# fmazilu/ASR-using-robust-NN

Hardware: AMD Instinct MI355X
Metric: utterances/sec (train, 1 s@16 kHz) (higher is better)
Workload: dtype f32 accumulate, fp16 two-plane split products in the training GEMMs (22-bit operands); 1 GPU; raw 16 kHz waveform -> on-GPU MFCC -> Lipschitz-constrained MLP train step (Adam+NonNeg, simple_norm_constraint rho=0.1), 1xMI355X; global_batch=1024, per_gpu_batch=1024, clip=1 s @ 16 kHz fp32, resident_pool_clips_per_gpu=65536, parallelism=dp1, hip_graph=False

## Files before the change

### asr-using-robust-nn_amd/build.py

```python
from __future__ import annotations

import os
import subprocess
import sys

HERE = os.path.dirname(os.path.abspath(__file__))
CSRC = os.path.join(HERE, "csrc")
OUT = os.path.join(HERE, "lipasr", "liblipasr.so")
SOURCES = ["core.hip", "spectral.hip", "gemm.hip", "mlp.hip", "optim.hip", "mfcc.hip", "mfcc_vjp.hip", "stft_bdft.hip", "lp_attack.hip"]
HEADERS = ["common.h", "mlp.h", "gemm.h", "mfcc_tables.h", "stft.h", os.path.join("..", "..", "include", "lipasr.h")]
EXTRA = {"stft_bdft.hip": ["-fno-slp-vectorize"]}
FLAGS = ["-O3", "--offload-arch=gfx950", "-fPIC", "-std=c++17", "-Wall", "-Wno-unused-function",
         "-fgpu-rdc" if False else "-fno-gpu-rdc"]


def _hipcc() -> str:
    for cand in (os.environ.get("HIPCC"), "/opt/rocm/bin/hipcc", "hipcc"):
        if cand and (os.path.isabs(cand) and os.path.exists(cand) or not os.path.isabs(cand)):
            return cand
    raise RuntimeError("hipcc not found")


def _stale() -> bool:
    if not os.path.exists(OUT):
        return True
    t = os.path.getmtime(OUT)
    deps = [os.path.join(CSRC, s) for s in SOURCES + HEADERS] + [os.path.abspath(__file__)]
    return any(os.path.getmtime(d) > t for d in deps)


def build(force: bool = False, verbose: bool = True) -> str:
    if not force and not _stale():
        return OUT
    objs = []
    procs = []
    os.makedirs(os.path.join(HERE, "build"), exist_ok=True)
    for s in SOURCES:
        obj = os.path.join(HERE, "build", s.replace(".hip", ".o"))
        cmd = [_hipcc(), *FLAGS, *EXTRA.get(s, []), "-c", os.path.join(CSRC, s), "-o", obj]
        if verbose:
            print(" ".join(cmd), flush=True)
        procs.append((s, subprocess.Popen(cmd, stdout=subprocess.PIPE, stderr=subprocess.STDOUT, text=True)))
        objs.append(obj)
    failed = False
    for s, p in procs:
        out, _ = p.communicate()
        if out.strip() and verbose:
            print(out)
        if p.returncode != 0:
            failed = True
            print(f"hipcc failed on {s}:\n{out}", file=sys.stderr)
    if failed:
        raise RuntimeError("liblipasr build failed")
    cmd = [_hipcc(), "--offload-arch=gfx950", "-shared", "-fPIC", *objs, "-o", OUT]
    if verbose:
        print(" ".join(cmd), flush=True)
    subprocess.check_call(cmd)
    return OUT


if __name__ == "__main__":
    print(build(force="--force" in sys.argv))
```

### asr-using-robust-nn_amd/csrc/gemm.h

```cpp
#pragma once
#include "mlp.h"

namespace lipasr {

enum Epi {
  EPI_STORE = 0,
  EPI_BIAS = 1,
  EPI_BIAS_RELU = 2,
  EPI_BIAS_RELU_BN = 3,
  EPI_DZ_INFER = 4,
  EPI_SIGNSTEP = 5,
  EPI_BIAS_RELU_STATS = 6,
  EPI_DH_STATS = 7,
  EPI_DZ_NOBN = 8,
  EPI_BIAS_SOFTMAX_CE = 9,
  EPI_BIAS_RELU_BNX = 10,
  EPI_DH_BNX = 11
};

struct DropArgs {
  int mode;
  float rate;
  uint64_t seed;
  const int* step_dev;
// ... 33 lines not shown
  float* extra_out;
  const float* y;
  float inv_batch;
  float* prob;
  float* dz;
  float* loss_rows;
  float* correct_rows;
  int bf16;
  const unsigned* sa_dyn;
  const unsigned* sb_dyn;
  unsigned* amax_out;
  unsigned* amax_zero;
  float sa, sb;
  int lds_min_tiles;
  const float* zeros;
  int cus;
  int ring;
  int xcd_map;
  unsigned long long* xc_gran;
  unsigned* xc_ctrl;
  int* xc_err;
  int xc_rt_max;
  int Bstat;
  float grad_scale;
  float* h_out;
  float* mmean_w;
  float* mvar_w;
  float* save_w;
  float* dgamma;
  float* dbeta;
};

constexpr int kAmaxSlots = 64, kAmaxStride = 16;
__device__ __forceinline__ float scale_from_amax(const unsigned* p, const float fallback) {
  if (!p) return fallback;
  const float a = wave_max(__uint_as_float(p[(threadIdx.x & 63) * kAmaxStride]));
  if (!(a > 0.0f) || !(a < INFINITY)) return 1.0f;
  int e = 0;
  (void)frexpf(a, &e);
  return ldexpf(1.0f, 14 - e);
}
__device__ __forceinline__ void amax_publish(unsigned* out, float m) {
  m = wave_max(m);
  if ((threadIdx.x & 63) == 0) {
    const unsigned w = (blockIdx.y * gridDim.x + blockIdx.x) * (blockDim.x >> 6) + (threadIdx.x >> 6);
    atomicMax(out + (w & (kAmaxSlots - 1)) * kAmaxStride, __float_as_uint(m));
  }
}
__device__ __forceinline__ void amax_clear(unsigned* out) {
  if (threadIdx.x < kAmaxSlots) out[threadIdx.x * kAmaxStride] = 0u;
}

constexpr int kMaxGroup = 8;
struct GemmGroup {
  int n;
  int tile_start[kMaxGroup + 1];
  GemmArgs g[kMaxGroup];
};

struct GemmKnobs {
  int gemm_mode = 0;
  bool split_dw0 = false;
  bool group_lds = true;
  int xcd_map = 0;
  bool no_ring = false;
  int ring_tile = 2;
  bool ring2 = true;
  bool ring_x1 = true;
};
const GemmKnobs& gemm_knobs();

enum GemmKind { GK_FRAG4 = 0, GK_FRAG16, GK_LDS, GK_RING, GK_RING_X1, GK_RING2, GK_KINDS };

struct GemmPick {
  int kind;
  int tile_m, tile_n, threads;
  size_t lds_bytes;
  const void* fn;
};

int pick_gemm(int amode, int bmode, const GemmArgs& g, GemmPick* out);
int launch_gemm(int amode, int bmode, const GemmArgs& g, hipStream_t st);
int launch_gemm_group_tn(const GemmArgs* gs, int n, hipStream_t st);
GemmArgs gemm_args(const float* A, int lda, const float* B, int ldb, float* C, int ldc, int M, int N, int K, int epi);
int gemm_row_tiles(int amode, int bmode, const GemmArgs& g);
bool exchange_fits(int bmode, int arith, int M, int N, int K, int lds_min_tiles, int xc_rt_max, int cus);

}
```

### asr-using-robust-nn_amd/csrc/gemm.hip

```cpp
#include "gemm.h"
#include <cstdint>
#include <map>
#include <mutex>
#include <type_traits>
#include <utility>

namespace lipasr {

typedef float f32x16 __attribute__((ext_vector_type(16)));
typedef __bf16 bf16x8 __attribute__((ext_vector_type(8)));

__device__ __forceinline__ bf16x8 to_bf16x8(const float (&v)[8]) {
  bf16x8 o;
#pragma unroll
  for (int j = 0; j < 8; ++j) o[j] = (__bf16)v[j];
  return o;
}

typedef _Float16 f16x8 __attribute__((ext_vector_type(8)));
typedef _Float16 f16x2v __attribute__((ext_vector_type(2)));
typedef float f32x2v __attribute__((ext_vector_type(2)));
template <bool UNIT>
__device__ __forceinline__ void split8(const float (&x)[8], const float scale, f16x8& hi, f16x8& lo) {
  unsigned h[4], l[4];
  if constexpr (UNIT) {
#pragma unroll
    for (int i = 0; i < 4; ++i) h[i] = __builtin_bit_cast(unsigned, __builtin_convertvector((f32x2v){x[2 * i], x[2 * i + 1]}, f16x2v));
    asm("v_fma_mixlo_f16 %0, %4, 1.0, -%12 op_sel_hi:[0,0,1]\n\t"
        "v_fma_mixlo_f16 %1, %6, 1.0, -%13 op_sel_hi:[0,0,1]\n\t"
        "v_fma_mixlo_f16 %2, %8, 1.0, -%14 op_sel_hi:[0,0,1]\n\t"
        "v_fma_mixlo_f16 %3, %10, 1.0, -%15 op_sel_hi:[0,0,1]\n\t"
        "v_fma_mixhi_f16 %0, %5, 1.0, -%12 op_sel:[0,0,1] op_sel_hi:[0,0,1]\n\t"
        "v_fma_mixhi_f16 %1, %7, 1.0, -%13 op_sel:[0,0,1] op_sel_hi:[0,0,1]\n\t"
        "v_fma_mixhi_f16 %2, %9, 1.0, -%14 op_sel:[0,0,1] op_sel_hi:[0,0,1]\n\t"
        "v_fma_mixhi_f16 %3, %11, 1.0, -%15 op_sel:[0,0,1] op_sel_hi:[0,0,1]\n\t"
        "s_nop 1"
        : "=&v"(l[0]), "=&v"(l[1]), "=&v"(l[2]), "=&v"(l[3])
        : "v"(x[0]), "v"(x[1]), "v"(x[2]), "v"(x[3]), "v"(x[4]), "v"(x[5]), "v"(x[6]), "v"(x[7]), "v"(h[0]), "v"(h[1]), "v"(h[2]), "v"(h[3]));
  } else {
    const float s = __builtin_bit_cast(float, __builtin_amdgcn_readfirstlane(__builtin_bit_cast(int, scale)));
    asm("v_fma_mixlo_f16 %0, %8, %16, 0 op_sel_hi:[0,0,0]\n\t"
        "v_fma_mixlo_f16 %1, %10, %16, 0 op_sel_hi:[0,0,0]\n\t"
        "v_fma_mixlo_f16 %2, %12, %16, 0 op_sel_hi:[0,0,0]\n\t"
        "v_fma_mixlo_f16 %3, %14, %16, 0 op_sel_hi:[0,0,0]\n\t"
        "v_fma_mixhi_f16 %0, %9, %16, 0 op_sel_hi:[0,0,0]\n\t"
        "v_fma_mixhi_f16 %1, %11, %16, 0 op_sel_hi:[0,0,0]\n\t"
        "v_fma_mixhi_f16 %2, %13, %16, 0 op_sel_hi:[0,0,0]\n\t"
        "v_fma_mixhi_f16 %3, %15, %16, 0 op_sel_hi:[0,0,0]\n\t"
        "v_fma_mixlo_f16 %4, %8, %16, -%0 op_sel_hi:[0,0,1]\n\t"
        "v_fma_mixlo_f16 %5, %10, %16, -%1 op_sel_hi:[0,0,1]\n\t"
        "v_fma_mixlo_f16 %6, %12, %16, -%2 op_sel_hi:[0,0,1]\n\t"
        "v_fma_mixlo_f16 %7, %14, %16, -%3 op_sel_hi:[0,0,1]\n\t"
        "v_fma_mixhi_f16 %4, %9, %16, -%0 op_sel:[0,0,1] op_sel_hi:[0,0,1]\n\t"
        "v_fma_mixhi_f16 %5, %11, %16, -%1 op_sel:[0,0,1] op_sel_hi:[0,0,1]\n\t"
        "v_fma_mixhi_f16 %6, %13, %16, -%2 op_sel:[0,0,1] op_sel_hi:[0,0,1]\n\t"
        "v_fma_mixhi_f16 %7, %15, %16, -%3 op_sel:[0,0,1] op_sel_hi:[0,0,1]\n\t"
        "s_nop 1"
        : "=&v"(h[0]), "=&v"(h[1]), "=&v"(h[2]), "=&v"(h[3]), "=&v"(l[0]), "=&v"(l[1]), "=&v"(l[2]), "=&v"(l[3])
        : "v"(x[0]), "v"(x[1]), "v"(x[2]), "v"(x[3]), "v"(x[4]), "v"(x[5]), "v"(x[6]), "v"(x[7]), "s"(s));
  }
  hi = __builtin_bit_cast(f16x8, make_uint4(h[0], h[1], h[2], h[3]));
  lo = __builtin_bit_cast(f16x8, make_uint4(l[0], l[1], l[2], l[3]));
}
// ... 259 lines not shown
    if (by == 0 && col < g.N) {
      g.dbeta[col] = dbt * g.grad_scale;
      g.dgamma[col] = dg * g.grad_scale;
    }
  }
}

struct BnxPre {
  float p0[4], p1[4], p2[4];
};
__device__ __forceinline__ void bnx_prefetch(const GemmArgs& g, const int gm, const int gn, BnxPre& q) {
  const bool rv = gm < g.M;
#pragma unroll
  for (int e = 0; e < 4; ++e) {
    const bool cv = rv && gn + e < g.N;
    if (g.epi == EPI_BIAS_RELU_BNX) {
      q.p0[e] = cv ? g.bias[gn + e] : 0.0f;
      q.p1[e] = 0.0f; q.p2[e] = 0.0f;
    } else {
      q.p0[e] = cv ? g.aux[(size_t)gm * g.ldc + gn + e] : 0.0f;
      q.p1[e] = cv ? g.save_mean[gn + e] : 0.0f;
      q.p2[e] = cv ? g.save_mean[g.N + gn + e] : 0.0f;
    }
  }
}

__device__ __forceinline__ void bnx_elem(const GemmArgs& g, const int step, const bool cv, const int gm, const int gn, const float acc,
                                         const BnxPre& q, const int e, float& val, float& av, float& s1, float& s2) {
  if (g.epi == EPI_BIAS_RELU_BNX) {
    const float a = cv ? fmaxf(acc + q.p0[e], 0.0f) : 0.0f;
    val = a; av = a; s1 = a; s2 = a * a;
  } else {
    const size_t idx = (size_t)gm * g.ldc + gn;
    const float gg = cv ? acc * dropout_mult(g.drop, step, idx) : 0.0f;
    const float a = q.p0[e];
    const float xh = cv ? (a - q.p1[e]) * q.p2[e] : 0.0f;
    val = gg; av = a; s1 = gg; s2 = gg * xh;
  }
}

__device__ __forceinline__ void xcd_tile(const int L, const int ntx, const int nty, int& bx, int& by) {
  const int total = ntx * nty;
  if (total < 16) { bx = L % ntx; by = L / ntx; return; }
  const int xcd = L & 7, q = L >> 3, base = total >> 3, rem = total & 7;
  const int t = xcd * base + min(xcd, rem) + q;
  int h = (int)(sqrtf((float)(base + (rem ? 1 : 0))) + 0.5f);
  h = max(1, min(h, nty));
  const int per_group = h * ntx, grp = t / per_group, u = t - grp * per_group;
  const int hg = min(h, nty - grp * h);
  bx = u / hg;
  by = grp * h + (u - bx * hg);
}

template <int AMODE, int BMODE, int NW, int BF, bool X = false>
__device__ __forceinline__ void gemm_tile(const GemmArgs& g, const int bx, const int by, const int n_row_tiles) {
  constexpr int TS = 32;
  constexpr int TPR = 8;
  extern __shared__ __attribute__((aligned(16))) float red[];
  float* stat = red + NW * TS * TS;
  const int tid = threadIdx.x, lane = tid & 63, wave = tid >> 6;
  const int r = lane & 31, h = lane >> 5;
  const int m0 = by * TS, n0 = bx * TS;
  const int nch = (g.K + 15) >> 4;
  const bool vecA = (AMODE == 0) && ((g.lda & 3) == 0) && ((reinterpret_cast<uintptr_t>(g.A) & 15) == 0);
  const bool vecB = (BMODE == 0) && ((g.ldb & 3) == 0) && ((reinterpret_cast<uintptr_t>(g.B) & 15) == 0);
  const int m_real = g.ones_row ? g.M - 1 : g.M;
  const int row_a = m0 + r;
  const bool aones = (AMODE == 1) && g.ones_row && (row_a == g.M - 1);
  const int ai = min(row_a, m_real - 1);
  const int bj = min(n0 + r, g.N - 1);

  unsigned xtag = 0;
  if constexpr (X) xtag = xc_tag<32>(XcView{g.xc_gran, g.xc_ctrl, g.xc_err, g.xc_rt_max}, bx);
  float rsa = 1.0f, rsb = 1.0f;
  if (BF == 2) { rsa = scale_from_amax(g.sa_dyn, g.sa); rsb = scale_from_amax(g.sb_dyn, g.sb); }
  if (g.amax_zero && bx == 0 && by == 0) amax_clear(g.amax_zero);
  f32x16 acc;
#pragma unroll
  for (int q = 0; q < 16; ++q) acc[q] = 0.0f;
  float a0[8], b0[8], a1[8], b1[8];
#pragma unroll
  for (int q = 0; q < 8; ++q) { a0[q] = b0[q] = a1[q] = b1[q] = 0.0f; }
  int c = wave;
  if (c < nch) {
    load_frag<AMODE>(g.A, g.lda, ai, c * 16 + 8 * h, g.K, vecA, a0, aones);
    load_frag<BMODE>(g.B, g.ldb, bj, c * 16 + 8 * h, g.K, vecB, b0);
  }
  while (c < nch) {
    const int cn = c + NW;
    if (cn < nch) {
      load_frag<AMODE>(g.A, g.lda, ai, cn * 16 + 8 * h, g.K, vecA, a1, aones);
      load_frag<BMODE>(g.B, g.ldb, bj, cn * 16 + 8 * h, g.K, vecB, b1);
    }
    if (BF == 1) {
      acc = __builtin_amdgcn_mfma_f32_32x32x16_bf16(to_bf16x8(a0), to_bf16x8(b0), acc, 0, 0, 0);
    } else if (BF == 2) {
      acc = mfma_split(a0, b0, rsa, rsb, acc);
    } else {
#pragma unroll
      for (int q = 0; q < 8; ++q) acc = __builtin_amdgcn_mfma_f32_32x32x2f32(a0[q], b0[q], acc, 0, 0, 0);
    }
#pragma unroll
    for (int q = 0; q < 8; ++q) { a0[q] = a1[q]; b0[q] = b1[q]; }
    c = cn;
  }
  if (BF == 2) {
    const float un = 1.0f / (rsa * rsb);
#pragma unroll
// ... 29 lines not shown
        for (int o = TPR; o < 64; o <<= 1) {
          c1[e] += __shfl_xor(c1[e], o, 64);
          c2[e] += __shfl_xor(c2[e], o, 64);
        }
      }
      if (lane < TPR) {
#pragma unroll
        for (int e = 0; e < 4; ++e) {
          stat[(wave * TPR + lane) * 8 + e] = c1[e];
          stat[(wave * TPR + lane) * 8 + 4 + e] = c2[e];
        }
      }
      __syncthreads();
      float* mine = red;
      float* colp = red + 64;
      double* sbuf = reinterpret_cast<double*>(red + 128);
      double* tot = sbuf + 4 * 64;
      if (tid < 2 * TS) {
        const int which = tid / TS, col = tid % TS, l4 = col >> 2, e = col & 3;
        float t = 0.0f;
#pragma unroll
        for (int w = 0; w < 4; ++w) t += stat[(w * TPR + l4) * 8 + which * 4 + e];
        mine[tid] = t;
      }
      __syncthreads();
      BnxLate late;
      bnx_late_load(g, gn, late);
      float mm0, mv0;
      bnx_moving_load(g, by, n0 + tid, tid < TS, mm0, mv0);
      XcView xc{g.xc_gran, g.xc_ctrl, g.xc_err, g.xc_rt_max};
      xc_exchange<256, 32>(xc, bx, by, g.Bstat < 0 ? 0 : n_row_tiles, xtag, mine, sbuf, tot, [&]() {
        if (g.epi == EPI_BIAS_RELU_BNX && gm1[0] < g.M) {
          float* crow = g.C + (size_t)gm1[0] * g.ldc;
          if (gn + 3 < g.N && ((g.ldc & 3) == 0) && ((reinterpret_cast<uintptr_t>(crow) & 15) == 0)) {
            *reinterpret_cast<float4*>(crow + gn) = make_float4(val[0][0], val[0][1], val[0][2], val[0][3]);
          } else {
#pragma unroll
            for (int e = 0; e < 4; ++e)
              if (gn + e < g.N) crow[gn + e] = val[0][e];
          }
        }
      });
      if (tid < TS) bnx_column(g, by, n0 + tid, tid, TS, tot, colp, mm0, mv0);
      __syncthreads();
      bnx_finish<1>(g, step, gm1, gn, val, av, colp, TS, c4, late);
      return;
    }
  }

  const bool stats = (g.epi == EPI_BIAS_RELU_STATS) || (g.epi == EPI_DH_STATS);
  float cs1[4] = {0.f, 0.f, 0.f, 0.f}, cs2[4] = {0.f, 0.f, 0.f, 0.f};
  if (tid < 256) {
    const int step = g.drop.step_dev ? *g.drop.step_dev : 0;
    const int tcol = tid & 7, row = tid >> 3;
    const int c4 = tcol * 4;
    const int gn = n0 + c4;
    float4 s = *reinterpret_cast<const float4*>(red + row * TS + c4);
#pragma unroll
    for (int w = 1; w < NW; ++w) {
      const float4 t = *reinterpret_cast<const float4*>(red + w * TS * TS + row * TS + c4);
      s.x += t.x; s.y += t.y; s.z += t.z; s.w += t.w;
    }
    const int gm = m0 + row;
    if (g.epi == EPI_BIAS_SOFTMAX_CE) {
      const bool rv = gm < g.M;
      float z[4];
      float mx = -INFINITY;
      int am = 0x7fffffff;
#pragma unroll
      for (int e = 0; e < 4; ++e) {
        const bool cv = rv && (gn + e < g.N);
        z[e] = cv ? (&s.x)[e] + g.bias[gn + e] : -INFINITY;
        if (z[e] > mx) { mx = z[e]; am = gn + e; }
      }
#pragma unroll
      for (int o2 = 1; o2 < 8; o2 <<= 1) {
        const float omx = __shfl_xor(mx, o2, 64);
        const int oam = __shfl_xor(am, o2, 64);
        if (omx > mx || (omx == mx && oam < am)) { mx = omx; am = oam; }
      }
      float se = 0.0f;
#pragma unroll
      for (int e = 0; e < 4; ++e) se += (z[e] > -INFINITY) ? expf(z[e] - mx) : 0.0f;
#pragma unroll
      for (int o2 = 1; o2 < 8; o2 <<= 1) se += __shfl_xor(se, o2, 64);
      const float lse = logf(se), inv = 1.0f / se;
      float loss = 0.0f, ymax = -INFINITY;
      int ay = 0x7fffffff;
#pragma unroll
      for (int e = 0; e < 4; ++e) {
        if (rv && gn + e < g.N) {
          const size_t idx = (size_t)gm * g.N + gn + e;
          const float zs = z[e] - mx;
          const float pc = expf(zs) * inv;
          g.C[(size_t)gm * g.ldc + gn + e] = z[e];
          if (g.prob) g.prob[idx] = pc;
          if (g.y) {
            const float yc = g.y[idx];
            if (yc != 0.0f) loss -= yc * (zs - lse);
            if (yc > ymax) { ymax = yc; ay = gn + e; }
            if (g.dz) g.dz[idx] = (pc - yc) * g.inv_batch;
          }
        }
      }
#pragma unroll
      for (int o2 = 1; o2 < 8; o2 <<= 1) {
        loss += __shfl_xor(loss, o2, 64);
        const float oym = __shfl_xor(ymax, o2, 64);
        const int oay = __shfl_xor(ay, o2, 64);
        if (oym > ymax || (oym == ymax && oay < ay)) { ymax = oym; ay = oay; }
      }
      if (rv && tcol == 0) {
        if (g.loss_rows) g.loss_rows[gm] = loss;
        if (g.correct_rows) g.correct_rows[gm] = (am == ay) ? 1.0f : 0.0f;
      }
    } else if (gm < g.M) {
      const float v[4] = {s.x, s.y, s.z, s.w};
      float o[4];
#pragma unroll
      for (int e = 0; e < 4; ++e) {
        float t1 = 0.0f, t2 = 0.0f;
        o[e] = (gn + e < g.N) ? epilogue_elem(g, step, gm, gn + e, v[e], t1, t2) : 0.0f;
        cs1[e] = t1;
        cs2[e] = t2;
      }
      float* crow;
      if (g.ones_row && gm == g.M - 1) crow = g.extra_out;
      else crow = (g.epi == EPI_SIGNSTEP ? g.x_adv : g.C) + (size_t)gm * g.ldc;
      if (gn + 3 < g.N && ((g.ldc & 3) == 0) && ((reinterpret_cast<uintptr_t>(crow) & 15) == 0)) {
        *reinterpret_cast<float4*>(crow + gn) = make_float4(o[0], o[1], o[2], o[3]);
      } else {
#pragma unroll
        for (int e = 0; e < 4; ++e)
          if (gn + e < g.N) crow[gn + e] = o[e];
      }
    }
  }
  if (stats) {
    if (tid < 256) {
#pragma unroll
      for (int e = 0; e < 4; ++e) {
#pragma unroll
        for (int o = TPR; o < 64; o <<= 1) {
          cs1[e] += __shfl_xor(cs1[e], o, 64);
          cs2[e] += __shfl_xor(cs2[e], o, 64);
        }
      }
      if (lane < TPR) {
#pragma unroll
        for (int e = 0; e < 4; ++e) {
          stat[(wave * TPR + lane) * 8 + e] = cs1[e];
          stat[(wave * TPR + lane) * 8 + 4 + e] = cs2[e];
        }
      }
    }
    __syncthreads();
    if (tid < 2 * TS) {
      const int which = tid / TS, col = tid % TS;
      const int l4 = col >> 2, e = col & 3;
      float t = 0.0f;
#pragma unroll
      for (int w = 0; w < 4; ++w) t += stat[(w * TPR + l4) * 8 + which * 4 + e];
      if (n0 + col < g.N) g.part[((size_t)which * n_row_tiles + by) * g.N + n0 + col] = t;
    }
  }
}

template <int AMODE, int BMODE, int NW, int BF = 0, bool X = false>
__global__ __launch_bounds__(64 * NW) void gemm_f32_kernel(GemmArgs g) {
  int bx = blockIdx.x, by = blockIdx.y;
  if (g.xcd_map) xcd_tile(blockIdx.y * gridDim.x + blockIdx.x, gridDim.x, gridDim.y, bx, by);
  gemm_tile<AMODE, BMODE, NW, BF, X>(g, bx, by, gridDim.y);
}


template <int AMODE, int BMODE, int NW, int BF = 0>
__global__ __launch_bounds__(64 * NW) void gemm_f32_grouped_kernel(GemmGroup grp) {
  int p = 0;
  while (p + 1 < grp.n && (int)blockIdx.x >= grp.tile_start[p + 1]) ++p;
  const GemmArgs& g = grp.g[p];
  const int local = blockIdx.x - grp.tile_start[p];
  const int ntx = (g.N + 31) / 32, nty = (g.M + 31) / 32;
  int bx = local % ntx, by = local / ntx;
  if (g.xcd_map && (grp.tile_start[p] & 7) == 0) xcd_tile(local, ntx, nty, bx, by);
  gemm_tile<AMODE, BMODE, NW, BF>(g, bx, by, nty);
}

constexpr int kLdsBK = 32, kLdsLD = 68;

template <int MODE>
__device__ __forceinline__ float4 tile_fetch(const float* __restrict__ P, int ld, int i0, int i_real, int k0, int K,
                                             bool ones_last, int i_last, int tid) {
  float t[4] = {0.f, 0.f, 0.f, 0.f};
  const bool al = ((ld & 3) == 0) && ((reinterpret_cast<uintptr_t>(P) & 15) == 0);
  if (MODE == 0) {
    const int i = i0 + (tid >> 3);
    const int kq = k0 + (tid & 7) * 4;
    const float* p = P + (size_t)min(i, i_real - 1) * ld + kq;
    if (kq + 3 < K && al) {
      const float4 x = *reinterpret_cast<const float4*>(p);
      t[0] = x.x; t[1] = x.y; t[2] = x.z; t[3] = x.w;
    } else {
#pragma unroll
      for (int c = 0; c < 4; ++c) t[c] = (kq + c < K) ? p[c] : 0.0f;
    }
  } else {
    const int k = k0 + (tid >> 4);
    const int iq = i0 + (tid & 15) * 4;
    if (k < K) {
      const float* p = P + (size_t)k * ld;
      if (iq + 3 < i_real && al) {
        const float4 x = *reinterpret_cast<const float4*>(p + iq);
        t[0] = x.x; t[1] = x.y; t[2] = x.z; t[3] = x.w;
      } else {
#pragma unroll
        for (int c = 0; c < 4; ++c) {
          const int i = iq + c;
          t[c] = (ones_last && i == i_last) ? 1.0f : p[min(i, i_real - 1)];
        }
      }
    }
  }
  return make_float4(t[0], t[1], t[2], t[3]);
}

template <int MODE>
__device__ __forceinline__ void tile_store(float* __restrict__ S, int tid, const float4 v) {
  if (MODE == 0) {
    const int i = tid >> 3, kq = (tid & 7) * 4;
    S[(kq + 0) * kLdsLD + i] = v.x;
    S[(kq + 1) * kLdsLD + i] = v.y;
    S[(kq + 2) * kLdsLD + i] = v.z;
    S[(kq + 3) * kLdsLD + i] = v.w;
  } else {
    const int k = tid >> 4, iq = (tid & 15) * 4;
    *reinterpret_cast<float4*>(S + k * kLdsLD + iq) = v;
  }
}

constexpr int kLdsBKMax = 32;
constexpr size_t lds_gemm_bytes(int bk) {
  return ((size_t)(2 * 2 * bk * kLdsLD > 2 * 64 * 64 ? 2 * 2 * bk * kLdsLD : 2 * 64 * 64) + 8 * 16 * 8) * sizeof(float);
}

template <bool X>
__device__ __forceinline__ void lds_tile_epilogue(const GemmArgs& g, const f32x16& acc, float* lds, float* stat, const int bx, const int by,
                                                  const int n_row_tiles, const unsigned xtag) {
  constexpr int TS = 64;
  const int tid = threadIdx.x, lane = tid & 63, wave = tid >> 6;
  const int r = lane & 31, h = lane >> 5;
  const int kh = wave >> 2, wi = (wave >> 1) & 1, wj = wave & 1;
  const int m0 = by * TS, n0 = bx * TS;
  BnxPre xpre[2];
  if constexpr (X) {
    bnx_prefetch(g, m0 + (tid >> 4), n0 + (tid & 15) * 4, xpre[0]);
    bnx_prefetch(g, m0 + (tid >> 4) + 32, n0 + (tid & 15) * 4, xpre[1]);
  }
  float* red = lds;
#pragma unroll
  for (int q = 0; q < 16; ++q) {
    const int row = 32 * wi + (q & 3) + 8 * (q >> 2) + 4 * h;
    red[kh * TS * TS + row * TS + 32 * wj + r] = acc[q];
  }
  __syncthreads();
  const bool stats = (g.epi == EPI_BIAS_RELU_STATS) || (g.epi == EPI_DH_STATS);
  const int step = g.drop.step_dev ? *g.drop.step_dev : 0;
  const int tcol = tid & 15, trow = tid >> 4;
  const int c4 = tcol * 4, gn = n0 + c4;
  if constexpr (X) {
    const int gm2[2] = {m0 + trow, m0 + trow + 32};
    float val[2][4], av[2][4], c1[4] = {0.f, 0.f, 0.f, 0.f}, c2[4] = {0.f, 0.f, 0.f, 0.f};
#pragma unroll
    for (int pass = 0; pass < 2; ++pass) {
      const int row = trow + 32 * pass;
      float4 s = *reinterpret_cast<const float4*>(red + row * TS + c4);
      const float4 s2 = *reinterpret_cast<const float4*>(red + TS * TS + row * TS + c4);
      const float accv[4] = {s.x + s2.x, s.y + s2.y, s.z + s2.z, s.w + s2.w};
#pragma unroll
      for (int e = 0; e < 4; ++e) {
        float t1, t2;
        bnx_elem(g, step, gm2[pass] < g.M && gn + e < g.N, gm2[pass], gn + e, accv[e], xpre[pass], e, val[pass][e], av[pass][e], t1, t2);
        c1[e] += t1;
        c2[e] += t2;
      }
    }
#pragma unroll
    for (int e = 0; e < 4; ++e) {
      c1[e] += __shfl_xor(c1[e], 16, 64); c1[e] += __shfl_xor(c1[e], 32, 64);
      c2[e] += __shfl_xor(c2[e], 16, 64); c2[e] += __shfl_xor(c2[e], 32, 64);
    }
    if (lane < 16) {
#pragma unroll
      for (int e = 0; e < 4; ++e) {
        stat[(wave * 16 + lane) * 8 + e] = c1[e];
        stat[(wave * 16 + lane) * 8 + 4 + e] = c2[e];
      }
    }
    __syncthreads();
    float* mine = red;
    float* colp = red + 128;
    double* sbuf = reinterpret_cast<double*>(red + 256);
    double* tot = sbuf + 4 * 128;
    if (tid < 2 * TS) {
      const int which = tid / TS, col = tid % TS, l4 = col >> 2, e = col & 3;
      float t = 0.0f;
#pragma unroll
      for (int w = 0; w < 8; ++w) t += stat[(w * 16 + l4) * 8 + which * 4 + e];
      mine[tid] = t;
    }
    __syncthreads();
    BnxLate late;
    bnx_late_load(g, gn, late);
    float mm0, mv0;
    bnx_moving_load(g, by, n0 + tid, tid < TS, mm0, mv0);
    XcView xc{g.xc_gran, g.xc_ctrl, g.xc_err, g.xc_rt_max};
    xc_exchange<512, 64>(xc, bx, by, g.Bstat < 0 ? 0 : n_row_tiles, xtag, mine, sbuf, tot, [&]() {
      if (g.epi != EPI_BIAS_RELU_BNX) return;
#pragma unroll
      for (int pass = 0; pass < 2; ++pass) {
        if (gm2[pass] >= g.M) continue;
        float* crow = g.C + (size_t)gm2[pass] * g.ldc;
        if (gn + 3 < g.N && ((g.ldc & 3) == 0) && ((reinterpret_cast<uintptr_t>(crow) & 15) == 0)) {
          *reinterpret_cast<float4*>(crow + gn) = make_float4(val[pass][0], val[pass][1], val[pass][2], val[pass][3]);
        } else {
#pragma unroll
          for (int e = 0; e < 4; ++e)
            if (gn + e < g.N) crow[gn + e] = val[pass][e];
        }
      }
    });
    if (tid < TS) bnx_column(g, by, n0 + tid, tid, TS, tot, colp, mm0, mv0);
    __syncthreads();
    bnx_finish<2>(g, step, gm2, gn, val, av, colp, TS, c4, late);
    return;
  }
  float cs1[4] = {0.f, 0.f, 0.f, 0.f}, cs2[4] = {0.f, 0.f, 0.f, 0.f};
#pragma unroll
  for (int pass = 0; pass < 2; ++pass) {
    const int row = trow + 32 * pass;
    float4 s = *reinterpret_cast<const float4*>(red + row * TS + c4);
    const float4 s2 = *reinterpret_cast<const float4*>(red + TS * TS + row * TS + c4);
    s.x += s2.x; s.y += s2.y; s.z += s2.z; s.w += s2.w;
    const int gm = m0 + row;
    if (gm < g.M) {
      const float v[4] = {s.x, s.y, s.z, s.w};
      float o[4];
#pragma unroll
      for (int e = 0; e < 4; ++e) {
        float t1 = 0.0f, t2 = 0.0f;
        o[e] = (gn + e < g.N) ? epilogue_elem(g, step, gm, gn + e, v[e], t1, t2) : 0.0f;
        cs1[e] += t1;
        cs2[e] += t2;
      }
      float* crow;
      if (g.ones_row && gm == g.M - 1) crow = g.extra_out;
      else crow = (g.epi == EPI_SIGNSTEP ? g.x_adv : g.C) + (size_t)gm * g.ldc;
      if (gn + 3 < g.N && ((g.ldc & 3) == 0) && ((reinterpret_cast<uintptr_t>(crow) & 15) == 0)) {
        *reinterpret_cast<float4*>(crow + gn) = make_float4(o[0], o[1], o[2], o[3]);
      } else {
#pragma unroll
        for (int e = 0; e < 4; ++e)
          if (gn + e < g.N) crow[gn + e] = o[e];
      }
    }
  }
  if (stats) {
#pragma unroll
    for (int e = 0; e < 4; ++e) {
      cs1[e] += __shfl_xor(cs1[e], 16, 64); cs1[e] += __shfl_xor(cs1[e], 32, 64);
      cs2[e] += __shfl_xor(cs2[e], 16, 64); cs2[e] += __shfl_xor(cs2[e], 32, 64);
    }
    if (lane < 16) {
#pragma unroll
      for (int e = 0; e < 4; ++e) {
        stat[(wave * 16 + lane) * 8 + e] = cs1[e];
        stat[(wave * 16 + lane) * 8 + 4 + e] = cs2[e];
      }
    }
    __syncthreads();
    if (tid < 2 * TS) {
      const int which = tid / TS, col = tid % TS;
      const int l4 = col >> 2, e = col & 3;
      float t = 0.0f;
#pragma unroll
      for (int w = 0; w < 8; ++w) t += stat[(w * 16 + l4) * 8 + which * 4 + e];
      if (n0 + col < g.N) g.part[((size_t)which * n_row_tiles + by) * g.N + n0 + col] = t;
    }
  }
}


template <int AMODE, int BMODE, int BF, int BK, bool X = false>
__device__ __forceinline__ void gemm_lds_tile(const GemmArgs& g, const int bx, const int by, const int n_row_tiles) {
  constexpr int TS = 64;
  constexpr int NF = BK / kLdsBK;
  extern __shared__ __attribute__((aligned(16))) float lds[];
  float* stat = lds + (2 * 2 * BK * kLdsLD > 2 * 64 * 64 ? 2 * 2 * BK * kLdsLD : 2 * 64 * 64);
  const int tid = threadIdx.x, lane = tid & 63, wave = tid >> 6;
  const int r = lane & 31, h = lane >> 5;
  const int kh = wave >> 2, wi = (wave >> 1) & 1, wj = wave & 1;
  const int m0 = by * TS, n0 = bx * TS;
  const int m_real = g.ones_row ? g.M - 1 : g.M;
  const int nst = (g.K + BK - 1) / BK;
  const bool ones = g.ones_row != 0;
  unsigned xtag = 0;
  if constexpr (X) xtag = xc_tag<64>(XcView{g.xc_gran, g.xc_ctrl, g.xc_err, g.xc_rt_max}, bx);
  float rsa = 1.0f, rsb = 1.0f;
  if (BF == 2) { rsa = scale_from_amax(g.sa_dyn, g.sa); rsb = scale_from_amax(g.sb_dyn, g.sb); }
  if (g.amax_zero && bx == 0 && by == 0) amax_clear(g.amax_zero);
  f32x16 acc;
#pragma unroll
  for (int q = 0; q < 16; ++q) acc[q] = 0.0f;
  struct Tile { float4 a[NF], b[NF]; };
  auto fetch = [&](Tile& tl, const int t) {
#pragma unroll
    for (int f = 0; f < NF; ++f) {
      tl.a[f] = tile_fetch<AMODE>(g.A, g.lda, m0, m_real, t * BK + f * kLdsBK, g.K, ones, g.M - 1, tid);
      tl.b[f] = tile_fetch<BMODE>(g.B, g.ldb, n0, g.N, t * BK + f * kLdsBK, g.K, false, 0, tid);
    }
  };
  auto park = [&](const Tile& tl, const int t) {
    float* An = lds + (t & 1) * 2 * BK * kLdsLD;
#pragma unroll
    for (int f = 0; f < NF; ++f) {
      tile_store<AMODE>(An + f * kLdsBK * kLdsLD, tid, tl.a[f]);
      tile_store<BMODE>(An + BK * kLdsLD + f * kLdsBK * kLdsLD, tid, tl.b[f]);
    }
  };
  Tile t0, t1;
  fetch(t0, 0);
  if (nst > 1) fetch(t1, 1);
  park(t0, 0);
  __syncthreads();
  auto kstep = [&](const int t, Tile& free_slot, const Tile& ready) {
    if (t + 2 < nst) fetch(free_slot, t + 2);
    constexpr int kstr = BF ? kLdsLD : 2 * kLdsLD;
    const int koff = BF ? 8 * h : h;
    const float* base = lds + (t & 1) * 2 * BK * kLdsLD + ((BK / 2) * kh + koff) * kLdsLD + r;
#pragma unroll
    for (int q = 0; q < BK / 32; ++q) {
      const float* As = base + 16 * q * kLdsLD + 32 * wi;
      const float* Bs = base + BK * kLdsLD + 16 * q * kLdsLD + 32 * wj;
      float av[8], bv[8];
#pragma unroll
      for (int s = 0; s < 8; ++s) {
        av[s] = As[s * kstr];
        bv[s] = Bs[s * kstr];
      }
      if (BF == 1) {
        acc = __builtin_amdgcn_mfma_f32_32x32x16_bf16(to_bf16x8(av), to_bf16x8(bv), acc, 0, 0, 0);
      } else if (BF == 2) {
        acc = mfma_split(av, bv, rsa, rsb, acc);
      } else {
#pragma unroll
        for (int s = 0; s < 8; ++s) acc = __builtin_amdgcn_mfma_f32_32x32x2f32(av[s], bv[s], acc, 0, 0, 0);
      }
    }
    if (t + 1 < nst) park(ready, t + 1);
    __syncthreads();
  };
  for (int t = 0; t < nst; t += 2) {
    kstep(t, t0, t1);
    if (t + 1 < nst) kstep(t + 1, t1, t0);
  }
  if (BF == 2) {
    const float un = 1.0f / (rsa * rsb);
#pragma unroll
    for (int q = 0; q < 16; ++q) acc[q] *= un;
  }
  lds_tile_epilogue<X>(g, acc, lds, stat, bx, by, n_row_tiles, xtag);
}


#ifndef LIPASR_RING_STAGES
#define LIPASR_RING_STAGES 4
#endif
constexpr int kRingStages = LIPASR_RING_STAGES;
constexpr int kRingTile = 64 * 32;
constexpr size_t ring_gemm_bytes() { return (size_t)(kRingStages * 2 * kRingTile + 8 * 16 * 8) * sizeof(float); }

__device__ __forceinline__ void dma16(const float* gsrc, const unsigned lds_byte_addr) {
  unsigned keep;
  asm volatile("s_mov_b32 %0, m0\n\ts_mov_b32 m0, %2\n\ts_nop 0\n\tglobal_load_lds_dwordx4 %1, off\n\ts_mov_b32 m0, %0"
               : "=&s"(keep)
               : "v"(gsrc), "s"(lds_byte_addr)
               : "memory");
}

template <int MODE>
__device__ __forceinline__ const float* ring_src(const float* P, const int ld, const int i0, const int i_real, const int wave, const int lane) {
  if (MODE == 1) {
    const int k = 4 * wave + (lane >> 4), i = min(i0 + (lane & 15) * 4, i_real - 4);
    return P + (size_t)k * ld + i;
  }
  const int il = 8 * wave + (lane >> 3), c = (lane & 7) ^ ((il >> 1) & 7);
  return P + (size_t)min(i0 + il, i_real - 1) * ld + 4 * c;
}
template <int MODE>
__device__ __forceinline__ size_t ring_step(const int ld) { return MODE == 1 ? (size_t)32 * ld : (size_t)32; }

template <int MODE>
__device__ __forceinline__ void ring_frag(const float* __restrict__ T, const int il, const int kh, const int hh, float (&v)[8]) {
  if (MODE == 1) {
    const float* q = T + (16 * kh + 8 * hh) * 64 + il;
#pragma unroll
    for (int s = 0; s < 8; ++s) v[s] = q[s * 64];
  } else {
    const int sw = (il >> 1) & 7, c0 = 4 * kh + 2 * hh;
    const float4 lo = *reinterpret_cast<const float4*>(T + (il * 8 + (c0 ^ sw)) * 4);
    const float4 hi = *reinterpret_cast<const float4*>(T + (il * 8 + ((c0 + 1) ^ sw)) * 4);
    v[0] = lo.x; v[1] = lo.y; v[2] = lo.z; v[3] = lo.w;
    v[4] = hi.x; v[5] = hi.y; v[6] = hi.z; v[7] = hi.w;
  }
}

template <int AMODE, int BMODE, bool X = false, int NL = 0>
__device__ __forceinline__ void gemm_ring_tile(const GemmArgs& g, const int bx, const int by, const int n_row_tiles) {
  constexpr int TS = 64, S = kRingStages;
  extern __shared__ __attribute__((aligned(16))) float lds[];
  float* stat = lds + S * 2 * kRingTile;
  const int tid = threadIdx.x, lane = tid & 63;
  const int wave = __builtin_amdgcn_readfirstlane(tid >> 6);
  const int r = lane & 31, hh = lane >> 5;
  const int kh = wave >> 2, wi = (wave >> 1) & 1, wj = wave & 1;
  const int m0 = by * TS, n0 = bx * TS;
  const int m_real = g.ones_row ? g.M - 1 : g.M;
  const int nst = (g.K + 31) >> 5;
  unsigned xtag = 0;
  if constexpr (X) xtag = xc_tag<64>(XcView{g.xc_gran, g.xc_ctrl, g.xc_err, g.xc_rt_max}, bx);
  const int koff_a = AMODE == 1 ? 4 * wave + (lane >> 4) : 4 * ((lane & 7) ^ (((8 * wave + (lane >> 3)) >> 1) & 7));
  const int koff_b = BMODE == 1 ? 4 * wave + (lane >> 4) : 4 * ((lane & 7) ^ (((8 * wave + (lane >> 3)) >> 1) & 7));
  const bool k_tail = (g.K & 31) != 0;
  const float rsa = scale_from_amax(g.sa_dyn, g.sa), rsb = scale_from_amax(g.sb_dyn, g.sb);
  if (g.amax_zero && bx == 0 && by == 0) amax_clear(g.amax_zero);
  const float* pa = ring_src<AMODE>(g.A, g.lda, m0, m_real, wave, lane);
  const float* pb = ring_src<BMODE>(g.B, g.ldb, n0, g.N, wave, lane);
  const size_t sa_step = ring_step<AMODE>(g.lda), sb_step = ring_step<BMODE>(g.ldb);
  const unsigned lds0 = __builtin_amdgcn_readfirstlane((unsigned)(size_t)lds) + (unsigned)wave * 1024u;
  auto issue = [&](const int t) {
    const unsigned slot = lds0 + (unsigned)(t % S) * (2u * kRingTile * 4u);
    const bool last = k_tail && t == nst - 1;
    dma16((last && 32 * t + koff_a >= g.K) ? g.zeros : pa, slot);
    dma16((last && 32 * t + koff_b >= g.K) ? g.zeros : pb, slot + kRingTile * 4u);
    pa += sa_step;
    pb += sb_step;
  };
  const int il_ones = (AMODE == 1 && g.ones_row && g.M - 1 >= m0 && g.M - 1 < m0 + TS) ? g.M - 1 - m0 : -1;
  if constexpr (NL > 0) {
    if (wave >= 8) {
      const int L = wave - 8;
      constexpr int NP = 8 / NL;
      const float* sa[NP];
      const float* sb[NP];
      int ka[NP], kb[NP];
#pragma unroll
      for (int q = 0; q < NP; ++q) {
        const int w = L + NL * q;
        sa[q] = ring_src<AMODE>(g.A, g.lda, m0, m_real, w, lane);
        sb[q] = ring_src<BMODE>(g.B, g.ldb, n0, g.N, w, lane);
        ka[q] = AMODE == 1 ? 4 * w + (lane >> 4) : 4 * ((lane & 7) ^ (((8 * w + (lane >> 3)) >> 1) & 7));
        kb[q] = BMODE == 1 ? 4 * w + (lane >> 4) : 4 * ((lane & 7) ^ (((8 * w + (lane >> 3)) >> 1) & 7));
      }
      const unsigned base = __builtin_amdgcn_readfirstlane((unsigned)(size_t)lds);
      auto issue_l = [&](const int t) {
        const unsigned slot = base + (unsigned)(t % S) * (2u * kRingTile * 4u);
        const bool last = k_tail && t == nst - 1;
#pragma unroll
        for (int q = 0; q < NP; ++q) {
          const unsigned d = slot + (unsigned)(L + NL * q) * 1024u;
          dma16((last && 32 * t + ka[q] >= g.K) ? g.zeros : sa[q], d);
// ... 4 lines not shown
      };
      for (int t = 0; t < min(S - 1, nst); ++t) issue_l(t);
      for (int t = 0; t < nst; ++t) {
        const int ahead = min(t + S - 2, nst - 1) - t;
        if (ahead >= 2) asm volatile("s_waitcnt vmcnt(%0)" ::"n"(4 * NP) : "memory");
        else if (ahead == 1) asm volatile("s_waitcnt vmcnt(%0)" ::"n"(2 * NP) : "memory");
        else asm volatile("s_waitcnt vmcnt(0)" ::: "memory");
        if (il_ones >= 0 && lane < 4 * NP) lds[(t % S) * 2 * kRingTile + (4 * (L + NL * (lane >> 2)) + (lane & 3)) * 64 + il_ones] = 1.0f;
        __syncthreads();
        if (t + S - 1 < nst) issue_l(t + S - 1);
      }
      __syncthreads();
      return;
    }
  }
  const int pre = NL > 0 ? 0 : min(S - 1, nst);
  for (int t = 0; t < pre; ++t) issue(t);
  f32x16 acc;
#pragma unroll
  for (int q = 0; q < 16; ++q) acc[q] = 0.0f;
  auto k_loop = [&](auto unit_a) {
    constexpr bool UA = decltype(unit_a)::value;
    for (int t = 0; t < nst; ++t) {
      float* At = lds + (t % S) * 2 * kRingTile;
      if constexpr (NL == 0) {
        const int ahead = min(t + S - 2, nst - 1) - t;
        if (ahead >= 2) asm volatile("s_waitcnt vmcnt(4)" ::: "memory");
        else if (ahead == 1) asm volatile("s_waitcnt vmcnt(2)" ::: "memory");
        else asm volatile("s_waitcnt vmcnt(0)" ::: "memory");
        if (il_ones >= 0 && lane < 4) At[(4 * wave + lane) * 64 + il_ones] = 1.0f;
      }
      __syncthreads();
#if !defined(LIPASR_RING_PROBE) || LIPASR_RING_PROBE != 2
      if constexpr (NL == 0) {
        if (t + S - 1 < nst) issue(t + S - 1);
      }
#endif
#if !defined(LIPASR_RING_PROBE) || LIPASR_RING_PROBE != 1
      float av[8], bv[8];
      ring_frag<AMODE>(At, 32 * wi + r, kh, hh, av);
      ring_frag<BMODE>(At + kRingTile, 32 * wj + r, kh, hh, bv);
      acc = mfma_split<UA>(av, bv, rsa, rsb, acc);
#endif
    }
  };
  if (rsa == 1.0f) k_loop(std::true_type{});
  else k_loop(std::false_type{});
  {
    const float un = 1.0f / (rsa * rsb);
#pragma unroll
    for (int q = 0; q < 16; ++q) acc[q] *= un;
  }
  __syncthreads();
  lds_tile_epilogue<X>(g, acc, lds, stat, bx, by, n_row_tiles, xtag);
}

#ifndef LIPASR_RING_LOADERS
#define LIPASR_RING_LOADERS 0
#endif
constexpr int kRingLoaders = LIPASR_RING_LOADERS;
template <int AMODE, int BMODE, bool X = false>
__global__ __launch_bounds__(512 + 64 * kRingLoaders) void gemm_ring_kernel(GemmArgs g) {
  int bx = blockIdx.x, by = blockIdx.y;
  if (g.xcd_map) xcd_tile(blockIdx.y * gridDim.x + blockIdx.x, gridDim.x, gridDim.y, bx, by);
  gemm_ring_tile<AMODE, BMODE, X, kRingLoaders>(g, bx, by, gridDim.y);
}
constexpr int kRingLoadersOnePerCu = 4;
template <int BMODE>
__global__ __launch_bounds__(512 + 64 * kRingLoadersOnePerCu) void gemm_ring_x1_kernel(GemmArgs g) {
  int bx = blockIdx.x, by = blockIdx.y;
  if (g.xcd_map) xcd_tile(blockIdx.y * gridDim.x + blockIdx.x, gridDim.x, gridDim.y, bx, by);
  gemm_ring_tile<0, BMODE, true, kRingLoadersOnePerCu>(g, bx, by, gridDim.y);
}

template <int AMODE, int BMODE, int BF = 0, int BK = kLdsBKMax, bool X = false>
__global__ __launch_bounds__(512) void gemm_lds_kernel(GemmArgs g) {
  int bx = blockIdx.x, by = blockIdx.y;
  if (g.xcd_map) xcd_tile(blockIdx.y * gridDim.x + blockIdx.x, gridDim.x, gridDim.y, bx, by);
  gemm_lds_tile<AMODE, BMODE, BF, BK, X>(g, bx, by, gridDim.y);
}

template <int AMODE, int BMODE, int BF = 0>
__global__ __launch_bounds__(512) void gemm_lds_grouped_kernel(GemmGroup grp) {
  int p = 0;
  while (p + 1 < grp.n && (int)blockIdx.x >= grp.tile_start[p + 1]) ++p;
  const GemmArgs& g = grp.g[p];
  const int local = blockIdx.x - grp.tile_start[p];
  const int ntx = (g.N + 63) / 64, nty = (g.M + 63) / 64;
  int bx = local % ntx, by = local / ntx;
  if (g.xcd_map && (grp.tile_start[p] & 7) == 0) xcd_tile(local, ntx, nty, bx, by);
  gemm_lds_tile<AMODE, BMODE, BF, kLdsBKMax>(g, bx, by, nty);
}


constexpr int kR128Stages = 3;
constexpr int kR128Tile = 32 * 128;
constexpr size_t ring128_bytes() { return (size_t)(kR128Stages * 2 * kR128Tile) * sizeof(float); }

__device__ __forceinline__ void gemm_ring128_tile(const GemmArgs& g, const int bx, const int by) {
  constexpr int TS = 128, S = kR128Stages;
  extern __shared__ __attribute__((aligned(16))) float lds[];
  const int tid = threadIdx.x, lane = tid & 63;
  const int wave = __builtin_amdgcn_readfirstlane(tid >> 6);
  const int r = lane & 31, hh = lane >> 5;
  const int ri = wave >> 1, cj = wave & 1;
  const int m0 = by * TS, n0 = bx * TS;
  const int m_real = g.ones_row ? g.M - 1 : g.M;
  const int nst = (g.K + 31) >> 5;
  const float rsa = scale_from_amax(g.sa_dyn, g.sa), rsb = scale_from_amax(g.sb_dyn, g.sb);
  const int kl = 4 * wave + (lane >> 5), il = (lane & 31) * 4;
  const float* pa = g.A + (size_t)kl * g.lda + min(m0 + il, m_real - 4);
  const float* pb = g.B + (size_t)kl * g.ldb + min(n0 + il, g.N - 4);
  const size_t a2 = (size_t)2 * g.lda, b2 = (size_t)2 * g.ldb, a32 = (size_t)32 * g.lda, b32 = (size_t)32 * g.ldb;
  const bool k_tail = (g.K & 31) != 0;
  const unsigned lds0 = __builtin_amdgcn_readfirstlane((unsigned)(size_t)lds) + (unsigned)wave * 2048u;
  auto issue = [&](const int t) {
    const unsigned slot = lds0 + (unsigned)(t % S) * (2u * kR128Tile * 4u);
    const bool z0 = k_tail && 32 * t + kl >= g.K, z1 = k_tail && 32 * t + kl + 2 >= g.K;
    dma16(z0 ? g.zeros : pa, slot);
    dma16(z1 ? g.zeros : pa + a2, slot + 1024u);
    dma16(z0 ? g.zeros : pb, slot + kR128Tile * 4u);
    dma16(z1 ? g.zeros : pb + b2, slot + kR128Tile * 4u + 1024u);
    pa += a32;
    pb += b32;
  };
  const int pre = min(S - 1, nst);
  for (int t = 0; t < pre; ++t) issue(t);
  const int il_ones = (g.ones_row && g.M - 1 >= m0 && g.M - 1 < m0 + TS) ? g.M - 1 - m0 : -1;
  f32x16 acc0, acc1;
#pragma unroll
  for (int q = 0; q < 16; ++q) { acc0[q] = 0.0f; acc1[q] = 0.0f; }
  auto k_loop = [&](auto unit_a) {
  constexpr bool UA = decltype(unit_a)::value;
  for (int t = 0; t < nst; ++t) {
    const int ahead = min(t + S - 2, nst - 1) - t;
    if (ahead >= 1) asm volatile("s_waitcnt vmcnt(4)" ::: "memory");
    else asm volatile("s_waitcnt vmcnt(0)" ::: "memory");
    float* At = lds + (t % S) * 2 * kR128Tile;
    if (il_ones >= 0 && lane < 4) At[(4 * wave + lane) * TS + il_ones] = 1.0f;
    __syncthreads();
#if !defined(LIPASR_RING_PROBE) || LIPASR_RING_PROBE != 2
    if (t + S - 1 < nst) issue(t + S - 1);
#endif
    const float* Bt = At + kR128Tile;
#if !defined(LIPASR_RING_PROBE) || LIPASR_RING_PROBE != 1
#pragma unroll
    for (int c = 0; c < 2; ++c) {
      const float* qa = At + (16 * c + 8 * hh) * TS + 32 * ri + r;
      const float* qb = Bt + (16 * c + 8 * hh) * TS + 64 * cj + r;
      float av[8], b0[8], b1[8];
#pragma unroll
      for (int s8 = 0; s8 < 8; ++s8) {
        av[s8] = qa[s8 * TS];
        b0[s8] = qb[s8 * TS];
        b1[s8] = qb[s8 * TS + 32];
      }
      f16x8 ah, al, bh, bl;
      split8<UA>(av, rsa, ah, al);
      split8<false>(b0, rsb, bh, bl);
      acc0 = __builtin_amdgcn_mfma_f32_32x32x16_f16(ah, bh, acc0, 0, 0, 0);
      acc0 = __builtin_amdgcn_mfma_f32_32x32x16_f16(ah, bl, acc0, 0, 0, 0);
      acc0 = __builtin_amdgcn_mfma_f32_32x32x16_f16(al, bh, acc0, 0, 0, 0);
      split8<false>(b1, rsb, bh, bl);
      acc1 = __builtin_amdgcn_mfma_f32_32x32x16_f16(ah, bh, acc1, 0, 0, 0);
      acc1 = __builtin_amdgcn_mfma_f32_32x32x16_f16(ah, bl, acc1, 0, 0, 0);
      acc1 = __builtin_amdgcn_mfma_f32_32x32x16_f16(al, bh, acc1, 0, 0, 0);
    }
#else
    (void)Bt;
#endif
  }
  };
  if (rsa == 1.0f) k_loop(std::true_type{});
  else k_loop(std::false_type{});
  const float un = 1.0f / (rsa * rsb);
  const int gn0 = n0 + 64 * cj + r, gn1 = gn0 + 32;
#pragma unroll
  for (int q = 0; q < 16; ++q) {
    const int gm = m0 + 32 * ri + (q & 3) + 8 * (q >> 2) + 4 * hh;
    if (gm >= g.M) continue;
    float* crow = (g.ones_row && gm == g.M - 1) ? g.extra_out : g.C + (size_t)gm * g.ldc;
    if (gn0 < g.N) crow[gn0] = acc0[q] * un;
    if (gn1 < g.N) crow[gn1] = acc1[q] * un;
  }
}

#ifndef LIPASR_R128_LOADERS
#define LIPASR_R128_LOADERS 4
#endif
constexpr int kR128Loaders = LIPASR_R128_LOADERS;
constexpr int kR128PlaneBytes = 128 * 64;
constexpr size_t ring128s_bytes() { return ring128_bytes() + (size_t)2 * 4 * kR128PlaneBytes; }

__device__ __forceinline__ void gemm_ring128s_tile(const GemmArgs& g, const int bx, const int by) {
  constexpr int TS = 128, S = kR128Stages;
  extern __shared__ __attribute__((aligned(16))) float lds[];
  char* const planes = reinterpret_cast<char*>(lds) + ring128_bytes();
  const int tid = threadIdx.x, lane = tid & 63;
  const int wave = __builtin_amdgcn_readfirstlane(tid >> 6);
  const int r = lane & 31, hh = lane >> 5;
  const int ri = wave >> 1, cj = wave & 1;
  const int m0 = by * TS, n0 = bx * TS;
  const int m_real = g.ones_row ? g.M - 1 : g.M;
  const int nst = (g.K + 31) >> 5;
  const float rsa = scale_from_amax(g.sa_dyn, g.sa), rsb = scale_from_amax(g.sb_dyn, g.sb);
  const int il_ones = (g.ones_row && g.M - 1 >= m0 && g.M - 1 < m0 + TS) ? g.M - 1 - m0 : -1;
  if (wave >= 8) {
    const int L = wave - 8;
    constexpr int NQ = 32 / kR128Loaders;
    const float* src[NQ];
    int krow[NQ];
    unsigned dst[NQ];
#pragma unroll
    for (int q = 0; q < NQ; ++q) {
      const int op = q / (NQ / 2), j = kR128Loaders * (q % (NQ / 2)) + L;
      krow[q] = 2 * j + (lane >> 5);
      const int c = (lane & 31) * 4;
      src[q] = op ? g.B + (size_t)krow[q] * g.ldb + min(n0 + c, g.N - 4) : g.A + (size_t)krow[q] * g.lda + min(m0 + c, m_real - 4);
      dst[q] = (unsigned)op * (unsigned)(kR128Tile * 4) + (unsigned)j * 1024u;
    }
    const size_t a32 = (size_t)32 * g.lda, b32 = (size_t)32 * g.ldb;
    const bool k_tail = (g.K & 31) != 0;
    const unsigned lds0 = __builtin_amdgcn_readfirstlane((unsigned)(size_t)lds);
    auto issue = [&](const int t) {
      const unsigned slot = lds0 + (unsigned)(t % S) * (2u * kR128Tile * 4u);
#pragma unroll
      for (int q = 0; q < NQ; ++q) {
#if defined(LIPASR_R128_PROBE) && LIPASR_R128_PROBE == 3
        dma16(g.zeros, slot + dst[q]);
#else
        dma16((k_tail && 32 * t + krow[q] >= g.K) ? g.zeros : src[q], slot + dst[q]);
#endif
        src[q] += q < NQ / 2 ? a32 : b32;
      }
    };
    for (int t = 0; t < min(2, nst); ++t) issue(t);
    for (int t = 0; t <= nst; ++t) {
      if (t < nst) {
        if (t + 1 < nst) asm volatile("s_waitcnt vmcnt(%0)" ::"n"(NQ) : "memory");
        else asm volatile("s_waitcnt vmcnt(0)" ::: "memory");
        if (il_ones >= 0 && lane < NQ) {
          const int k = 2 * (kR128Loaders * (lane >> 1) + L) + (lane & 1);
          lds[(t % S) * 2 * kR128Tile + k * TS + il_ones] = 1.0f;
        }
      }
      __syncthreads();
#if !defined(LIPASR_R128_PROBE) || LIPASR_R128_PROBE != 2
      if (t + 2 < nst) issue(t + 2);
#endif
    }
    return;
  }
  const int si = 64 * (wave & 1) + lane, sc = wave >> 1;
  const unsigned sp_off = (unsigned)si * 64u + (unsigned)((sc ^ ((si >> 2) & 3)) << 4);
  const int row_a = 32 * ri + r, row_b = 64 * cj + r;
  unsigned off_a[2], off_b[2];
#pragma unroll
  for (int cc = 0; cc < 2; ++cc) {
    off_a[cc] = (unsigned)row_a * 64u + (unsigned)(((2 * cc + hh) ^ ((row_a >> 2) & 3)) << 4);
    off_b[cc] = (unsigned)row_b * 64u + (unsigned)(((2 * cc + hh) ^ ((row_b >> 2) & 3)) << 4);
  }
  f32x16 acc0, acc1;
#pragma unroll
  for (int q = 0; q < 16; ++q) { acc0[q] = 0.0f; acc1[q] = 0.0f; }
  auto k_loop = [&](auto unit_a) {
    constexpr bool UA = decltype(unit_a)::value;
    for (int t = 0; t <= nst; ++t) {
      __syncthreads();
#if !defined(LIPASR_R128_PROBE) || (LIPASR_R128_PROBE != 1 && LIPASR_R128_PROBE != 3)
      if (t < nst) {
        const float* Ra = lds + (t % S) * 2 * kR128Tile + (8 * sc) * TS + si;
        char* P = planes + (t & 1) * 4 * kR128PlaneBytes + sp_off;
        float av[8], bv[8];
#pragma unroll
        for (int s8 = 0; s8 < 8; ++s8) {
          av[s8] = Ra[s8 * TS];
          bv[s8] = Ra[kR128Tile + s8 * TS];
        }
        f16x8 h, l;
        split8<UA>(av, rsa, h, l);
        *reinterpret_cast<f16x8*>(P) = h;
        *reinterpret_cast<f16x8*>(P + kR128PlaneBytes) = l;
        split8<false>(bv, rsb, h, l);
        *reinterpret_cast<f16x8*>(P + 2 * kR128PlaneBytes) = h;
        *reinterpret_cast<f16x8*>(P + 3 * kR128PlaneBytes) = l;
      }
      if (t >= 1) {
        const char* P = planes + ((t - 1) & 1) * 4 * kR128PlaneBytes;
#pragma unroll
        for (int cc = 0; cc < 2; ++cc) {
          const f16x8 ah = *reinterpret_cast<const f16x8*>(P + off_a[cc]);
          const f16x8 al = *reinterpret_cast<const f16x8*>(P + kR128PlaneBytes + off_a[cc]);
          const f16x8 b0h = *reinterpret_cast<const f16x8*>(P + 2 * kR128PlaneBytes + off_b[cc]);
          const f16x8 b0l = *reinterpret_cast<const f16x8*>(P + 3 * kR128PlaneBytes + off_b[cc]);
          const f16x8 b1h = *reinterpret_cast<const f16x8*>(P + 2 * kR128PlaneBytes + off_b[cc] + 32 * 64);
          const f16x8 b1l = *reinterpret_cast<const f16x8*>(P + 3 * kR128PlaneBytes + off_b[cc] + 32 * 64);
          acc0 = __builtin_amdgcn_mfma_f32_32x32x16_f16(ah, b0h, acc0, 0, 0, 0);
          acc1 = __builtin_amdgcn_mfma_f32_32x32x16_f16(ah, b1h, acc1, 0, 0, 0);
          acc0 = __builtin_amdgcn_mfma_f32_32x32x16_f16(ah, b0l, acc0, 0, 0, 0);
          acc1 = __builtin_amdgcn_mfma_f32_32x32x16_f16(ah, b1l, acc1, 0, 0, 0);
          acc0 = __builtin_amdgcn_mfma_f32_32x32x16_f16(al, b0h, acc0, 0, 0, 0);
          acc1 = __builtin_amdgcn_mfma_f32_32x32x16_f16(al, b1h, acc1, 0, 0, 0);
        }
      }
#endif
    }
  };
  if (rsa == 1.0f) k_loop(std::true_type{});
  else k_loop(std::false_type{});
  const float un = 1.0f / (rsa * rsb);
  const int gn0 = n0 + 64 * cj + r, gn1 = gn0 + 32;
#pragma unroll
  for (int q = 0; q < 16; ++q) {
    const int gm = m0 + 32 * ri + (q & 3) + 8 * (q >> 2) + 4 * hh;
    if (gm >= g.M) continue;
    float* crow = (g.ones_row && gm == g.M - 1) ? g.extra_out : g.C + (size_t)gm * g.ldc;
    if (gn0 < g.N) crow[gn0] = acc0[q] * un;
    if (gn1 < g.N) crow[gn1] = acc1[q] * un;
  }
}

__global__ __launch_bounds__(512 + 64 * kR128Loaders) void gemm_ring_grouped_kernel(GemmGroup grp) {
  int p = 0;
  while (p + 1 < grp.n && (int)blockIdx.x >= grp.tile_start[p + 1]) ++p;
  const GemmArgs& g = grp.g[p];
  const int local = blockIdx.x - grp.tile_start[p];
  const int ts = g.ring >= 2 ? 128 : 64;
  const int ntx = (g.N + ts - 1) / ts, nty = (g.M + ts - 1) / ts;
  int bx = local % ntx, by = local / ntx;
  if (g.xcd_map && (grp.tile_start[p] & 7) == 0) xcd_tile(local, ntx, nty, bx, by);
  if (g.ring == 2) { gemm_ring128s_tile(g, bx, by); return; }
  if (threadIdx.x >= 512) return;
  if (g.ring == 3) gemm_ring128_tile(g, bx, by);
  else if (g.ring) gemm_ring_tile<1, 1>(g, bx, by, nty);
  else gemm_lds_tile<1, 1, 2, kLdsBKMax>(g, bx, by, nty);
}

constexpr int kR2TileA = 128 * 32, kR2TileB = 64 * 32;
constexpr int kR2Slot = kR2TileA + kR2TileB;
constexpr int kR2Stages = 3;
constexpr int kR2PlaneA = 128 * 64, kR2PlaneB = 64 * 64;
constexpr int kR2Planes = 2 * kR2PlaneA + 2 * kR2PlaneB;
constexpr size_t ring2_bytes() { return (size_t)kR2Stages * kR2Slot * sizeof(float) + 2 * (size_t)kR2Planes + (size_t)8 * 16 * 8 * sizeof(float); }
#ifndef LIPASR_R2_LOADERS
#define LIPASR_R2_LOADERS 4
#endif
constexpr int kR2Loaders = LIPASR_R2_LOADERS;

template <int BMODE>
__device__ __forceinline__ void gemm_ring2_tile(const GemmArgs& g, const int bx, const int by, const int n_row_tiles) {
  constexpr int S = kR2Stages;
  extern __shared__ __attribute__((aligned(16))) float lds[];
  char* const planes = reinterpret_cast<char*>(lds + S * kR2Slot);
  float* const stat = reinterpret_cast<float*>(planes + 2 * kR2Planes);
  const int tid = threadIdx.x, lane = tid & 63;
  const int wave = __builtin_amdgcn_readfirstlane(tid >> 6);
  const int r = lane & 31, hh = lane >> 5;
  const int ri = wave >> 1, cj = wave & 1;
  const int m0 = by * 128, n0 = bx * 64;
  const int nst = (g.K + 31) >> 5;
  const unsigned xtag = xc_tag<64>(XcView{g.xc_gran, g.xc_ctrl, g.xc_err, g.xc_rt_max}, bx);
  const float rsa = scale_from_amax(g.sa_dyn, g.sa), rsb = scale_from_amax(g.sb_dyn, g.sb);
  if (g.amax_zero && bx == 0 && by == 0) amax_clear(g.amax_zero);
  if (wave >= 8) {
    const int L = wave - 8;
    constexpr int NQ = 24 / kR2Loaders;
    const float* src[NQ];
    int koff[NQ];
#pragma unroll
    for (int q = 0; q < NQ; ++q) {
      const int j = kR2Loaders * q + L;
      if (j < 16) {
        const int row = 8 * j + (lane >> 3);
        koff[q] = 4 * ((lane & 7) ^ ((row >> 1) & 7));
        src[q] = g.A + (size_t)min(m0 + row, g.M - 1) * g.lda + koff[q];
      } else if (BMODE == 1) {
        koff[q] = 4 * (j - 16) + (lane >> 4);
        src[q] = g.B + (size_t)koff[q] * g.ldb + min(n0 + (lane & 15) * 4, g.N - 4);
      } else {
        const int br = 8 * (j - 16) + (lane >> 3);
        koff[q] = 4 * ((lane & 7) ^ ((br >> 1) & 7));
        src[q] = g.B + (size_t)min(n0 + br, g.N - 1) * g.ldb + koff[q];
      }
    }
    const size_t sb_step = BMODE == 1 ? (size_t)32 * g.ldb : (size_t)32;
    const bool k_tail = (g.K & 31) != 0;
    const unsigned lds0 = __builtin_amdgcn_readfirstlane((unsigned)(size_t)lds);
    auto issue = [&](const int t) {
// ... 285 lines not shown
    kind = ring_legal(amode, bmode, g) ? GK_RING : GK_LDS;
  } else {
    const long tiles = (long)((g.N + 31) / 32) * ((g.M + 31) / 32);
    const bool deep = tiles <= 192 && g.K >= 512 && g.epi != EPI_BIAS_RELU_STATS && g.epi != EPI_DH_STATS;
    kind = deep ? GK_FRAG16 : GK_FRAG4;
  }
  *out = gemm_instance(kind, exchange, amode ? 1 : 0, bmode ? 1 : 0, kind >= GK_RING ? 2 : arith_index(g.bf16));
  if (!out->fn) { set_error("gemm: no kernel instance for this problem"); return LIPASR_EINVAL; }
  return LIPASR_OK;
}

int launch_gemm(int amode, int bmode, const GemmArgs& g, hipStream_t st) {
  GemmPick p;
  const int rc = pick_gemm(amode, bmode, g, &p);
  if (rc != LIPASR_OK) return rc;
  if (p.kind == GK_RING2) ++g_launch_count[0];
  (void)ensure_dyn_lds(p.fn, p.lds_bytes);
  void* args[] = {const_cast<GemmArgs*>(&g)};
  (void)hipLaunchKernel(p.fn, dim3((g.N + p.tile_n - 1) / p.tile_n, (g.M + p.tile_m - 1) / p.tile_m), dim3(p.threads), args, p.lds_bytes, st);
  LP_LAUNCH_CHECK();
  return LIPASR_OK;
}

int gemm_row_tiles(int amode, int bmode, const GemmArgs& g) {
  GemmPick p;
  return pick_gemm(amode, bmode, g, &p) == LIPASR_OK ? (g.M + p.tile_m - 1) / p.tile_m : 0;
}

static int blocks_per_cu(const GemmPick& p) {
  int occ = 0;
  (void)ensure_dyn_lds(p.fn, p.lds_bytes);
  if (hipOccupancyMaxActiveBlocksPerMultiprocessor(&occ, p.fn, p.threads, p.lds_bytes) != hipSuccess) { (void)hipGetLastError(); return 0; }
  const int by_sgpr = 24 / (p.threads / 64);
  return std::min(occ, by_sgpr);
}

bool exchange_fits(int bmode, int arith, int M, int N, int K, int lds_min_tiles, int xc_rt_max, int cus) {
  const bool lds_k = use_lds_gemm(M, N, K, lds_min_tiles);
  const int ts = lds_k ? 64 : 32;
  const long row_tiles = (M + ts - 1) / ts, tiles = row_tiles * ((N + ts - 1) / ts);
  if (row_tiles > xc_rt_max || row_tiles > 64) return false;
  static int per_cu[2][2][3] = {{{-1, -1, -1}, {-1, -1, -1}}, {{-1, -1, -1}, {-1, -1, -1}}}, ring_pc[2] = {-1, -1};
  const int b = bmode ? 1 : 0, ar = arith_index(arith);
  int& pc = per_cu[b][lds_k ? 1 : 0][ar];
  if (pc < 0) pc = blocks_per_cu(gemm_instance(lds_k ? GK_LDS : GK_FRAG4, true, 0, b, ar));
  int per = pc;
  if (ar == 2 && lds_k) {
    if (ring_pc[b] < 0) ring_pc[b] = blocks_per_cu(gemm_instance(GK_RING, true, 0, b, 2));
    per = std::min(per, ring_pc[b]);
  }
  return per > 0 && tiles <= (long)per * cus;
}

int launch_gemm_group_tn(const GemmArgs* gs, int n, hipStream_t st) {
  int done = 0;
  while (done < n) {
    GemmGroup grp;
    memset(&grp, 0, sizeof(grp));
    long big = 0;
    for (int k = 0; k < kMaxGroup && done + k < n; ++k)
      big += (long)((gs[done + k].N + 63) / 64) * ((gs[done + k].M + 63) / 64);
    const bool lds_tiles = g_knobs.group_lds && big >= 128 && gs[done].K >= 64;
    const int ts = lds_tiles ? 64 : 32;
    const int ar = gs[done].bf16;
    int ring_tile = g_knobs.ring_tile;
    if (ring_tile >= 2 && lds_tiles && ar == 2) {
      long n128 = 0;
      for (int q = 0; q < kMaxGroup && done + q < n; ++q)
        if (ring_legal(1, 1, gs[done + q])) n128 += (long)((gs[done + q].N + 127) / 128) * ((gs[done + q].M + 127) / 128);
      if (10 * n128 < 4 * (long)(gs[done].cus > 0 ? gs[done].cus : device_cus())) ring_tile = 1;
    }
    int k = 0, tiles = 0;
    bool any_ring = false;
    for (; k < kMaxGroup && done + k < n; ++k) {
      const GemmArgs& g = gs[done + k];
      if (g.M <= 0 || g.N <= 0 || g.K <= 0) { set_error("grouped gemm: empty problem"); return LIPASR_EINVAL; }
      grp.g[k] = g;
      if (lds_tiles && ar == 2 && ring_legal(1, 1, g)) { grp.g[k].ring = ring_tile; any_ring = true; }
      const int tp = grp.g[k].ring >= 2 ? 128 : ts;
      grp.tile_start[k] = tiles;
      tiles += ((g.N + tp - 1) / tp) * ((g.M + tp - 1) / tp);
    }
    grp.n = k;
    grp.tile_start[k] = tiles;
    const GemmTable& t = gemm_table();
    const void* fn = lds_tiles ? t.grouped_lds[arith_index(ar)] : t.grouped_frag[arith_index(ar)];
    int threads = lds_tiles ? 512 : 256;
    size_t lds = lds_tiles ? lds_gemm_bytes(kLdsBKMax) : frag_gemm_bytes(4);
    if (any_ring) {
      fn = t.grouped_ring;
      if (ring_tile == 2 && !ensure_dyn_lds(fn, ring128s_bytes())) {
        ring_tile = 3;
        for (int q = 0; q < k; ++q) if (grp.g[q].ring == 2) grp.g[q].ring = 3;
      }
      lds = std::max(ring_gemm_bytes(), ring_tile == 2 ? ring128s_bytes() : ring_tile == 3 ? ring128_bytes() : (size_t)0);
      threads = ring_tile == 2 ? 512 + 64 * kR128Loaders : 512;
      if (ring_tile == 2) ++g_launch_count[1];
    }
    (void)ensure_dyn_lds(fn, lds);
    void* args[] = {&grp};
    (void)hipLaunchKernel(fn, dim3(tiles), dim3(threads), args, lds, st);
    LP_LAUNCH_CHECK();
    done += k;
  }
  return LIPASR_OK;
}

GemmArgs gemm_args(const float* A, int lda, const float* B, int ldb, float* C, int ldc, int M, int N, int K, int epi) {
  GemmArgs g;
  memset(&g, 0, sizeof(g));
  g.A = A; g.B = B; g.C = C; g.M = M; g.N = N; g.K = K; g.lda = lda; g.ldb = ldb; g.ldc = ldc; g.epi = epi;
  g.xcd_map = g_knobs.xcd_map;
  g.sa = g.sb = 1.0f;
  return g;
}

}

using namespace lipasr;

extern "C" {

long lipasr_debug_launch_count(int kind) { return (kind == 0 || kind == 1) ? g_launch_count[kind] : -1; }

int lipasr_debug_gemm_mode(int mode) {
  GemmKnobs k;
  k.gemm_mode = mode & 3;
  k.split_dw0 = (mode >> 2) & 1;
  k.group_lds = !((mode >> 3) & 1);
  k.xcd_map = (mode >> 4) & 1;
  k.no_ring = (mode >> 5) & 1;
  k.ring_tile = ((mode >> 6) & 1) ? 1 : ((mode >> 7) & 1) ? 3 : 2;
  k.ring2 = !((mode >> 8) & 1);
  k.ring_x1 = !((mode >> 9) & 1);
  g_knobs = k;
  return LIPASR_OK;
}

int lipasr_gemm_f32(lipasr_handle_t h, int transA, int transB, int M, int N, int K, const float* A, int lda,
                    const float* B, int ldb, float* C, int ldc, lipasr_stream_t stream) {
  LP_CHECK_ARG(h && A && B && C, "lipasr_gemm_f32: null argument");
  LP_CHECK_ARG(M > 0 && N > 0 && K > 0, "lipasr_gemm_f32: empty problem %dx%dx%d", M, N, K);
  LP_CHECK_ARG(lda >= (transA ? M : K) && ldb >= (transB ? K : N) && ldc >= N, "lipasr_gemm_f32: leading dimension too small");
  GemmArgs g = gemm_args(A, lda, B, ldb, C, ldc, M, N, K, EPI_STORE);
  return launch_gemm(transA ? 1 : 0, transB ? 0 : 1, g, S(stream));
}

int lipasr_gemm_f16x2(lipasr_handle_t h, int transA, int transB, int M, int N, int K, const float* A, int lda, const float* B,
                      int ldb, float* C, int ldc, float scale_a, float scale_b, lipasr_stream_t stream) {
  LP_CHECK_ARG(h && A && B && C, "lipasr_gemm_f16x2: null argument");
  LP_CHECK_ARG(M > 0 && N > 0 && K > 0, "lipasr_gemm_f16x2: empty problem %dx%dx%d", M, N, K);
  LP_CHECK_ARG(lda >= (transA ? M : K) && ldb >= (transB ? K : N) && ldc >= N, "lipasr_gemm_f16x2: leading dimension too small");
  int ea = 0, eb = 0;
  LP_CHECK_ARG(scale_a > 0.0f && scale_b > 0.0f && frexpf(scale_a, &ea) == 0.5f && frexpf(scale_b, &eb) == 0.5f,
// ... 11 lines not shown
```

### asr-using-robust-nn_amd/csrc/mlp.h

```cpp
#pragma once
#include "common.h"

namespace lipasr {

struct MlpLayer {
  int n_in = 0, n_out = 0;
  bool bn = false, nonneg = false;
  float dropout = 0.f;
  size_t offW = 0, offb = 0, offg = 0, offbe = 0;
  size_t offmm = 0, offmv = 0;
  size_t offA = 0;
  size_t offH = 0;
  size_t offMean = 0;
  size_t offDz = 0;
};

constexpr float kBnMomentum = 0.99f;
constexpr float kBnEps = 1e-3f;

}

struct lipasr_mlp {
  lipasr_ctx* ctx = nullptr;
  int n_layers = 0;
  int max_batch = 0;
  int max_width = 0;
  lipasr::MlpLayer L[LIPASR_MAX_LAYERS];
  size_t n_params = 0, n_state = 0;
  float* ws = nullptr;
  size_t ws_floats = 0;
  size_t offLogits = 0, offProb = 0, offDzLast = 0, offG0 = 0, offG1 = 0, offG2 = 0, offPart = 0;
  int compute_bf16 = 0;
  float last_inv_batch = 1.0f;
  int lds_min_tiles = 0;
  int fuse_bn = 1;
  int cu_budget = 0;
  int n_cus = 0;
  int xc_rt_max = 0;
  unsigned long long* xc_gran = nullptr;
  unsigned* xc_ctrl = nullptr;
  unsigned* amax = nullptr;
  int* xc_err = nullptr;
  size_t xc_gran_off[2][LIPASR_MAX_LAYERS] = {};
  size_t xc_ctrl_off[2][LIPASR_MAX_LAYERS] = {};
};
```

### asr-using-robust-nn_amd/csrc/mlp.hip

```cpp
#include "gemm.h"
#include <cstdlib>

namespace lipasr {

enum OperandKind { OP_ACT = 0, OP_WEIGHT = 1, OP_GRAD = 2 };
static float grad_scale_for(float g0) {
  int e = 0;
  (void)frexpf(g0 > 0.0f ? g0 : 1.0f, &e);
  return ldexpf(1.0f, 8 - e);
}
static int plan_cus(const lipasr_mlp* m) { return m->cu_budget > 0 ? std::min(m->cu_budget, m->n_cus) : m->n_cus; }
static void set_arith(GemmArgs& g, const lipasr_mlp* m, int kind_a, int kind_b, float g0 = 1.0f, bool training = true) {
  g.bf16 = (m->compute_bf16 == 2 && !training) ? 0 : m->compute_bf16;
  g.zeros = reinterpret_cast<const float*>(m->xc_ctrl + 4);
  g.cus = plan_cus(m);
  const float sc[3] = {1.0f, 4096.0f, grad_scale_for(g0)};
  g.sa = sc[kind_a];
  g.sb = sc[kind_b];
}
static bool bnx_fits(const lipasr_mlp* m, bool forward, int M, int N, int K) {
  if (!m->fuse_bn || !m->xc_gran) return false;
  return exchange_fits(forward ? 1 : 0, m->compute_bf16, M, N, K, m->lds_min_tiles, m->xc_rt_max, plan_cus(m));
}
#ifdef LIPASR_PROBES
// ... 633 lines not shown
    gx.drop = drop_for_layer(m, l - 1, dropout);
    gx.part = part;
    if (P.bn) gx.save_mean = ws + P.offMean;
    if (bnx) {
      gx.xc_gran = m->xc_gran + m->xc_gran_off[1][l - 1]; gx.xc_ctrl = m->xc_ctrl + m->xc_ctrl_off[1][l - 1]; gx.xc_err = m->xc_err;
      gx.xc_rt_max = m->xc_rt_max;
      gx.Bstat = xc_nowait() ? -bstat : bstat; gx.grad_scale = sa.grad_scale;
      gx.gamma = params + P.offg;
      gx.dgamma = grads + P.offg; gx.dbeta = grads + P.offbe;
    }
    set_arith(gx, m, OP_GRAD, OP_WEIGHT, inv_batch);
    const bool dyn = m->compute_bf16 == 2;
    if (dyn && l < Lc - 1 && L.bn) gx.sa_dyn = m->amax + (size_t)l * kAmaxSlots * kAmaxStride;
    if (dyn && P.bn) gx.amax_out = m->amax + (size_t)(l - 1) * kAmaxSlots * kAmaxStride;
    gx.lds_min_tiles = m->lds_min_tiles;
    if (LP_ON) {
      rc = launch_gemm(0, 0, gx, st);
      if (rc != LIPASR_OK) return rc;
      if (sa.seg >= 0 && P.bn) {
        hipLaunchKernelGGL(part_reduce_kernel, dim3((P.n_out + 255) / 256), dim3(256), 0, st, part,
                           gemm_row_tiles(0, 0, gx), P.n_out);
        LP_LAUNCH_CHECK();
      }
    }
    if (P.bn) ++cur;
    if (P.bn && LP_ON && !bnx) {
      BnBwdArgs b;
      memset(&b, 0, sizeof(b));
      b.g = tmp; b.a = ws + P.offA; b.dz = ws + P.offDz; b.B = batch; b.N = P.n_out;
      b.Bstat = bstat; b.grad_scale = sa.grad_scale;
      b.part = part;
      b.n_tiles = sa.seg >= 0 ? 1 : gemm_row_tiles(0, 0, gx);
      b.gamma = params + P.offg; b.save_mean = ws + P.offMean;
      b.dgamma = grads + P.offg; b.dbeta = grads + P.offbe;
      b.amax_out = dyn ? m->amax + (size_t)(l - 1) * kAmaxSlots * kAmaxStride : nullptr;
      const dim3 grid((P.n_out + 127) / 128, (batch + kApplyRows - 1) / kApplyRows);
      hipLaunchKernelGGL(bn_apply_bwd_kernel, grid, apply_block, 0, st, b);
      LP_LAUNCH_CHECK();
    }
  }
  GemmArgs gw[LIPASR_MAX_LAYERS];
  for (int l = 0; l < Lc; ++l) {
    const MlpLayer& L = m->L[l];
    const float* lin = (l == 0) ? x : (ws + m->L[l - 1].offH);
    const float* gin = (l == Lc - 1) ? (ws + m->offDzLast) : (ws + L.offDz);
    gw[l] = gemm_args(lin, L.n_in, gin, L.n_out, grads + L.offW, L.n_out, L.n_in + 1, L.n_out, batch, EPI_STORE);
    gw[l].ones_row = 1;
    gw[l].extra_out = grads + L.offb;
    set_arith(gw[l], m, OP_ACT, OP_GRAD, inv_batch);
    if (m->compute_bf16 == 2 && l < Lc - 1 && L.bn) gw[l].sb_dyn = m->amax + (size_t)l * kAmaxSlots * kAmaxStride;
  }
  if (!LP_ON) return LIPASR_OK;
#undef LP_ON
  if (dw_mode == 0 || Lc == 1) return launch_gemm_group_tn(gw, Lc, st);
  rc = launch_gemm_group_tn(gw + 1, Lc - 1, st);
  if (rc != LIPASR_OK || dw_mode == 2) return rc;
  return launch_gemm(1, 1, gw[0], st);
}

int lipasr_mlp_train_fwd_bwd(lipasr_mlp_t m, const float* params, float* bnstate, const float* x, const float* y_onehot,
                             int batch, float inv_batch, const lipasr_dropout_cfg* dropout, float* grads,
                             float* loss_rows, float* correct_rows, float* probs, lipasr_stream_t stream) {
  return train_fwd_bwd_impl(m, params, bnstate, x, y_onehot, batch, inv_batch, dropout, grads, loss_rows, correct_rows, probs,
                            stream, gemm_knobs().split_dw0 ? 1 : 0);
}

int lipasr_mlp_train_fwd_bwd_head(lipasr_mlp_t m, const float* params, float* bnstate, const float* x, const float* y_onehot,
                                  int batch, float inv_batch, const lipasr_dropout_cfg* dropout, float* grads,
                                  float* loss_rows, float* correct_rows, float* probs, lipasr_stream_t stream) {
  return train_fwd_bwd_impl(m, params, bnstate, x, y_onehot, batch, inv_batch, dropout, grads, loss_rows, correct_rows, probs,
                            stream, 2);
}

int lipasr_mlp_train_dw0(lipasr_mlp_t m, const float* x, int batch, float* grads, lipasr_stream_t stream) {
  int rc = check_batch("lipasr_mlp_train_dw0", m, batch);
  if (rc != LIPASR_OK) return rc;
  LP_CHECK_ARG(x && grads, "lipasr_mlp_train_dw0: null argument");
  if (m->n_layers == 1) return LIPASR_OK;
  const MlpLayer& L = m->L[0];
  GemmArgs g = gemm_args(x, L.n_in, m->ws + L.offDz, L.n_out, grads + L.offW, L.n_out, L.n_in + 1, L.n_out, batch, EPI_STORE);
  g.ones_row = 1;
  g.extra_out = grads + L.offb;
  set_arith(g, m, OP_ACT, OP_GRAD, m->last_inv_batch);
  if (m->compute_bf16 == 2 && L.bn) g.sb_dyn = m->amax;
  return launch_gemm(1, 1, g, S(stream));
}

int lipasr_mlp_train_segments(lipasr_mlp_t m, int* n_segments) {
  LP_CHECK_ARG(m && n_segments, "lipasr_mlp_train_segments: null argument");
  int n = 1;
  for (int l = 0; l + 1 < m->n_layers; ++l)
    if (m->L[l].bn) n += 2;
  *n_segments = n;
  return LIPASR_OK;
}

int lipasr_mlp_train_segment_exchange(lipasr_mlp_t m, int batch, int seg, size_t* floats) {
  int rc = check_batch("lipasr_mlp_train_segment_exchange", m, batch);
  if (rc != LIPASR_OK) return rc;
  LP_CHECK_ARG(floats != nullptr && seg >= 0, "lipasr_mlp_train_segment_exchange: bad argument");
  *floats = 0;
  int cur = 0;
  for (int l = 0; l + 1 < m->n_layers; ++l)
    if (m->L[l].bn) {
      if (cur == seg) { *floats = 2 * (size_t)m->L[l].n_out; return LIPASR_OK; }
      ++cur;
// ... 101 lines not shown
  if (rc != LIPASR_OK) return rc;
  LP_CHECK_ARG(params && x_adv && x0 && y_onehot, "lipasr_mlp_attack_step: null argument");
  LP_CHECK_ARG(m->n_state == 0 || bnstate, "lipasr_mlp_attack_step: bnstate is null");
  LP_CHECK_ARG(eps >= 0.0f && !(alpha != alpha), "lipasr_mlp_attack_step: eps=%g alpha=%g", (double)eps, (double)alpha);
  return attack_common(m, params, bnstate, x_adv, y_onehot, batch, nullptr, x_adv, x0, alpha, eps, S(stream));
}

int lipasr_mlp_attack_step_lp(lipasr_mlp_t m, const float* params, const float* bnstate, float* x_adv, const float* x0,
                              const float* y_onehot, int batch, float norm, float alpha, float eps, lipasr_stream_t stream) {
  int code = 0;
  int rc = lp_norm_code("lipasr_mlp_attack_step_lp", norm, &code);
  if (rc != LIPASR_OK) return rc;
  if (code == 0) return lipasr_mlp_attack_step(m, params, bnstate, x_adv, x0, y_onehot, batch, alpha, eps, stream);
  rc = check_batch("lipasr_mlp_attack_step_lp", m, batch);
  if (rc != LIPASR_OK) return rc;
  LP_CHECK_ARG(params && x_adv && x0 && y_onehot, "lipasr_mlp_attack_step_lp: null argument");
  LP_CHECK_ARG(m->n_state == 0 || bnstate, "lipasr_mlp_attack_step_lp: bnstate is null");
  LP_CHECK_ARG(eps >= 0.0f && !(alpha != alpha), "lipasr_mlp_attack_step_lp: eps=%g alpha=%g", (double)eps, (double)alpha);
  float* g = m->ws + (((m->n_layers - 1) & 1) ? m->offG1 : m->offG0);
  rc = attack_common(m, params, bnstate, x_adv, y_onehot, batch, g, nullptr, nullptr, 0.0f, 0.0f, S(stream));
  if (rc != LIPASR_OK) return rc;
  return lp_step_launch(x_adv, x0, g, batch, m->L[0].n_in, code, alpha, eps, S(stream));
}

int lipasr_mlp_output_vjp(lipasr_mlp_t m, const float* params, const float* bnstate, const float* x, const float* v,
                          int on_logits, int batch, float* probs_out, float* dx, lipasr_stream_t stream) {
  int rc = check_batch("lipasr_mlp_output_vjp", m, batch);
  if (rc != LIPASR_OK) return rc;
  LP_CHECK_ARG(params && x && v && dx, "lipasr_mlp_output_vjp: null argument");
  LP_CHECK_ARG(m->n_state == 0 || bnstate, "lipasr_mlp_output_vjp: bnstate is null");
  hipStream_t st = S(stream);
  float* lg = m->ws + m->offLogits;
  rc = forward_infer(m, params, bnstate, x, batch, true, lg, st);
  if (rc != LIPASR_OK) return rc;
  const int C = m->L[m->n_layers - 1].n_out;
  hipLaunchKernelGGL(softmax_vjp_kernel, dim3((batch + 255) / 256), dim3(256), 0, st, lg, v, batch, C, on_logits ? 1 : 0,
                     probs_out, m->ws + m->offDzLast);
  LP_LAUNCH_CHECK();
  return backward_infer(m, params, bnstate, batch, dx, nullptr, nullptr, 0.0f, 0.0f, st);
}

int lipasr_mlp_set_gemm_tiles(lipasr_mlp_t m, int lds_min_tiles) {
  LP_CHECK_ARG(m != nullptr && lds_min_tiles >= 0, "lipasr_mlp_set_gemm_tiles: bad argument");
  m->lds_min_tiles = lds_min_tiles;
  return LIPASR_OK;
}

int lipasr_mlp_set_fuse_bn(lipasr_mlp_t m, int mode) {
  LP_CHECK_ARG(m != nullptr && (mode == 0 || mode == 1), "lipasr_mlp_set_fuse_bn: bad argument");
  m->fuse_bn = mode;
  return LIPASR_OK;
}

int lipasr_mlp_set_cu_budget(lipasr_mlp_t m, int n_cus) {
  LP_CHECK_ARG(m != nullptr && n_cus >= 0, "lipasr_mlp_set_cu_budget: bad argument");
  m->cu_budget = n_cus;
  return LIPASR_OK;
}

int lipasr_mlp_exchange_errors(lipasr_mlp_t m, int* errors_host) {
  LP_CHECK_ARG(m != nullptr && errors_host != nullptr, "lipasr_mlp_exchange_errors: null argument");
  *errors_host = 0;
  if (!m->xc_err) return LIPASR_OK;
  DeviceGuard g(m->ctx->device);
  LP_HIP(hipMemcpy(errors_host, m->xc_err, sizeof(int), hipMemcpyDeviceToHost));
  if (*errors_host) LP_HIP(hipMemset(m->xc_err, 0, sizeof(int)));
  return LIPASR_OK;
}

int lipasr_mlp_set_compute(lipasr_mlp_t m, int mode) {
  LP_CHECK_ARG(m != nullptr, "lipasr_mlp_set_compute: null plan");
  LP_CHECK_ARG(mode >= 0 && mode <= 2, "lipasr_mlp_set_compute: mode %d (0 = exact fp32, 1 = bf16 operands, 2 = fp16 two-plane split)", mode);
  if (mode == 2) {
    for (int l = 0; l + 1 < m->n_layers; ++l)
      if (!m->L[l].bn) {
        set_error("lipasr_mlp_set_compute: mode 2 (fp16 two-plane split) needs BatchNormalization after every hidden Dense layer (layer %d has none); use mode 0", l);
        return LIPASR_EUNSUPPORTED;
      }
  }
  m->compute_bf16 = mode;
  return LIPASR_OK;
}

}
```

### asr-using-robust-nn_amd/csrc/optim.hip

```cpp
#include "mlp.h"

namespace lipasr {

struct SegTable {
  int n;
  unsigned start[4 * LIPASR_MAX_LAYERS];
  unsigned char nonneg[4 * LIPASR_MAX_LAYERS];
};

__global__ __launch_bounds__(256) void adam_nonneg_kernel(float* __restrict__ w, const float* __restrict__ g,
                                                           float* __restrict__ m, float* __restrict__ v, size_t n4,
                                                           SegTable segs, const int* __restrict__ step_dev, float lr,
                                                           float b1, float b2, float eps, float gscale) {
  __shared__ float lr_t_s;
  if (threadIdx.x == 0) {
    const double t = (double)(*step_dev + 1);
    lr_t_s = (float)((double)lr * sqrt(1.0 - pow((double)b2, t)) / (1.0 - pow((double)b1, t)));
  }
  __syncthreads();
  const float lr_t = lr_t_s;
  const float ob1 = 1.0f - b1, ob2 = 1.0f - b2;
  const size_t stride = (size_t)gridDim.x * 256;
  for (size_t i = (size_t)blockIdx.x * 256 + threadIdx.x; i < n4; i += stride) {
    const unsigned e = (unsigned)(i << 2);
    int s = 0;
    while (s + 1 < segs.n && e >= segs.start[s + 1]) ++s;
    const bool nn = segs.nonneg[s] != 0;
    float4 wv = reinterpret_cast<float4*>(w)[i];
    float4 gv = reinterpret_cast<const float4*>(g)[i];
    float4 mv = reinterpret_cast<float4*>(m)[i];
    float4 vv = reinterpret_cast<float4*>(v)[i];
#define LP_ADAM1(c)                                  \
  {                                                  \
    const float gg = gv.c * gscale;                  \
    mv.c = mv.c * b1 + gg * ob1;                     \
    vv.c = vv.c * b2 + (gg * gg) * ob2;              \
    float x = wv.c - lr_t * mv.c / (sqrtf(vv.c) + eps); \
    wv.c = (nn && !(x >= 0.0f)) ? 0.0f : x;          \
  }
    LP_ADAM1(x) LP_ADAM1(y) LP_ADAM1(z) LP_ADAM1(w)
#undef LP_ADAM1
    reinterpret_cast<float4*>(w)[i] = wv;
    reinterpret_cast<float4*>(m)[i] = mv;
    reinterpret_cast<float4*>(v)[i] = vv;
  }
}

__global__ void step_inc_kernel(int* step_dev) { *step_dev += 1; }

__global__ __launch_bounds__(256) void sign_step_kernel(float* __restrict__ x_adv, const float* __restrict__ x0,
                                                         const float* __restrict__ g, size_t n, float alpha, float eps) {
  const size_t stride = (size_t)gridDim.x * 256;
  const bool noclip = isinf(eps);
  for (size_t i = (size_t)blockIdx.x * 256 + threadIdx.x; i < n; i += stride) {
    const float gv = g[i];
    const float sg = (gv > 0.0f) ? 1.0f : ((gv < 0.0f) ? -1.0f : 0.0f);
    const float xa = x_adv[i] + alpha * sg;
    const float b = x0[i];
    x_adv[i] = noclip ? xa : b + fminf(fmaxf(xa - b, -eps), eps);
  }
}

__global__ __launch_bounds__(256) void scaler_fit_kernel(const float* __restrict__ x, int n_rows, int n_feat,
                                                          double* __restrict__ mean_out, double* __restrict__ scale_out) {
  __shared__ double part[8][33];
  const int tid = threadIdx.x, cx = tid & 31, ry = tid >> 5;
  const int j = blockIdx.x * 32 + cx;
  double s = 0.0;
  if (j < n_feat)
    for (int b = ry; b < n_rows; b += 8) s += (double)x[(size_t)b * n_feat + j];
  part[ry][cx] = s;
  __syncthreads();
  double tot = 0.0;
  for (int k = 0; k < 8; ++k) tot += part[k][cx];
  const double mean = tot / (double)n_rows;
  __syncthreads();
  double q = 0.0;
  if (j < n_feat)
    for (int b = ry; b < n_rows; b += 8) {
      const double d = (double)x[(size_t)b * n_feat + j] - mean;
      q += d * d;
    }
  part[ry][cx] = q;
  __syncthreads();
  if (ry == 0 && j < n_feat) {
    double tq = 0.0;
    for (int k = 0; k < 8; ++k) tq += part[k][cx];
    const double var = tq / (double)n_rows;
    double sc = sqrt(var);
    if (sc < 10.0 * 2.220446049250313e-16 || var <= (double)n_rows * 2.220446049250313e-16 * var +
                                                        ((double)n_rows * mean * 2.220446049250313e-16) *
                                                            ((double)n_rows * mean * 2.220446049250313e-16))
      sc = 1.0;
    mean_out[j] = mean;
    scale_out[j] = sc;
  }
}

__global__ __launch_bounds__(256) void scaler_apply_kernel(const float* __restrict__ x, size_t n, int n_feat,
                                                            const double* __restrict__ mean, const double* __restrict__ scale,
                                                            float* __restrict__ out) {
  const size_t stride = (size_t)gridDim.x * 256;
  for (size_t i = (size_t)blockIdx.x * 256 + threadIdx.x; i < n; i += stride) {
    const int j = (int)(i % (size_t)n_feat);
    out[i] = (float)(((double)x[i] - mean[j]) / scale[j]);
  }
}

static int layer_arrays(lipasr_mlp_t m, float* params, float** Ws, int* rows, int* cols) {
  for (int l = 0; l < m->n_layers; ++l) {
    Ws[l] = params + m->L[l].offW;
    rows[l] = m->L[l].n_in;
    cols[l] = m->L[l].n_out;
  }
  return m->n_layers;
}

}

using namespace lipasr;

extern "C" {

static int adam_launch(lipasr_mlp_t m, float* params, const float* grads, float* adam_m, float* adam_v, int* step_dev,
                       float lr, float beta1, float beta2, float eps, float grad_scale, bool bump_step,
                       lipasr_stream_t stream) {
  LP_CHECK_ARG(m && params && grads && adam_m && adam_v && step_dev, "lipasr_mlp_adam_nonneg: null argument");
  LP_CHECK_ARG(((reinterpret_cast<uintptr_t>(params) | reinterpret_cast<uintptr_t>(grads) |
                 reinterpret_cast<uintptr_t>(adam_m) | reinterpret_cast<uintptr_t>(adam_v)) & 15) == 0,
               "lipasr_mlp_adam_nonneg: flat buffers must be 16-byte aligned");
  LP_CHECK_ARG(lr > 0.0f && beta1 >= 0.0f && beta1 < 1.0f && beta2 >= 0.0f && beta2 < 1.0f && eps >= 0.0f,
               "lipasr_mlp_adam_nonneg: bad hyper-parameters");
  SegTable segs;
  memset(&segs, 0, sizeof(segs));
  int n = 0;
  for (int l = 0; l < m->n_layers; ++l) {
    const MlpLayer& L = m->L[l];
    segs.start[n] = (unsigned)L.offW; segs.nonneg[n++] = L.nonneg ? 1 : 0;
    segs.start[n] = (unsigned)L.offb; segs.nonneg[n++] = 0;
    if (L.bn) {
      segs.start[n] = (unsigned)L.offg; segs.nonneg[n++] = 0;
      segs.start[n] = (unsigned)L.offbe; segs.nonneg[n++] = 0;
    }
  }
  segs.n = n;
  const size_t n4 = m->n_params >> 2;
  int blocks = (int)((n4 + 255) / 256);
  if (blocks > 2048) blocks = 2048;
  hipLaunchKernelGGL(adam_nonneg_kernel, dim3(blocks), dim3(256), 0, S(stream), params, grads, adam_m, adam_v, n4, segs,
                     step_dev, lr, beta1, beta2, eps, grad_scale);
  LP_LAUNCH_CHECK();
  if (bump_step) {
    hipLaunchKernelGGL(step_inc_kernel, dim3(1), dim3(1), 0, S(stream), step_dev);
    LP_LAUNCH_CHECK();
  }
  return LIPASR_OK;
}

int lipasr_mlp_adam_nonneg(lipasr_mlp_t m, float* params, const float* grads, float* adam_m, float* adam_v,
                           int* step_dev, float lr, float beta1, float beta2, float eps, float grad_scale,
                           lipasr_stream_t stream) {
  return adam_launch(m, params, grads, adam_m, adam_v, step_dev, lr, beta1, beta2, eps, grad_scale, true, stream);
}

int lipasr_mlp_adam_project_product(lipasr_mlp_t m, float* params, const float* grads, float* adam_m, float* adam_v,
                                    int* step_dev, float lr, float beta1, float beta2, float eps, float grad_scale,
                                    float rho, const int* order, int n_order, float* norms_out,
                                    lipasr_stream_t stream) {
  int rc = adam_launch(m, params, grads, adam_m, adam_v, step_dev, lr, beta1, beta2, eps, grad_scale, false, stream);
  if (rc != LIPASR_OK) return rc;
  float* Ws[LIPASR_MAX_LAYERS];
  int rows[LIPASR_MAX_LAYERS], cols[LIPASR_MAX_LAYERS];
  const int n = layer_arrays(m, params, Ws, rows, cols);
  return lipasr::project_product_bump(m->ctx, Ws, rows, cols, n, rho, order, n_order, norms_out, step_dev, stream);
}

int lipasr_sign_step(lipasr_handle_t h, float* x_adv, const float* x0, const float* g, size_t n, float alpha, float eps,
                     lipasr_stream_t stream) {
  LP_CHECK_ARG(h && x_adv && x0 && g, "lipasr_sign_step: null argument");
  LP_CHECK_ARG(eps >= 0.0f, "lipasr_sign_step: eps=%g must be non-negative", (double)eps);
  if (n == 0) return LIPASR_OK;
  int blocks = (int)((n + 255) / 256);
  if (blocks > 2048) blocks = 2048;
  hipLaunchKernelGGL(sign_step_kernel, dim3(blocks), dim3(256), 0, S(stream), x_adv, x0, g, n, alpha, eps);
  LP_LAUNCH_CHECK();
// ... 54 lines not shown
```

### asr-using-robust-nn_amd/csrc/spectral.hip

```cpp
#include "common.h"

namespace lipasr {

constexpr double kEps = 2.220446049250313e-16;
constexpr int kMaxR = 32;
constexpr int kMaxOrder = 64;
constexpr int kChainRowsPerWave = 1;
constexpr int kChainRowsPerBlock = 4 * kChainRowsPerWave;
#ifndef LIPASR_SQUARINGS
#define LIPASR_SQUARINGS 40
#endif
constexpr int kSquarings = LIPASR_SQUARINGS;
#ifndef LIPASR_SIGMA_WGS
#define LIPASR_SIGMA_WGS 192
#endif

template <int RM>
__global__ __launch_bounds__(256) void chain_step_kernel(const float* __restrict__ Pin, int p_mode,
                                                          const float* __restrict__ W, int n_rows, int n_in, int R,
                                                          float* __restrict__ Pout, int emit_gram,
                                                          double* __restrict__ gram_part) {
  extern __shared__ __attribute__((aligned(16))) char smem_raw[];
  float* Ps = reinterpret_cast<float*>(smem_raw);
  float* rowsum = Ps + (size_t)R * n_in;
// ... 304 lines not shown
      double* t = cur; cur = nxt; nxt = t;
      if (fabs(tj - 1.0) < 1e-12) break;
    }
  }
  if (tid == 0) {
    if (bump) *bump += 1;
    const double sigma = zero ? 0.0 : exp(0.5 * log_lambda);
    if (sigma_out) *sigma_out = (float)sigma;
    if (scales) {
      double sc[LIPASR_MAX_LAYERS];
      for (int l = 0; l < oa.n_layers; ++l) sc[l] = 1.0;
      double n = sigma;
      for (int v = 0; v < oa.n_order; ++v) {
        norms_out[v] = (float)n;
        const double s = root_m(rho / (n + kEps), oa.n_layers);
        sc[oa.order[v]] *= s;
        n *= s;
      }
      norms_out[oa.n_order] = (float)n;
      for (int l = 0; l < oa.n_layers; ++l) scales[l] = (float)sc[l];
    }
  }
}

struct LayerPtrs {
  int n_layers;
  float* W[LIPASR_MAX_LAYERS];
  int rows[LIPASR_MAX_LAYERS];
  int cols[LIPASR_MAX_LAYERS];
  int wg_start[LIPASR_MAX_LAYERS + 1];
};

__global__ __launch_bounds__(256) void scale_layers_kernel(LayerPtrs lp, const float* __restrict__ scales) {
  const int l = blockIdx.y;
  const float s = scales[l];
  if (s == 1.0f) return;
  float* w = lp.W[l];
  const size_t n = (size_t)lp.rows[l] * lp.cols[l];
  const size_t stride = (size_t)gridDim.x * 256;
  if ((reinterpret_cast<uintptr_t>(w) & 15) == 0) {
    const size_t n4 = n >> 2;
    float4* w4 = reinterpret_cast<float4*>(w);
    for (size_t i = (size_t)blockIdx.x * 256 + threadIdx.x; i < n4; i += stride) {
      float4 x = w4[i];
      x.x *= s; x.y *= s; x.z *= s; x.w *= s;
      w4[i] = x;
    }
    for (size_t i = (n4 << 2) + (size_t)blockIdx.x * 256 + threadIdx.x; i < n; i += stride) w[i] *= s;
  } else {
    for (size_t i = (size_t)blockIdx.x * 256 + threadIdx.x; i < n; i += stride) w[i] *= s;
  }
}

#ifndef LIPASR_SSL_THREADS
#define LIPASR_SSL_THREADS 512
#endif
constexpr int kSslThreads = LIPASR_SSL_THREADS, kSslWaves = kSslThreads / 64;
__global__ __launch_bounds__(kSslThreads) void sigma_scale_layers_kernel(const float* __restrict__ P, int n, int R, double rho, OrderArgs oa,
                                                                  LayerPtrs lp, float* __restrict__ scales_out, float* __restrict__ norms_out,
                                                                  float* __restrict__ sigma_out, int* __restrict__ bump) {
  extern __shared__ __attribute__((aligned(16))) char ssl_raw[];
  const int tid = threadIdx.x;
  const int RR = R * R, total = R * n;
  double* A = reinterpret_cast<double*>(ssl_raw);
  double* B = A + RR;
  double* gpart0 = B + RR;
  float* Ps = reinterpret_cast<float*>(gpart0 + kSslWaves * RR);
  __shared__ float sc_s[LIPASR_MAX_LAYERS];
  if ((total & 3) == 0 && (reinterpret_cast<uintptr_t>(P) & 15) == 0) {
    const float4* src = reinterpret_cast<const float4*>(P);
    float4* dst = reinterpret_cast<float4*>(Ps);
    for (int f = tid; f < (total >> 2); f += kSslThreads) dst[f] = src[f];
  } else {
    for (int f = tid; f < total; f += kSslThreads) Ps[f] = P[f];
  }
  __syncthreads();
  {
    const int w = tid >> 6, lane = tid & 63;
    const int n_ent = R * (R + 1) / 2, nq = n >> 2;
    for (int e = lane; e < n_ent; e += 64) {
      int a = 0, rem = e;
      while (rem >= R - a) { rem -= R - a; ++a; }
      const int b = a + rem;
      const float* pa = Ps + (size_t)a * n;
      const float* pb = Ps + (size_t)b * n;
      double s = 0.0;
      if ((n & 3) == 0) {
        for (int q = w; q < nq; q += kSslWaves) {
          const float4 x = *reinterpret_cast<const float4*>(pa + 4 * q), y = *reinterpret_cast<const float4*>(pb + 4 * q);
          s = fma((double)x.x, (double)y.x, s); s = fma((double)x.y, (double)y.y, s);
          s = fma((double)x.z, (double)y.z, s); s = fma((double)x.w, (double)y.w, s);
        }
      } else {
        for (int i = w; i < n; i += kSslWaves) s = fma((double)pa[i], (double)pb[i], s);
      }
      gpart0[w * RR + a * R + b] = s;
      gpart0[w * RR + b * R + a] = s;
    }
  }
  __syncthreads();
  for (int e = tid; e < RR; e += kSslThreads) {
    double part[kSslWaves];
#pragma unroll
    for (int w = 0; w < kSslWaves; ++w) part[w] = gpart0[w * RR + e];
#pragma unroll
    for (int h = kSslWaves / 2; h >= 1; h >>= 1)
#pragma unroll
      for (int w = 0; w < h; ++w) part[w] = part[2 * w] + part[2 * w + 1];
    A[e] = part[0];
  }
  __syncthreads();
  double t0 = 0.0;
  for (int a = 0; a < R; ++a) t0 += A[a * R + a];
  __syncthreads();
  __shared__ double tj_s[kSquarings + 1];
  __shared__ double ll_s;
  const bool zero = !(t0 > 0.0);
  int n_it = 0;
  if (!zero) {
    for (int e = tid; e < RR; e += kSslThreads) A[e] /= t0;
    __syncthreads();
    double* cur = A;
    double* nxt = B;
    double c2 = 1.0;
    for (int it = 0; it < kSquarings; ++it) {
      for (int e = tid; e < RR; e += kSslThreads) {
        const int a = e / R, b = e - a * R;
        double s = 0.0;
        for (int c = 0; c < R; ++c) s = fma(cur[a * R + c], cur[c * R + b], s);
        nxt[e] = s * c2;
      }
      __syncthreads();
      double tj = 0.0;
      for (int a = 0; a < R; ++a) tj += nxt[a * R + a];
      if (tid == 0) tj_s[it] = tj;
      n_it = it + 1;
      const double inv = 1.0 / tj;
      c2 = inv * inv;
      double* t = cur; cur = nxt; nxt = t;
      if (fabs(tj - 1.0) < 1e-12) break;
    }
    if (tid < 64) {
      double term = 0.0;
      if (tid < n_it) term = ldexp(log(tj_s[tid]), -(tid + 1));
      term = wave_sum_d(term);
      if (tid == 0) ll_s = log(t0) + term;
    }
    __syncthreads();
  }
  const double log_lambda = zero ? 0.0 : ll_s;
  if (tid == 0) {
    const bool first = blockIdx.x == 0;
    if (first && bump) *bump += 1;
    const double sigma = zero ? 0.0 : exp(0.5 * log_lambda);
    if (first && sigma_out) *sigma_out = (float)sigma;
    double sc[LIPASR_MAX_LAYERS];
    for (int l = 0; l < oa.n_layers; ++l) sc[l] = 1.0;
    double nrm = sigma;
    for (int v = 0; v < oa.n_order; ++v) {
      if (first) norms_out[v] = (float)nrm;
      const double s = root_m(rho / (nrm + kEps), oa.n_layers);
      sc[oa.order[v]] *= s;
      nrm *= s;
    }
    if (first) norms_out[oa.n_order] = (float)nrm;
    for (int l = 0; l < oa.n_layers; ++l) {
      sc_s[l] = (float)sc[l];
      if (first && scales_out) scales_out[l] = (float)sc[l];
    }
  }
  __syncthreads();
  int l = 0;
  while (l + 1 < lp.n_layers && (int)blockIdx.x >= lp.wg_start[l + 1]) ++l;
  const float s = sc_s[l];
  if (s == 1.0f) return;
  float* w = lp.W[l];
  const size_t nw = (size_t)lp.rows[l] * lp.cols[l];
  const size_t j = (size_t)((int)blockIdx.x - lp.wg_start[l]);
  const size_t stride = (size_t)(lp.wg_start[l + 1] - lp.wg_start[l]) * kSslThreads;
  if ((reinterpret_cast<uintptr_t>(w) & 15) == 0) {
    const size_t n4 = nw >> 2;
    float4* w4 = reinterpret_cast<float4*>(w);
    for (size_t i = j * kSslThreads + threadIdx.x; i < n4; i += stride) {
      float4 x = w4[i];
      x.x *= s; x.y *= s; x.z *= s; x.w *= s;
      w4[i] = x;
    }
    for (size_t i = (n4 << 2) + j * kSslThreads + threadIdx.x; i < nw; i += stride) w[i] *= s;
  } else {
    for (size_t i = j * kSslThreads + threadIdx.x; i < nw; i += stride) w[i] *= s;
  }
}

struct PiArgs {
  int n_layers;
  const float* W[LIPASR_MAX_LAYERS];
  int rows[LIPASR_MAX_LAYERS];
  int cols[LIPASR_MAX_LAYERS];
  float* v[LIPASR_MAX_LAYERS];
  float* u[LIPASR_MAX_LAYERS];
  int blk_u[LIPASR_MAX_LAYERS + 1];
  int blk_v[LIPASR_MAX_LAYERS + 1];
  int clamp;
};

constexpr int kPiMaxDim = 8192;

__device__ __forceinline__ int find_layer(const int* prefix, int n, int blk) {
  int l = 0;
  while (l + 1 < n && blk >= prefix[l + 1]) ++l;
  return l;
}

__device__ __forceinline__ float start_vec(int j) {
  return 1.0f + 0.001f * (float)((((unsigned)j * 2654435761u) >> 24) & 255u);
}

__device__ __forceinline__ float block_sum_256(float x, float* red) {
  x = wave_sum(x);
  const int tid = threadIdx.x;
  __syncthreads();
  if ((tid & 63) == 0) red[tid >> 6] = x;
  __syncthreads();
  return (red[0] + red[1]) + (red[2] + red[3]);
}

__global__ __launch_bounds__(256) void pi_u_kernel(PiArgs a, int cold) {
  __shared__ __attribute__((aligned(16))) float vs[kPiMaxDim];
  __shared__ float red[4];
  const int tid = threadIdx.x, lane = tid & 63, wave = tid >> 6;
  const int l = find_layer(a.blk_u, a.n_layers, blockIdx.x);
  const int rows = a.rows[l], cols = a.cols[l];
  const float* W = a.W[l];
  float ss = 0.0f;
  for (int j = tid; j < cols; j += 256) {
    const float x = cold ? start_vec(j) : a.v[l][j];
    vs[j] = x;
    ss = fmaf(x, x, ss);
  }
  const float nv2 = block_sum_256(ss, red);
  const float inv = nv2 > 0.0f ? 1.0f / sqrtf(nv2) : 0.0f;
  const bool vec = ((cols & 3) == 0) && ((reinterpret_cast<uintptr_t>(W) & 15) == 0);
  const int row0 = (blockIdx.x - a.blk_u[l]) * 8 + wave * 2;
// ... 628 lines not shown
```

### asr-using-robust-nn_amd/lipasr/_native.py

```python
from __future__ import annotations

import ctypes as C
import os

import torch

_HERE = os.path.dirname(os.path.abspath(__file__))
LIB_PATH = os.environ.get("LIPASR_LIBRARY") or os.path.join(_HERE, "liblipasr.so")

if not os.path.exists(LIB_PATH):
    raise ImportError(
        f"{LIB_PATH} not found: build it with `python asr-using-robust-nn_amd/build.py` "
        "(or __graft_entry__.build()).  lipasr has no CPU fallback."
    )

lib = C.CDLL(LIB_PATH)

OK, EINVAL, ENOMEM, EHIP, EUNSUPPORTED, ESTATE = 0, -1, -2, -3, -4, -5
MAX_LAYERS = 16
SEG_W, SEG_B, SEG_GAMMA, SEG_BETA, SEG_MMEAN, SEG_MVAR = range(6)

c_f = C.c_void_p
c_h = C.c_void_p
c_s = C.c_void_p
# ... 11 lines not shown

PROTOTYPES = {
    "lipasr_version": (i32, []),
    "lipasr_last_error": (C.c_char_p, []),
    "lipasr_create": (i32, [i32, C.POINTER(c_h)]),
    "lipasr_destroy": (i32, [c_h]),
    "lipasr_timer_create": (i32, [c_h, PI]),
    "lipasr_timer_start": (i32, [c_h, i32, c_s]),
    "lipasr_timer_stop": (i32, [c_h, i32, c_s]),
    "lipasr_timer_elapsed_ms": (i32, [c_h, i32, C.POINTER(f32)]),
    "lipasr_graph_begin": (i32, [c_h, c_s]),
    "lipasr_graph_end": (i32, [c_h, c_s, PI]),
    "lipasr_graph_launch": (i32, [c_h, i32, c_s]),
    "lipasr_stream_create_masked": (i32, [c_h, C.POINTER(C.c_uint32), i32, C.POINTER(c_s)]),
    "lipasr_stream_destroy": (i32, [c_h, c_s]),
    "lipasr_graph_destroy": (i32, [c_h, i32]),
    "lipasr_sigma_max": (i32, [c_h, c_f, i32, i32, c_f, i32, i32, i32, c_f, c_s]),
    "lipasr_project_per_layer": (i32, [c_h, PV, PI, PI, i32, f32, c_f, i32, i32, c_f, c_s]),
    "lipasr_project_product": (i32, [c_h, PV, PI, PI, i32, f32, PI, i32, c_f, c_s]),
    "lipasr_product_norm": (i32, [c_h, PV, PI, PI, i32, c_f, c_s]),
    "lipasr_frobenius_project": (i32, [c_h, c_f, sz, f32, c_s]),
    "lipasr_bn_correction": (i32, [c_h, c_f, c_f, i32, c_f, c_s]),
    "lipasr_sv_clip": (i32, [c_h, c_f, i32, i32, f32, c_f, c_f, c_s]),
    "lipasr_sign_step": (i32, [c_h, c_f, c_f, c_f, sz, f32, f32, c_s]),
    "lipasr_lp_step": (i32, [c_h, c_f, c_f, c_f, i32, i32, f32, f32, f32, c_s]),
    "lipasr_lp_ball_init": (i32, [c_h, c_f, c_f, i32, i32, f32, f32, u64, c_f, i32, c_s]),
    "lipasr_scaler_fit": (i32, [c_h, c_f, i32, i32, c_f, c_f, c_s]),
    "lipasr_scaler_apply": (i32, [c_h, c_f, i32, i32, c_f, c_f, c_f, c_s]),
    "lipasr_gemm_f32": (i32, [c_h, i32, i32, i32, i32, i32, c_f, i32, c_f, i32, c_f, i32, c_s]),
    "lipasr_gemm_f16x2": (i32, [c_h, i32, i32, i32, i32, i32, c_f, i32, c_f, i32, c_f, i32, f32, f32, c_s]),
    "lipasr_mlp_create": (i32, [c_h, i32, PI, PI, C.POINTER(f32), PI, i32, C.POINTER(c_h)]),
    "lipasr_mlp_destroy": (i32, [c_h]),
    "lipasr_mlp_sizes": (i32, [c_h, C.POINTER(sz), C.POINTER(sz)]),
    "lipasr_mlp_segment": (i32, [c_h, i32, i32, C.POINTER(sz), C.POINTER(sz)]),
    "lipasr_mlp_train_fwd_bwd": (i32, [c_h, c_f, c_f, c_f, c_f, i32, f32, C.POINTER(DropoutCfg), c_f, c_f, c_f, c_f, c_s]),
    "lipasr_mlp_train_fwd_bwd_head": (i32, [c_h, c_f, c_f, c_f, c_f, i32, f32, C.POINTER(DropoutCfg), c_f, c_f, c_f, c_f, c_s]),
    "lipasr_mlp_train_dw0": (i32, [c_h, c_f, i32, c_f, c_s]),
    "lipasr_mlp_grad_split": (i32, [c_h, C.POINTER(sz)]),
    "lipasr_mlp_train_segments": (i32, [c_h, PI]),
    "lipasr_mlp_train_segment_exchange": (i32, [c_h, i32, i32, C.POINTER(sz)]),
    "lipasr_mlp_part_floats": (i32, [c_h, C.POINTER(sz)]),
    "lipasr_mlp_train_segment": (i32, [c_h, i32, c_f, c_f, c_f, c_f, i32, f32, C.POINTER(DropoutCfg), c_f, c_f, c_f, c_f, c_f, i32, f32, c_s]),
    "lipasr_mlp_adam_nonneg": (i32, [c_h, c_f, c_f, c_f, c_f, c_f, f32, f32, f32, f32, f32, c_s]),
    "lipasr_mlp_project_product": (i32, [c_h, c_f, f32, PI, i32, c_f, c_s]),
    "lipasr_mlp_adam_project_product": (i32, [c_h, c_f, c_f, c_f, c_f, c_f, f32, f32, f32, f32, f32, f32, PI, i32, c_f, c_s]),
    "lipasr_mlp_project_per_layer": (i32, [c_h, c_f, f32, c_f, i32, i32, c_f, c_s]),
    "lipasr_mlp_product_norm": (i32, [c_h, c_f, c_f, c_s]),
    "lipasr_mlp_predict": (i32, [c_h, c_f, c_f, c_f, i32, c_f, c_f, c_s]),
    "lipasr_mlp_input_grad": (i32, [c_h, c_f, c_f, c_f, c_f, i32, c_f, c_s]),
    "lipasr_mlp_set_compute": (i32, [c_h, i32]),
    "lipasr_mlp_set_gemm_tiles": (i32, [c_h, i32]),
    "lipasr_mlp_set_fuse_bn": (i32, [c_h, i32]),
    "lipasr_mlp_set_cu_budget": (i32, [c_h, i32]),
    "lipasr_mlp_exchange_errors": (i32, [c_h, C.POINTER(C.c_int)]),
    "lipasr_mlp_output_vjp": (i32, [c_h, c_f, c_f, c_f, c_f, i32, i32, c_f, c_f, c_s]),
    "lipasr_mlp_attack_step": (i32, [c_h, c_f, c_f, c_f, c_f, c_f, i32, f32, f32, c_s]),
    "lipasr_mlp_attack_step_lp": (i32, [c_h, c_f, c_f, c_f, c_f, c_f, i32, f32, f32, f32, c_s]),
    "lipasr_mlp_own_labels": (i32, [c_h, c_f, c_f, c_f, i32, c_f, c_s]),
    "lipasr_mfcc_plan": (i32, [c_h, i32, i32, i32]),
    "lipasr_mfcc_plan_ex": (i32, [c_h, i32, i32, i32, i32, i32]),
    "lipasr_mfcc_dims": (i32, [c_h, PI, PI]),
    "lipasr_mfcc_f32": (i32, [c_h, c_f, i32, i32, c_f, c_f, c_f, c_s]),
    "lipasr_resample_f32": (i32, [c_h, c_f, i32, c_f, c_s]),
    "lipasr_mfcc_from_22k": (i32, [c_h, c_f, i32, i32, i32, c_f, c_f, c_f, c_s]),
    "lipasr_mfcc_i16": (i32, [c_h, c_f, c_f, i32, i32, c_f, c_f, c_f, c_s]),
    "lipasr_mfcc_create": (i32, [c_h, i32, i32, i32, i32, i32, C.POINTER(c_h)]),
    "lipasr_mfcc_destroy": (i32, [c_h]),
    "lipasr_mfcc_plan_dims": (i32, [c_h, PI, PI, PI]),
    "lipasr_mfcc_extract": (i32, [c_h, c_f, i32, c_f, i32, i32, c_f, c_f, c_f, c_s]),
    "lipasr_mfcc_plan_resample": (i32, [c_h, c_f, i32, c_f, c_s]),
    "lipasr_mfcc_plan_from_22k": (i32, [c_h, c_f, i32, i32, i32, c_f, c_f, c_f, c_s]),
    "lipasr_mfcc_plan_vjp": (i32, [c_h, c_f, i32, i32, i32, c_f, c_f, c_f, i32, c_s]),
    "lipasr_mfcc_plan_resample_vjp": (i32, [c_h, c_f, i32, c_f, c_s]),
    "lipasr_mfcc_plan_profile_begin": (i32, [c_h, i32]),
    "lipasr_mfcc_plan_profile_end": (i32, [c_h, C.POINTER(f32), PI]),
    "lipasr_mfcc_plan_set": (i32, [c_h, i32, i32]),
    "lipasr_mfcc_profile_begin": (i32, [c_h, i32]),
    "lipasr_mfcc_profile_end": (i32, [c_h, C.POINTER(f32), PI]),
    "lipasr_add_noise_f32": (i32, [c_h, c_f, i32, i32, i32, f32, f32, u64, c_s]),
    "lipasr_debug_set": (i32, [c_h, i32, i32]),
    "lipasr_debug_gemm_mode": (i32, [i32]),
    "lipasr_debug_launch_count": (C.c_long, [i32]),
    "lipasr_flag_signal": (i32, [c_h, C.c_void_p, i32, c_s]),
    "lipasr_flag_wait": (i32, [c_h, C.c_void_p, i32, i32, C.c_void_p, c_s]),
    "lipasr_debug_chain_head": (i32, [i32]),
    "lipasr_debug_table": (i32, [i32, i32, C.POINTER(f32), i32]),
}

for _name, (_res, _args) in PROTOTYPES.items():
    _fn = getattr(lib, _name)
    _fn.restype = _res
    _fn.argtypes = _args


if os.environ.get("LIPASR_CHAIN_HEAD"):
    lib.lipasr_debug_chain_head(int(os.environ["LIPASR_CHAIN_HEAD"]))
if os.environ.get("LIPASR_GEMM_MODE"):
    lib.lipasr_debug_gemm_mode(int(os.environ["LIPASR_GEMM_MODE"]))


def last_error() -> str:
    return (lib.lipasr_last_error() or b"").decode("utf-8", "replace")


class LipasrError(RuntimeError):
    def __init__(self, code: int, msg: str):
# ... 151 lines not shown
```

### asr-using-robust-nn_amd/lipasr/keras.py

```python
from __future__ import annotations

import ctypes as C
import math
import os
import time

import numpy as np
import torch

from . import _native as N
from . import keras_h5

_name_counts = {}


def _auto_name(prefix):
    k = _name_counts.get(prefix, 0)
    _name_counts[prefix] = k + 1
    return prefix if k == 0 else f"{prefix}_{k}"


def reset_layer_names():
    _name_counts.clear()

# ... 433 lines not shown
        elif enable and any(b["drop"] for b in self._blocks):
            cfg.mode = 1
            cfg.seed = (self._dropout_seed + 0x9E3779B97F4A7C15 * self._replica_rank) & 0xFFFFFFFFFFFFFFFF
            cfg.step_dev = self._step.data_ptr()
        else:
            cfg.mode = 0
        return cfg

    def train_fwd_bwd(self, xb, yb, inv_batch=None, masks=None, dropout=True, probs=None, defer_dw0=False):
        bsz = xb.shape[0]
        cfg = self._dropout_cfg(masks, dropout)
        inv = 1.0 / bsz if inv_batch is None else inv_batch
        fn = N.lib.lipasr_mlp_train_fwd_bwd_head if defer_dw0 else N.lib.lipasr_mlp_train_fwd_bwd
        N.check(fn(self._plan, N.ptr(self._params), N.ptr(self._bnstate), N.ptr(xb), N.ptr(yb), bsz, inv,
                   C.byref(cfg), N.ptr(self._grads), N.ptr(self._loss_rows), N.ptr(self._correct_rows),
                   N.ptr(probs), N.stream_ptr()))

    def syncbn_segments(self):
        if getattr(self, "_part", None) is None:
            n = N.sz()
            N.check(N.lib.lipasr_mlp_part_floats(self._plan, C.byref(n)))
            self._part = torch.zeros(int(n.value), device=self._device)
            ns = C.c_int()
            N.check(N.lib.lipasr_mlp_train_segments(self._plan, C.byref(ns)))
            self._n_segments = ns.value
        return self._n_segments

    def syncbn_segment(self, seg, xb, yb, global_batch, world, masks=None, dropout=True, probs=None):
        bsz = xb.shape[0]
        cfg = self._dropout_cfg(masks, dropout)
        self.syncbn_segments()
        N.check(N.lib.lipasr_mlp_train_segment(self._plan, seg, N.ptr(self._params), N.ptr(self._bnstate), N.ptr(xb), N.ptr(yb), bsz,
                                               1.0 / float(global_batch), C.byref(cfg), N.ptr(self._grads), N.ptr(self._loss_rows),
                                               N.ptr(self._correct_rows), N.ptr(probs), N.ptr(self._part), int(global_batch),
                                               1.0 / float(world), N.stream_ptr()))
        n = N.sz()
        N.check(N.lib.lipasr_mlp_train_segment_exchange(self._plan, bsz, seg, C.byref(n)))
        return int(n.value)

    def train_fwd_bwd_syncbn(self, xb, yb, dp, global_batch, masks=None, dropout=True, probs=None):
        for seg in range(self.syncbn_segments()):
            n = self.syncbn_segment(seg, xb, yb, global_batch, dp.world, masks=masks, dropout=dropout, probs=probs)
            if n:
                dp.allreduce_grads(self._part[:n])

    def train_dw0(self, xb):
        N.check(N.lib.lipasr_mlp_train_dw0(self._plan, N.ptr(xb), xb.shape[0], N.ptr(self._grads), N.stream_ptr()))

    @property
    def late_floats(self):
        n = N.sz()
        N.check(N.lib.lipasr_mlp_grad_split(self._plan, C.byref(n)))
        return int(n.value)

    def apply_adam(self, grad_scale=1.0):
        lr, b1, b2, eps = self._adam
        N.check(N.lib.lipasr_mlp_adam_nonneg(self._plan, N.ptr(self._params), N.ptr(self._grads), N.ptr(self._adam_m), N.ptr(self._adam_v),
                                             N.ptr(self._step), lr, b1, b2, eps, grad_scale, N.stream_ptr()))

    def apply_adam_project_product(self, rho, order, norms_out, grad_scale=1.0):
        lr, b1, b2, eps = self._adam
        N.check(N.lib.lipasr_mlp_adam_project_product(self._plan, N.ptr(self._params), N.ptr(self._grads), N.ptr(self._adam_m),
                                                      N.ptr(self._adam_v), N.ptr(self._step), lr, b1, b2, eps, grad_scale, float(rho), order,
                                                      len(order), N.ptr(norms_out), N.stream_ptr()))

    def train_on_batch(self, xb, yb, masks=None, dropout=True):
        if self._dp is not None:
            self._dp.train_step(self, xb, yb, masks=masks, dropout=dropout)
            return
        self.train_fwd_bwd(xb, yb, masks=masks, dropout=dropout)
        self.apply_adam()

    def fit(self, x, y=None, epochs=1, batch_size=32, validation_data=None, verbose=1, callbacks=None):
        if not self._compiled:
            raise RuntimeError("call compile() before fit()")
        ds = x if isinstance(x, Dataset) else Dataset(x, y, batch_size)
        if ds.batch_size is None:
            ds = ds.batch(batch_size)
        if ds.batch_size > self._max_batch:
            raise ValueError(f"batch {ds.batch_size} exceeds the plan's max_batch {self._max_batch}")
        xs, ys = ds.materialize(self._device)
        val = None
        if validation_data is not None:
            vd = validation_data if isinstance(validation_data, Dataset) else Dataset(validation_data[0], validation_data[1], ds.batch_size)
            val = vd.materialize(self._device)
        callbacks = list(callbacks or [])
        for cb in callbacks:
            cb.set_model(self) if hasattr(cb, "set_model") else setattr(cb, "model", self)
        for cb in callbacks:
            cb.on_train_begin()
        self.stop_training = False
        history = {"loss": [], "accuracy": []}
        n, bs = xs.shape[0], ds.batch_size
        for epoch in range(epochs):
            t0 = time.time()
            for cb in callbacks:
                cb.on_epoch_begin(epoch)
            loss_sum = torch.zeros((), device=self._device)
            acc_sum = torch.zeros((), device=self._device)
            for bi, s in enumerate(range(0, n, bs)):
                xb, yb = xs[s:s + bs], ys[s:s + bs]
                self.train_on_batch(xb, yb)
                k = xb.shape[0]
                loss_sum += self._loss_rows[:k].sum()
                acc_sum += self._correct_rows[:k].sum()
                for cb in callbacks:
# ... 216 lines not shown
```

### asr-using-robust-nn_amd/lipasr/pipeline.py

```python
from __future__ import annotations

import ctypes as C

import torch

from . import _native as N
from .extract_features_construct_dataset import MfccExtractor
from .parallel import DataParallel


class TrainPipeline:
    def __init__(self, model, batch, sr_in=16000, n_samp=16000, utterance_length=44, rho=0.1, constraint="product",
                 affine=None, pgd=None, dp=None, use_graph="auto", per_layer_iters=4, extractor=None, mfcc_cus="auto",
                 sync_inputs=True, overlap_buckets=False, sync_bn=False, train_cus="auto"):
        self.sync_inputs = bool(sync_inputs)
        if pgd:
            from .attacks import _norm_value

            self._pgd_norm = _norm_value(pgd.get("norm", float("inf")))
            rinit = int(pgd.get("num_random_init", 0))
            if rinit not in (0, 1):
                raise ValueError(f"pgd num_random_init={rinit}: 0 or 1 (more restarts inside training are not supported)")
            self._pgd_rinit = rinit == 1
            self._pgd_seed = (0xBA11000000000000 + int(model._seed)) & 0xFFFFFFFFFFFFFFFF
        self._train_cus = train_cus
        self.overlap_buckets = bool(overlap_buckets)
        self.model, self.batch, self.L = model, int(batch), int(utterance_length)
        self.dev = model._device
        self.h = N.get_handle(self.dev.index)
        self.ex = MfccExtractor(sr_in, n_samp, self.batch, self.dev) if extractor is None else extractor
        self._custom_ex = extractor is not None
        self.rho, self.constraint, self.pgd = float(rho), constraint, pgd
        self.dp = dp if dp is not None else DataParallel()
        model._replica_rank = self.dp.rank
        self._late = model.late_floats
        self.sync_bn = bool(sync_bn) and self.dp.world > 1
        self.use_graph = (bool(pgd) or self.sync_bn) if use_graph == "auto" else bool(use_graph)
        self.per_layer_iters = per_layer_iters
        self.mean, self.scale = affine if affine is not None else (None, None)
        nf = 20 * self.L
        if model._widths[0] != nf:
            raise ValueError(f"model input width {model._widths[0]} != {nf}")
        self._nbuf = 2
        self._feats2 = [torch.zeros(self.batch, nf, device=self.dev) for _ in range(self._nbuf)]
        self._labels2 = [torch.zeros(self.batch, model._n_classes, device=self.dev) for _ in range(self._nbuf)]
        self.feats, self.labels = self._feats2[0], self._labels2[0]
        self.x_adv = torch.zeros(self.batch, nf, device=self.dev) if pgd else None
        nl = len(model._blocks)
        self.norms = torch.zeros(nl + 1, device=self.dev)
        self.sigmas = torch.zeros(nl, device=self.dev)
        self.v_state = torch.zeros(sum(model._widths[1:]), device=self.dev)
        self._order = N.int_array(list(range(nl)))
        self._warm = False
        self._masked_stream = self._masked_train_stream = None
        self._gemm_tiles_set = False
        self.stream = torch.cuda.Stream(device=self.dev)
        self.mfcc_stream = self._make_mfcc_stream(mfcc_cus)
        import os as _os

        self._wide_stream = torch.cuda.Stream(device=self.dev) if (self._masked_stream is not None and not self._custom_ex
                                                                  and _os.environ.get("LIPASR_WIDE_WHEN_IDLE", "1") == "1") else None
        self._ev_last_mfcc = None
        self._last_xs = None
        self._last_train_ev = None
        self._n_cu = torch.cuda.get_device_properties(self.dev).multi_processor_count
        self._flags = None
        self._flag_err = None
        want_flags = _os.environ.get("LIPASR_GPU_FLAGS", "auto")
# ... 75 lines not shown
    def _own_queue_train_stream(self, n_cu):
        import os

        if os.environ.get("LIPASR_TRAIN_OWN_QUEUE", "1") != "1":
            return
        words = (n_cu + 31) // 32
        mask2 = (C.c_uint32 * words)()
        for b in range(n_cu):
            mask2[b // 32] |= 1 << (b % 32)
        st2 = N.c_s()
        if N.lib.lipasr_stream_create_masked(self.h.h, mask2, words, C.byref(st2)) == N.OK:
            self._masked_train_stream = st2
            self.stream = torch.cuda.ExternalStream(st2.value, device=self.dev)

    def _check_flags(self):
        fe = self._flag_err
        if fe is None:
            return
        code = int(fe[0])
        if code:
            fe[0] = 0
            self._failed = True
            what = ("is overdue (it is still waiting: nothing ran out of order)" if code == 1
                    else "gave up: what its stream did afterwards was not ordered against the other stream")
            raise RuntimeError(f"TrainPipeline: a device-side wait between the extraction and the classifier stream {what} "
                               f"after {self._flag_timeout_ms} ms without the other stream's signal; LIPASR_GPU_FLAGS=0 uses events")

    def _pgd_loop(self, bsz, x, y):
        m = self.model
        eps, eps_step = float(self.pgd["eps"]), float(self.pgd.get("eps_step", 0.1))
        xa = self.x_adv[:bsz]
        if self._pgd_rinit:
            N.check(N.lib.lipasr_lp_ball_init(self.h.h, N.ptr(xa), N.ptr(x), bsz, xa.shape[1], self._pgd_norm, eps, self._pgd_seed,
                                              N.ptr(m._step), self.dp.rank, N.stream_ptr()))
        else:
            xa.copy_(x)
        for _ in range(int(self.pgd.get("max_iter", 20))):
            if self._pgd_norm == float("inf"):
                N.check(N.lib.lipasr_mlp_attack_step(m._plan, N.ptr(m._params), N.ptr(m._bnstate), N.ptr(xa), N.ptr(x), N.ptr(y), bsz,
                                                     eps_step, eps, N.stream_ptr()))
            else:
                N.check(N.lib.lipasr_mlp_attack_step_lp(m._plan, N.ptr(m._params), N.ptr(m._bnstate), N.ptr(xa), N.ptr(x), N.ptr(y), bsz,
                                                        self._pgd_norm, eps_step, eps, N.stream_ptr()))
        return xa

    def _attack_and_train(self, bsz, b, global_batch, defer_dw0=False):
        m = self.model
        x = self._feats2[b][:bsz]
        y = self._labels2[b][:bsz]
        if self.pgd:
            x = self._pgd_loop(bsz, x, y)
        m.train_fwd_bwd(x, y, inv_batch=1.0 / float(global_batch), defer_dw0=defer_dw0)

    def _attack_only(self, bsz, b):
        x = self._feats2[b][:bsz]
        if not self.pgd:
            return x
        return self._pgd_loop(bsz, x, self._labels2[b][:bsz])

    def _syncbn_step(self, bsz, b, gb):
        m = self.model
        n_seg = m.syncbn_segments()
        y = self._labels2[b][:bsz]
        xin = (self.x_adv if self.pgd else self._feats2[b])[:bsz]
        if not self.use_graph:
            self._attack_only(bsz, b)
            for seg in range(n_seg):
                n = m.syncbn_segment(seg, xin, y, gb, self.dp.world)
                if n:
                    self.dp.allreduce_grads(m._part[:n])
            self.dp.allreduce_grads(m._grads)
            self._update()
            return
        key = (bsz, b, gb, "syncbn")
        g = self._graphs.get(key)
        if g is None:
            counts = []

            def first():
                self._attack_only(bsz, b)
                counts.append(m.syncbn_segment(0, xin, y, gb, self.dp.world))

            ids = [self._capture(first)]
            for seg in range(1, n_seg):
                ids.append(self._capture(lambda s=seg: counts.append(m.syncbn_segment(s, xin, y, gb, self.dp.world))))
            ids.append(self._capture(self._update))
            self._sync_counts = getattr(self, "_sync_counts", {})
            self._sync_counts[key] = counts
            g = tuple(ids)
            self._graphs[key] = g
        counts = self._sync_counts[key]
        for seg in range(n_seg):
            N.check(N.lib.lipasr_graph_launch(self.h.h, g[seg], N.stream_ptr()))
            if counts[seg]:
                self.dp.allreduce_grads(m._part[:counts[seg]])
        self.dp.allreduce_grads(m._grads)
        N.check(N.lib.lipasr_graph_launch(self.h.h, g[n_seg], N.stream_ptr()))

    def _dw0(self, bsz, b):
        self.model.train_dw0((self.x_adv if self.pgd else self._feats2[b])[:bsz])

    def _reduce_and_update_eager(self, bsz, b):
        m = self.model
        late = self._late
        ha = self.dp.allreduce_async(m._grads[late:])
        self._dw0(bsz, b)
# ... 60 lines not shown
        if wide:
            xs = self._wide_stream
            self.ex.set(1, self._n_cu)
        if self.sync_inputs:
            xs.wait_stream(caller)
        with torch.cuda.stream(xs):
            if self._flags is not None:
                if self._last_xs is not None and self._last_xs is not xs:
                    xs.wait_stream(self._last_xs)
                self._last_xs = xs
            elif self._ev_last_mfcc is not None and self._wide_stream is not None:
                xs.wait_event(self._ev_last_mfcc)
            if self._flags is not None:
                fl = self._flags
                if self._i > self._nbuf:
                    N.check(N.lib.lipasr_flag_wait(self.h.h, fl[self._nbuf + b:].data_ptr(), self._i - self._nbuf, self._flag_timeout_ms, self._flag_err.data_ptr(), N.stream_ptr()))
            elif self._ev_free[b] is not None:
                xs.wait_event(self._ev_free[b])
            if features is not None:
                self._feats2[b][:bsz].copy_(features)
            else:
                if self._custom_ex:
                    self.ex(waves, self.mean, self.scale, out=self._feats2[b][:bsz])
                else:
                    self.ex(waves, self.L, self.mean, self.scale, out=self._feats2[b][:bsz])
            self._labels2[b][:bsz].copy_(y_onehot)
            if self._flags is not None:
                N.check(N.lib.lipasr_flag_signal(self.h.h, self._flags[b:].data_ptr(), self._i, N.stream_ptr()))
            else:
                self._ev_feat[b].record(xs)
                self._ev_last_mfcc = self._ev_feat[b]
        if wide:
            self.ex.set(1, self.mfcc_cus)
        if self.sync_inputs:
            if self._flags is not None:
                caller.wait_stream(xs)
            else:
                caller.wait_event(self._ev_feat[b])
        with torch.cuda.stream(self.stream):
            self._warm_start()
            if self._flags is not None:
                N.check(N.lib.lipasr_flag_wait(self.h.h, self._flags[b:].data_ptr(), self._i, self._flag_timeout_ms, self._flag_err.data_ptr(), N.stream_ptr()))
            else:
                self.stream.wait_event(self._ev_feat[b])
            prof = None
            if getattr(self, "_prof", None) is not None and self._prof_i < len(self._prof):
                prof = self._prof[self._prof_i]
                self._prof_i += 1
                prof[0].record(self.stream)
            if self.sync_bn:
                self._syncbn_step(bsz, b, gb)
            elif not self.use_graph:
                if self.dp.world == 1:
                    self._attack_and_train(bsz, b, gb)
                    self._update()
                elif self.overlap_buckets:
                    self._attack_and_train(bsz, b, gb, defer_dw0=True)
                    self._reduce_and_update_eager(bsz, b)
                else:
                    self._attack_and_train(bsz, b, gb)
                    self.dp.allreduce_grads(self.model._grads)
                    self._update()
            else:
                g = self._graphs.get((bsz, b, gb))
                if g is None:
                    if self.dp.world == 1:
                        g = (self._capture(lambda: (self._attack_and_train(bsz, b, gb), self._update())),)
                    elif self.overlap_buckets:
                        g = (self._capture(self._attack_and_train, bsz, b, gb, True), self._capture(self._dw0, bsz, b),
                             self._capture(self._update))
                    else:
                        g = (self._capture(self._attack_and_train, bsz, b, gb), self._capture(self._update))
                    self._graphs[(bsz, b, gb)] = g
                N.check(N.lib.lipasr_graph_launch(self.h.h, g[0], N.stream_ptr()))
                if len(g) == 3:
                    late = self._late
                    ha = self.dp.allreduce_async(self.model._grads[late:])
                    N.check(N.lib.lipasr_graph_launch(self.h.h, g[1], N.stream_ptr()))
                    hb = self.dp.allreduce_async(self.model._grads[:late])
                    ha.wait()
                    hb.wait()
                    N.check(N.lib.lipasr_graph_launch(self.h.h, g[2], N.stream_ptr()))
                elif len(g) == 2:
                    self.dp.allreduce_grads(self.model._grads)
                    N.check(N.lib.lipasr_graph_launch(self.h.h, g[1], N.stream_ptr()))
            if prof is not None:
                prof[1].record(self.stream)
            if self._flags is not None:
                N.check(N.lib.lipasr_flag_signal(self.h.h, self._flags[self._nbuf + b:].data_ptr(), self._i, N.stream_ptr()))
            else:
                ev = torch.cuda.Event()
                ev.record(self.stream)
                self._ev_free[b] = ev
                self._last_train_ev = ev

    def synchronize(self):
        if getattr(self, "_wide_stream", None) is not None:
            self._wide_stream.synchronize()
        self.mfcc_stream.synchronize()
        self.stream.synchronize()
        self._check_flags()
        if self.model.exchange_errors():
            raise RuntimeError("TrainPipeline: a BatchNorm exchange inside a GEMM gave up after 2 s (workgroups of one column block were never "
                               "resident together: is the plan's CU budget larger than its stream's CU mask?); the step's results are invalid. "
                               "LIPASR_FUSE_BN=0 uses the launch chain")

    @property
    def mfcc_stream_kind(self):
        return "masked" if self._masked_stream is not None else "shared"

    def close(self):
        if getattr(self, "_closed", True):
            return
        if N._capture_depth > 0:
            N._deferred.append((self.close, ()))
            return
        self._closed = True
        if not self.h.alive:
            self._graphs.clear()
            self._masked_stream = self._masked_train_stream = None
# ... 36 lines not shown
```

### include/lipasr.h

```cpp
#ifndef LIPASR_H
#define LIPASR_H

#include <stddef.h>
#include <stdint.h>

#ifdef __cplusplus
extern "C" {
#endif

#define LIPASR_OK            0
#define LIPASR_EINVAL       -1
#define LIPASR_ENOMEM       -2
#define LIPASR_EHIP         -3
#define LIPASR_EUNSUPPORTED -4
#define LIPASR_ESTATE       -5

#define LIPASR_MAX_LAYERS   16
#define LIPASR_N_MFCC       20
#define LIPASR_N_MELS       128
#define LIPASR_N_FFT        2048
#define LIPASR_HOP          512
#define LIPASR_SR           22050

typedef struct lipasr_ctx* lipasr_handle_t;
// ... 58 lines not shown
int lipasr_scaler_apply(lipasr_handle_t h, const float* x, int n_rows, int n_feat, const double* mean,
                        const double* scale, float* out, lipasr_stream_t stream);

int lipasr_gemm_f32(lipasr_handle_t h, int transA, int transB, int M, int N, int K, const float* A,
                    int lda, const float* B, int ldb, float* C, int ldc, lipasr_stream_t stream);

int lipasr_gemm_f16x2(lipasr_handle_t h, int transA, int transB, int M, int N, int K, const float* A, int lda,
                      const float* B, int ldb, float* C, int ldc, float scale_a, float scale_b, lipasr_stream_t stream);

#define LIPASR_SEG_W      0
#define LIPASR_SEG_B      1
#define LIPASR_SEG_GAMMA  2
#define LIPASR_SEG_BETA   3
#define LIPASR_SEG_MMEAN  4
#define LIPASR_SEG_MVAR   5

int lipasr_mlp_create(lipasr_handle_t h, int n_layers, const int* widths, const int* bn,
                      const float* dropout, const int* nonneg, int max_batch, lipasr_mlp_t* out);
int lipasr_mlp_destroy(lipasr_mlp_t m);
int lipasr_mlp_sizes(lipasr_mlp_t m, size_t* n_params, size_t* n_state);
int lipasr_mlp_segment(lipasr_mlp_t m, int layer, int kind, size_t* offset, size_t* count);

typedef struct lipasr_dropout_cfg {
  int mode;
  uint64_t seed;
  const int* step_dev;
  const float* const* masks;
} lipasr_dropout_cfg;

int lipasr_mlp_train_fwd_bwd(lipasr_mlp_t m, const float* params, float* bnstate, const float* x,
                             const float* y_onehot, int batch, float inv_batch,
                             const lipasr_dropout_cfg* dropout, float* grads, float* loss_rows,
                             float* correct_rows, float* probs, lipasr_stream_t stream);

int lipasr_mlp_train_fwd_bwd_head(lipasr_mlp_t m, const float* params, float* bnstate, const float* x,
                                  const float* y_onehot, int batch, float inv_batch,
                                  const lipasr_dropout_cfg* dropout, float* grads, float* loss_rows,
                                  float* correct_rows, float* probs, lipasr_stream_t stream);
int lipasr_mlp_train_dw0(lipasr_mlp_t m, const float* x, int batch, float* grads, lipasr_stream_t stream);
int lipasr_mlp_grad_split(lipasr_mlp_t m, size_t* late_floats);

int lipasr_mlp_train_segments(lipasr_mlp_t m, int* n_segments);
int lipasr_mlp_train_segment_exchange(lipasr_mlp_t m, int batch, int seg, size_t* floats);
int lipasr_mlp_part_floats(lipasr_mlp_t m, size_t* floats);
int lipasr_mlp_train_segment(lipasr_mlp_t m, int seg, const float* params, float* bnstate, const float* x,
                             const float* y_onehot, int batch, float inv_batch,
                             const lipasr_dropout_cfg* dropout, float* grads, float* loss_rows,
                             float* correct_rows, float* probs, float* part, int stat_batch,
                             float stat_grad_scale, lipasr_stream_t stream);

int lipasr_mlp_adam_nonneg(lipasr_mlp_t m, float* params, const float* grads, float* adam_m,
                           float* adam_v, int* step_dev, float lr, float beta1, float beta2, float eps,
                           float grad_scale, lipasr_stream_t stream);

int lipasr_mlp_adam_project_product(lipasr_mlp_t m, float* params, const float* grads, float* adam_m,
                                    float* adam_v, int* step_dev, float lr, float beta1, float beta2,
                                    float eps, float grad_scale, float rho, const int* order,
                                    int n_order, float* norms_out, lipasr_stream_t stream);
int lipasr_mlp_project_product(lipasr_mlp_t m, float* params, float rho, const int* order, int n_order,
                               float* norms_out, lipasr_stream_t stream);
int lipasr_mlp_project_per_layer(lipasr_mlp_t m, float* params, float rho, float* v_state, int warm,
                                 int iters, float* sigmas_out, lipasr_stream_t stream);
int lipasr_mlp_product_norm(lipasr_mlp_t m, const float* params, float* sigma_out, lipasr_stream_t stream);

int lipasr_mlp_set_compute(lipasr_mlp_t m, int mode);

int lipasr_mlp_set_gemm_tiles(lipasr_mlp_t m, int lds_min_tiles);

int lipasr_mlp_set_fuse_bn(lipasr_mlp_t m, int mode);
int lipasr_mlp_set_cu_budget(lipasr_mlp_t m, int n_cus);
int lipasr_mlp_exchange_errors(lipasr_mlp_t m, int* errors_host);

int lipasr_mlp_predict(lipasr_mlp_t m, const float* params, const float* bnstate, const float* x,
                       int batch, float* probs, float* logits, lipasr_stream_t stream);

int lipasr_mlp_input_grad(lipasr_mlp_t m, const float* params, const float* bnstate, const float* x,
                          const float* y_onehot, int batch, float* dx, lipasr_stream_t stream);

int lipasr_mlp_output_vjp(lipasr_mlp_t m, const float* params, const float* bnstate, const float* x,
                          const float* v, int on_logits, int batch, float* probs_out, float* dx,
                          lipasr_stream_t stream);

int lipasr_mlp_attack_step(lipasr_mlp_t m, const float* params, const float* bnstate, float* x_adv,
                           const float* x0, const float* y_onehot, int batch, float alpha, float eps,
                           lipasr_stream_t stream);

int lipasr_mlp_attack_step_lp(lipasr_mlp_t m, const float* params, const float* bnstate, float* x_adv, const float* x0,
                              const float* y_onehot, int batch, float norm, float alpha, float eps, lipasr_stream_t stream);

int lipasr_mlp_own_labels(lipasr_mlp_t m, const float* params, const float* bnstate, const float* x,
                          int batch, float* y_onehot_out, lipasr_stream_t stream);

int lipasr_mfcc_plan(lipasr_handle_t h, int sr_in, int n_samp, int batch_max);
int lipasr_mfcc_plan_ex(lipasr_handle_t h, int sr_in, int n_samp, int batch_max, int n_fft, int hop);
int lipasr_mfcc_dims(lipasr_handle_t h, int* n_y, int* n_frames);

int lipasr_mfcc_f32(lipasr_handle_t h, const float* wav, int batch, int utterance_length,
                    const double* affine_mean, const double* affine_scale, float* out,
                    lipasr_stream_t stream);
int lipasr_resample_f32(lipasr_handle_t h, const float* wav, int batch, float* y, lipasr_stream_t stream);
int lipasr_mfcc_from_22k(lipasr_handle_t h, const float* y, int batch, int n_y, int utterance_length,
                         const double* affine_mean, const double* affine_scale, float* out,
                         lipasr_stream_t stream);

int lipasr_mfcc_i16(lipasr_handle_t h, const int16_t* pcm, const int* n_valid, int batch,
                    int utterance_length, const double* affine_mean, const double* affine_scale,
// ... 43 lines not shown
```

Before: 3.070 million utterances/sec.

## Fuse Adam+NonNeg weight update into weight-gradient GEMM epilogues

Adds an optional fused path where the grouped weight-gradient GEMM kernels apply the Adam+NonNeg update to weights, m and v right in their epilogue, as each gradient tile is written. Leftover elementwise parameters such as biases are handled by extra blocks appended to the same grouped launch. The goal is to remove the separate optimizer pass that re-reads gradients, weights and moment buffers, plus its kernel launch. The cost is extra global traffic and register pressure in the GEMM epilogues, more complex kernels, and a stateful on/off mode set around the 1-GPU train step. The projection kernel is also restructured to prefetch weights before it computes the scale.

```diff
diff --git a/asr-using-robust-nn_amd/build.py b/asr-using-robust-nn_amd/build.py
--- a/asr-using-robust-nn_amd/build.py
+++ b/asr-using-robust-nn_amd/build.py
@@ -8,7 +8,7 @@
 CSRC = os.path.join(HERE, "csrc")
 OUT = os.path.join(HERE, "lipasr", "liblipasr.so")
 SOURCES = ["core.hip", "spectral.hip", "gemm.hip", "mlp.hip", "optim.hip", "mfcc.hip", "mfcc_vjp.hip", "stft_bdft.hip", "lp_attack.hip"]
-HEADERS = ["common.h", "mlp.h", "gemm.h", "mfcc_tables.h", "stft.h", os.path.join("..", "..", "include", "lipasr.h")]
+HEADERS = ["common.h", "mlp.h", "gemm.h", "adam.h", "mfcc_tables.h", "stft.h", os.path.join("..", "..", "include", "lipasr.h")]
 EXTRA = {"stft_bdft.hip": ["-fno-slp-vectorize"]}
 FLAGS = ["-O3", "--offload-arch=gfx950", "-fPIC", "-std=c++17", "-Wall", "-Wno-unused-function",
          "-fgpu-rdc" if False else "-fno-gpu-rdc"]
diff --git a/asr-using-robust-nn_amd/csrc/adam.h b/asr-using-robust-nn_amd/csrc/adam.h
--- /dev/null
+++ b/asr-using-robust-nn_amd/csrc/adam.h
@@ -0,0 +1,22 @@
+#pragma once
+#include <hip/hip_runtime.h>
+
+namespace lipasr {
+
+__device__ __forceinline__ float adam_lr_t(const int* __restrict__ step_dev, float lr, float b1, float b2) {
+  const double t = (double)(*step_dev + 1);
+  return (float)((double)lr * sqrt(1.0 - pow((double)b2, t)) / (1.0 - pow((double)b1, t)));
+}
+
+__device__ __forceinline__ void adam_nonneg_elem(float& w, float& m, float& v, const float g, const float gscale, const float lr_t,
+                                                 const float b1, const float ob1, const float b2, const float ob2, const float eps,
+                                                 const bool nn) {
+#pragma clang fp contract(off)
+  const float gg = g * gscale;
+  m = fmaf(gg, ob1, m * b1);
+  v = fmaf(gg * gg, ob2, v * b2);
+  const float x = w - lr_t * m / (sqrtf(v) + eps);
+  w = (nn && !(x >= 0.0f)) ? 0.0f : x;
+}
+
+}
diff --git a/asr-using-robust-nn_amd/csrc/gemm.h b/asr-using-robust-nn_amd/csrc/gemm.h
--- a/asr-using-robust-nn_amd/csrc/gemm.h
+++ b/asr-using-robust-nn_amd/csrc/gemm.h
@@ -109,10 +109,35 @@
 }
 
 constexpr int kMaxGroup = 8;
+
+constexpr int kFusedEwMax = 2 * kMaxGroup;
+struct FusedAdam {
+  float* w;
+  float* m;
+  float* v;
+  const float* g0;
+  const int* step_dev;
+  float lr, b1, b2, eps;
+  unsigned nonneg;
+  int ew_n, ew_block0;
+  unsigned ew_off[kFusedEwMax], ew_cnt[kFusedEwMax];
+  int ew_blk[kFusedEwMax + 1];
+};
+constexpr int kFusedEwPerBlock = 1024;
+
 struct GemmGroup {
   int n;
   int tile_start[kMaxGroup + 1];
   GemmArgs g[kMaxGroup];
+  FusedAdam fu;
+};
+
+struct FusedUpdate {
+  float* w; float* m; float* v; const float* g0; const int* step_dev;
+  float lr, b1, b2, eps;
+  const unsigned char* nonneg;
+  int ew_n;
+  unsigned ew_off[kFusedEwMax], ew_cnt[kFusedEwMax];
 };
 
 struct GemmKnobs {
@@ -138,7 +163,7 @@
 
 int pick_gemm(int amode, int bmode, const GemmArgs& g, GemmPick* out);
 int launch_gemm(int amode, int bmode, const GemmArgs& g, hipStream_t st);
-int launch_gemm_group_tn(const GemmArgs* gs, int n, hipStream_t st);
+int launch_gemm_group_tn(const GemmArgs* gs, int n, hipStream_t st, const FusedUpdate* fused = nullptr);
 GemmArgs gemm_args(const float* A, int lda, const float* B, int ldb, float* C, int ldc, int M, int N, int K, int epi);
 int gemm_row_tiles(int amode, int bmode, const GemmArgs& g);
 bool exchange_fits(int bmode, int arith, int M, int N, int K, int lds_min_tiles, int xc_rt_max, int cus);
diff --git a/asr-using-robust-nn_amd/csrc/gemm.hip b/asr-using-robust-nn_amd/csrc/gemm.hip
--- a/asr-using-robust-nn_amd/csrc/gemm.hip
+++ b/asr-using-robust-nn_amd/csrc/gemm.hip
@@ -1,4 +1,5 @@
 #include "gemm.h"
+#include "adam.h"
 #include <cstdint>
 #include <map>
 #include <mutex>
@@ -9,6 +10,51 @@
 
 typedef float f32x16 __attribute__((ext_vector_type(16)));
 typedef __bf16 bf16x8 __attribute__((ext_vector_type(8)));
+
+struct FuseCtx {
+  const FusedAdam* fu;
+  bool on;
+  bool nn;
+};
+__device__ __forceinline__ void fused_adam1(const FusedAdam& fu, const float lr_t, const bool nn, const float* gp, const float gval) {
+  const size_t i = (size_t)(gp - fu.g0);
+  float w = fu.w[i], m = fu.m[i], v = fu.v[i];
+  adam_nonneg_elem(w, m, v, gval, 1.0f, lr_t, fu.b1, 1.0f - fu.b1, fu.b2, 1.0f - fu.b2, fu.eps, nn);
+  fu.w[i] = w;
+  fu.m[i] = m;
+  fu.v[i] = v;
+}
+__device__ __forceinline__ void fused_adam4(const FusedAdam& fu, const float lr_t, const bool nn, const float* gp, const float (&gval)[4]) {
+  const size_t i = (size_t)(gp - fu.g0);
+  float4 w = *reinterpret_cast<const float4*>(fu.w + i), m = *reinterpret_cast<const float4*>(fu.m + i), v = *reinterpret_cast<const float4*>(fu.v + i);
+  const float ob1 = 1.0f - fu.b1, ob2 = 1.0f - fu.b2;
+  adam_nonneg_elem(w.x, m.x, v.x, gval[0], 1.0f, lr_t, fu.b1, ob1, fu.b2, ob2, fu.eps, nn);
+  adam_nonneg_elem(w.y, m.y, v.y, gval[1], 1.0f, lr_t, fu.b1, ob1, fu.b2, ob2, fu.eps, nn);
+  adam_nonneg_elem(w.z, m.z, v.z, gval[2], 1.0f, lr_t, fu.b1, ob1, fu.b2, ob2, fu.eps, nn);
+  adam_nonneg_elem(w.w, m.w, v.w, gval[3], 1.0f, lr_t, fu.b1, ob1, fu.b2, ob2, fu.eps, nn);
+  *reinterpret_cast<float4*>(fu.w + i) = w;
+  *reinterpret_cast<float4*>(fu.m + i) = m;
+  *reinterpret_cast<float4*>(fu.v + i) = v;
+}
+__device__ __forceinline__ bool fused_elementwise(const FusedAdam& fu) {
+  if (!fu.w || (int)blockIdx.x < fu.ew_block0) return false;
+  if (threadIdx.x >= kFusedEwPerBlock / 4) return true;
+  const int b = (int)blockIdx.x - fu.ew_block0;
+  int k = 0;
+  while (k + 1 < fu.ew_n && b >= fu.ew_blk[k + 1]) ++k;
+  const unsigned e = (unsigned)(b - fu.ew_blk[k]) * kFusedEwPerBlock + threadIdx.x * 4u, cnt = fu.ew_cnt[k];
+  if (e >= cnt) return true;
+  const float lr_t = adam_lr_t(fu.step_dev, fu.lr, fu.b1, fu.b2);
+  const float* gp = fu.g0 + fu.ew_off[k] + e;
+  if (e + 3 < cnt) {
+    const float4 gv = *reinterpret_cast<const float4*>(gp);
+    const float g4[4] = {gv.x, gv.y, gv.z, gv.w};
+    fused_adam4(fu, lr_t, false, gp, g4);
+  } else {
+    for (unsigned q = 0; e + q < cnt; ++q) fused_adam1(fu, lr_t, false, gp + q, gp[q]);
+  }
+  return true;
+}
 
 __device__ __forceinline__ bf16x8 to_bf16x8(const float (&v)[8]) {
   bf16x8 o;
@@ -374,8 +420,9 @@
   by = grp * h + (u - bx * hg);
 }
 
-template <int AMODE, int BMODE, int NW, int BF, bool X = false>
-__device__ __forceinline__ void gemm_tile(const GemmArgs& g, const int bx, const int by, const int n_row_tiles) {
+template <int AMODE, int BMODE, int NW, int BF, bool X = false, bool FU = false>
+__device__ __forceinline__ void gemm_tile(const GemmArgs& g, const int bx, const int by, const int n_row_tiles,
+                                          const FuseCtx fz = FuseCtx{nullptr, false, false}) {
   constexpr int TS = 32;
   constexpr int TPR = 8;
   extern __shared__ __attribute__((aligned(16))) float red[];
@@ -511,6 +558,9 @@
   float cs1[4] = {0.f, 0.f, 0.f, 0.f}, cs2[4] = {0.f, 0.f, 0.f, 0.f};
   if (tid < 256) {
     const int step = g.drop.step_dev ? *g.drop.step_dev : 0;
+    float lr_t = 0.0f;
+    if constexpr (FU) { if (fz.on) lr_t = adam_lr_t(fz.fu->step_dev, fz.fu->lr, fz.fu->b1, fz.fu->b2); }
+    (void)lr_t;
     const int tcol = tid & 7, row = tid >> 3;
     const int c4 = tcol * 4;
     const int gn = n0 + c4;
@@ -586,12 +636,25 @@
       float* crow;
       if (g.ones_row && gm == g.M - 1) crow = g.extra_out;
       else crow = (g.epi == EPI_SIGNSTEP ? g.x_adv : g.C) + (size_t)gm * g.ldc;
-      if (gn + 3 < g.N && ((g.ldc & 3) == 0) && ((reinterpret_cast<uintptr_t>(crow) & 15) == 0)) {
+      const bool vec4 = gn + 3 < g.N && ((g.ldc & 3) == 0) && ((reinterpret_cast<uintptr_t>(crow) & 15) == 0);
+      if (vec4) {
         *reinterpret_cast<float4*>(crow + gn) = make_float4(o[0], o[1], o[2], o[3]);
       } else {
 #pragma unroll
         for (int e = 0; e < 4; ++e)
           if (gn + e < g.N) crow[gn + e] = o[e];
+      }
+      if constexpr (FU) {
+        if (fz.on) {
+          const bool nn = fz.nn && !(g.ones_row && gm == g.M - 1);
+          if (vec4) {
+            fused_adam4(*fz.fu, lr_t, nn, crow + gn, o);
+          } else {
+#pragma unroll
+            for (int e = 0; e < 4; ++e)
+              if (gn + e < g.N) fused_adam1(*fz.fu, lr_t, nn, crow + gn + e, o[e]);
+          }
+        }
       }
     }
   }
@@ -635,6 +698,7 @@
 
 template <int AMODE, int BMODE, int NW, int BF = 0>
 __global__ __launch_bounds__(64 * NW) void gemm_f32_grouped_kernel(GemmGroup grp) {
+  if (fused_elementwise(grp.fu)) return;
   int p = 0;
   while (p + 1 < grp.n && (int)blockIdx.x >= grp.tile_start[p + 1]) ++p;
   const GemmArgs& g = grp.g[p];
@@ -642,7 +706,7 @@
   const int ntx = (g.N + 31) / 32, nty = (g.M + 31) / 32;
   int bx = local % ntx, by = local / ntx;
   if (g.xcd_map && (grp.tile_start[p] & 7) == 0) xcd_tile(local, ntx, nty, bx, by);
-  gemm_tile<AMODE, BMODE, NW, BF>(g, bx, by, nty);
+  gemm_tile<AMODE, BMODE, NW, BF, false, true>(g, bx, by, nty, FuseCtx{&grp.fu, grp.fu.w != nullptr, ((grp.fu.nonneg >> p) & 1u) != 0});
 }
 
 constexpr int kLdsBK = 32, kLdsLD = 68;
@@ -702,9 +766,9 @@
   return ((size_t)(2 * 2 * bk * kLdsLD > 2 * 64 * 64 ? 2 * 2 * bk * kLdsLD : 2 * 64 * 64) + 8 * 16 * 8) * sizeof(float);
 }
 
-template <bool X>
+template <bool X, bool FU = false>
 __device__ __forceinline__ void lds_tile_epilogue(const GemmArgs& g, const f32x16& acc, float* lds, float* stat, const int bx, const int by,
-                                                  const int n_row_tiles, const unsigned xtag) {
+                                                  const int n_row_tiles, const unsigned xtag, const FuseCtx fz = FuseCtx{nullptr, false, false}) {
   constexpr int TS = 64;
   const int tid = threadIdx.x, lane = tid & 63, wave = tid >> 6;
   const int r = lane & 31, h = lane >> 5;
@@ -794,6 +858,9 @@
     return;
   }
   float cs1[4] = {0.f, 0.f, 0.f, 0.f}, cs2[4] = {0.f, 0.f, 0.f, 0.f};
+  float lr_t = 0.0f;
+  if constexpr (FU) { if (fz.on) lr_t = adam_lr_t(fz.fu->step_dev, fz.fu->lr, fz.fu->b1, fz.fu->b2); }
+  (void)lr_t;
 #pragma unroll
   for (int pass = 0; pass < 2; ++pass) {
     const int row = trow + 32 * pass;
@@ -814,12 +881,25 @@
       float* crow;
       if (g.ones_row && gm == g.M - 1) crow = g.extra_out;
       else crow = (g.epi == EPI_SIGNSTEP ? g.x_adv : g.C) + (size_t)gm * g.ldc;
-      if (gn + 3 < g.N && ((g.ldc & 3) == 0) && ((reinterpret_cast<uintptr_t>(crow) & 15) == 0)) {
+      const bool vec4 = gn + 3 < g.N && ((g.ldc & 3) == 0) && ((reinterpret_cast<uintptr_t>(crow) & 15) == 0);
+      if (vec4) {
         *reinterpret_cast<float4*>(crow + gn) = make_float4(o[0], o[1], o[2], o[3]);
       } else {
 #pragma unroll
         for (int e = 0; e < 4; ++e)
           if (gn + e < g.N) crow[gn + e] = o[e];
+      }
+      if constexpr (FU) {
+        if (fz.on) {
+          const bool nn = fz.nn && !(g.ones_row && gm == g.M - 1);
+          if (vec4) {
+            fused_adam4(*fz.fu, lr_t, nn, crow + gn, o);
+          } else {
+#pragma unroll
+            for (int e = 0; e < 4; ++e)
+              if (gn + e < g.N) fused_adam1(*fz.fu, lr_t, nn, crow + gn + e, o[e]);
+          }
+        }
       }
     }
   }
@@ -849,8 +929,8 @@
 }
 
 
-template <int AMODE, int BMODE, int BF, int BK, bool X = false>
-__device__ __forceinline__ void gemm_lds_tile(const GemmArgs& g, const int bx, const int by, const int n_row_tiles) {
+template <int AMODE, int BMODE, int BF, int BK, bool X = false, bool FU = false>
+__device__ __forceinline__ void gemm_lds_tile(const GemmArgs& g, const int bx, const int by, const int n_row_tiles, const FuseCtx fz = FuseCtx{nullptr, false, false}) {
   constexpr int TS = 64;
   constexpr int NF = BK / kLdsBK;
   extern __shared__ __attribute__((aligned(16))) float lds[];
@@ -927,7 +1007,7 @@
 #pragma unroll
     for (int q = 0; q < 16; ++q) acc[q] *= un;
   }
-  lds_tile_epilogue<X>(g, acc, lds, stat, bx, by, n_row_tiles, xtag);
+  lds_tile_epilogue<X, FU>(g, acc, lds, stat, bx, by, n_row_tiles, xtag, fz);
 }
 
 
@@ -973,8 +1053,8 @@
   }
 }
 
-template <int AMODE, int BMODE, bool X = false, int NL = 0>
-__device__ __forceinline__ void gemm_ring_tile(const GemmArgs& g, const int bx, const int by, const int n_row_tiles) {
+template <int AMODE, int BMODE, bool X = false, int NL = 0, bool FU = false>
+__device__ __forceinline__ void gemm_ring_tile(const GemmArgs& g, const int bx, const int by, const int n_row_tiles, const FuseCtx fz = FuseCtx{nullptr, false, false}) {
   constexpr int TS = 64, S = kRingStages;
   extern __shared__ __attribute__((aligned(16))) float lds[];
   float* stat = lds + S * 2 * kRingTile;
@@ -1085,7 +1165,7 @@
     for (int q = 0; q < 16; ++q) acc[q] *= un;
   }
   __syncthreads();
-  lds_tile_epilogue<X>(g, acc, lds, stat, bx, by, n_row_tiles, xtag);
+  lds_tile_epilogue<X, FU>(g, acc, lds, stat, bx, by, n_row_tiles, xtag, fz);
 }
 
 #ifndef LIPASR_RING_LOADERS
@@ -1115,6 +1195,7 @@
 
 template <int AMODE, int BMODE, int BF = 0>
 __global__ __launch_bounds__(512) void gemm_lds_grouped_kernel(GemmGroup grp) {
+  if (fused_elementwise(grp.fu)) return;
   int p = 0;
   while (p + 1 < grp.n && (int)blockIdx.x >= grp.tile_start[p + 1]) ++p;
   const GemmArgs& g = grp.g[p];
@@ -1122,7 +1203,7 @@
   const int ntx = (g.N + 63) / 64, nty = (g.M + 63) / 64;
   int bx = local % ntx, by = local / ntx;
   if (g.xcd_map && (grp.tile_start[p] & 7) == 0) xcd_tile(local, ntx, nty, bx, by);
-  gemm_lds_tile<AMODE, BMODE, BF, kLdsBKMax>(g, bx, by, nty);
+  gemm_lds_tile<AMODE, BMODE, BF, kLdsBKMax, false, true>(g, bx, by, nty, FuseCtx{&grp.fu, grp.fu.w != nullptr, ((grp.fu.nonneg >> p) & 1u) != 0});
 }
 
 
@@ -1130,7 +1211,71 @@
 constexpr int kR128Tile = 32 * 128;
 constexpr size_t ring128_bytes() { return (size_t)(kR128Stages * 2 * kR128Tile) * sizeof(float); }
 
-__device__ __forceinline__ void gemm_ring128_tile(const GemmArgs& g, const int bx, const int by) {
+struct R128Chunk { float w[8], m[8], v[8]; };
+__device__ __forceinline__ float* r128_row(const GemmArgs& g, const int gm) {
+  return (g.ones_row && gm == g.M - 1) ? g.extra_out : g.C + (size_t)gm * g.ldc;
+}
+__device__ __forceinline__ void r128_chunk_load(const GemmArgs& g, const FusedAdam& fu, const int c, const int gm_base, const int gn0, R128Chunk& k) {
+#pragma unroll
+  for (int j = 0; j < 4; ++j) {
+    const int gm = gm_base + j + 8 * c;
+    const bool row = gm < g.M;
+    const size_t i = row ? (size_t)(r128_row(g, gm) - fu.g0) + gn0 : 0;
+#pragma unroll
+    for (int u = 0; u < 2; ++u) {
+      const bool ok = row && gn0 + 32 * u < g.N;
+      k.w[2 * j + u] = ok ? fu.w[i + 32 * u] : 0.0f;
+      k.m[2 * j + u] = ok ? fu.m[i + 32 * u] : 0.0f;
+      k.v[2 * j + u] = ok ? fu.v[i + 32 * u] : 0.0f;
+    }
+  }
+}
+__device__ __forceinline__ void r128_epilogue(const GemmArgs& g, const f32x16& acc0, const f32x16& acc1, const float un, const int gm_base,
+                                              const int gn0, const FuseCtx fz, const float lr_t, const R128Chunk& pre) {
+  if (!fz.on) {
+#pragma unroll
+    for (int q = 0; q < 16; ++q) {
+      const int gm = gm_base + (q & 3) + 8 * (q >> 2);
+      if (gm >= g.M) continue;
+      float* crow = r128_row(g, gm);
+      if (gn0 < g.N) crow[gn0] = acc0[q] * un;
+      if (gn0 + 32 < g.N) crow[gn0 + 32] = acc1[q] * un;
+    }
+    return;
+  }
+  const FusedAdam& fu = *fz.fu;
+  const float ob1 = 1.0f - fu.b1, ob2 = 1.0f - fu.b2;
+  auto update = [&](const int c, R128Chunk& k) {
+#pragma unroll
+    for (int j = 0; j < 4; ++j) {
+      const int q = 4 * c + j, gm = gm_base + j + 8 * c;
+      if (gm >= g.M) continue;
+      float* crow = r128_row(g, gm);
+      const bool nn = fz.nn && !(g.ones_row && gm == g.M - 1);
+      const size_t i = (size_t)(crow - fu.g0) + gn0;
+#pragma unroll
+      for (int u = 0; u < 2; ++u) {
+        if (gn0 + 32 * u >= g.N) continue;
+        const float gv = (u ? acc1[q] : acc0[q]) * un;
+        crow[gn0 + 32 * u] = gv;
+        adam_nonneg_elem(k.w[2 * j + u], k.m[2 * j + u], k.v[2 * j + u], gv, 1.0f, lr_t, fu.b1, ob1, fu.b2, ob2, fu.eps, nn);
+        fu.w[i + 32 * u] = k.w[2 * j + u];
+        fu.m[i + 32 * u] = k.m[2 * j + u];
+        fu.v[i + 32 * u] = k.v[2 * j + u];
+      }
+    }
+  };
+  R128Chunk a = pre, b;
+  r128_chunk_load(g, fu, 1, gm_base, gn0, b);
+  update(0, a);
+  r128_chunk_load(g, fu, 2, gm_base, gn0, a);
+  update(1, b);
+  r128_chunk_load(g, fu, 3, gm_base, gn0, b);
+  update(2, a);
+  update(3, b);
+}
+
+__device__ __forceinline__ void gemm_ring128_tile(const GemmArgs& g, const int bx, const int by, const FuseCtx fz) {
   constexpr int TS = 128, S = kR128Stages;
   extern __shared__ __attribute__((aligned(16))) float lds[];
   const int tid = threadIdx.x, lane = tid & 63;
@@ -1207,15 +1352,14 @@
   if (rsa == 1.0f) k_loop(std::true_type{});
   else k_loop(std::false_type{});
   const float un = 1.0f / (rsa * rsb);
-  const int gn0 = n0 + 64 * cj + r, gn1 = gn0 + 32;
-#pragma unroll
-  for (int q = 0; q < 16; ++q) {
-    const int gm = m0 + 32 * ri + (q & 3) + 8 * (q >> 2) + 4 * hh;
-    if (gm >= g.M) continue;
-    float* crow = (g.ones_row && gm == g.M - 1) ? g.extra_out : g.C + (size_t)gm * g.ldc;
-    if (gn0 < g.N) crow[gn0] = acc0[q] * un;
-    if (gn1 < g.N) crow[gn1] = acc1[q] * un;
-  }
+  const int gn0 = n0 + 64 * cj + r, gm_base = m0 + 32 * ri + 4 * hh;
+  float lr_t = 0.0f;
+  R128Chunk first;
+  if (fz.on) {
+    lr_t = adam_lr_t(fz.fu->step_dev, fz.fu->lr, fz.fu->b1, fz.fu->b2);
+    r128_chunk_load(g, *fz.fu, 0, gm_base, gn0, first);
+  }
+  r128_epilogue(g, acc0, acc1, un, gm_base, gn0, fz, lr_t, first);
 }
 
 #ifndef LIPASR_R128_LOADERS
@@ -1225,7 +1369,7 @@
 constexpr int kR128PlaneBytes = 128 * 64;
 constexpr size_t ring128s_bytes() { return ring128_bytes() + (size_t)2 * 4 * kR128PlaneBytes; }
 
-__device__ __forceinline__ void gemm_ring128s_tile(const GemmArgs& g, const int bx, const int by) {
+__device__ __forceinline__ void gemm_ring128s_tile(const GemmArgs& g, const int bx, const int by, const FuseCtx fz) {
   constexpr int TS = 128, S = kR128Stages;
   extern __shared__ __attribute__((aligned(16))) float lds[];
   char* const planes = reinterpret_cast<char*>(lds) + ring128_bytes();
@@ -1268,6 +1412,8 @@
       }
     };
     for (int t = 0; t < min(2, nst); ++t) issue(t);
+    float lr_t = 0.0f;
+    if (fz.on && L == 0) lr_t = adam_lr_t(fz.fu->step_dev, fz.fu->lr, fz.fu->b1, fz.fu->b2);
     for (int t = 0; t <= nst; ++t) {
       if (t < nst) {
         if (t + 1 < nst) asm volatile("s_waitcnt vmcnt(%0)" ::"n"(NQ) : "memory");
@@ -1282,6 +1428,10 @@
       if (t + 2 < nst) issue(t + 2);
 #endif
     }
+    if (fz.on) {
+      if (L == 0 && lane == 0) lds[0] = lr_t;
+      __syncthreads();
+    }
     return;
   }
   const int si = 64 * (wave & 1) + lane, sc = wave >> 1;
@@ -1296,6 +1446,9 @@
   f32x16 acc0, acc1;
 #pragma unroll
   for (int q = 0; q < 16; ++q) { acc0[q] = 0.0f; acc1[q] = 0.0f; }
+  const int gn0 = n0 + 64 * cj + r, gm_base = m0 + 32 * ri + 4 * hh;
+  R128Chunk pre;
+  if (fz.on) r128_chunk_load(g, *fz.fu, 0, gm_base, gn0, pre);
   auto k_loop = [&](auto unit_a) {
     constexpr bool UA = decltype(unit_a)::value;
     for (int t = 0; t <= nst; ++t) {
@@ -1342,18 +1495,16 @@
   if (rsa == 1.0f) k_loop(std::true_type{});
   else k_loop(std::false_type{});
   const float un = 1.0f / (rsa * rsb);
-  const int gn0 = n0 + 64 * cj + r, gn1 = gn0 + 32;
-#pragma unroll
-  for (int q = 0; q < 16; ++q) {
-    const int gm = m0 + 32 * ri + (q & 3) + 8 * (q >> 2) + 4 * hh;
-    if (gm >= g.M) continue;
-    float* crow = (g.ones_row && gm == g.M - 1) ? g.extra_out : g.C + (size_t)gm * g.ldc;
-    if (gn0 < g.N) crow[gn0] = acc0[q] * un;
-    if (gn1 < g.N) crow[gn1] = acc1[q] * un;
-  }
+  float lr_t = 0.0f;
+  if (fz.on) {
+    __syncthreads();
+    lr_t = lds[0];
+  }
+  r128_epilogue(g, acc0, acc1, un, gm_base, gn0, fz, lr_t, pre);
 }
 
 __global__ __launch_bounds__(512 + 64 * kR128Loaders) void gemm_ring_grouped_kernel(GemmGroup grp) {
+  if (fused_elementwise(grp.fu)) return;
   int p = 0;
   while (p + 1 < grp.n && (int)blockIdx.x >= grp.tile_start[p + 1]) ++p;
   const GemmArgs& g = grp.g[p];
@@ -1362,11 +1513,12 @@
   const int ntx = (g.N + ts - 1) / ts, nty = (g.M + ts - 1) / ts;
   int bx = local % ntx, by = local / ntx;
   if (g.xcd_map && (grp.tile_start[p] & 7) == 0) xcd_tile(local, ntx, nty, bx, by);
-  if (g.ring == 2) { gemm_ring128s_tile(g, bx, by); return; }
+  const FuseCtx fz{&grp.fu, grp.fu.w != nullptr, ((grp.fu.nonneg >> p) & 1u) != 0};
+  if (g.ring == 2) { gemm_ring128s_tile(g, bx, by, fz); return; }
   if (threadIdx.x >= 512) return;
-  if (g.ring == 3) gemm_ring128_tile(g, bx, by);
-  else if (g.ring) gemm_ring_tile<1, 1>(g, bx, by, nty);
-  else gemm_lds_tile<1, 1, 2, kLdsBKMax>(g, bx, by, nty);
+  if (g.ring == 3) gemm_ring128_tile(g, bx, by, fz);
+  else if (g.ring) gemm_ring_tile<1, 1, false, 0, true>(g, bx, by, nty, fz);
+  else gemm_lds_tile<1, 1, 2, kLdsBKMax, false, true>(g, bx, by, nty, fz);
 }
 
 constexpr int kR2TileA = 128 * 32, kR2TileB = 64 * 32;
@@ -1758,7 +1910,7 @@
   return per > 0 && tiles <= (long)per * cus;
 }
 
-int launch_gemm_group_tn(const GemmArgs* gs, int n, hipStream_t st) {
+int launch_gemm_group_tn(const GemmArgs* gs, int n, hipStream_t st, const FusedUpdate* fused) {
   int done = 0;
   while (done < n) {
     GemmGroup grp;
@@ -1789,6 +1941,25 @@
     }
     grp.n = k;
     grp.tile_start[k] = tiles;
+    int grid = tiles;
+    if (fused) {
+      FusedAdam& fu = grp.fu;
+      fu.w = fused->w; fu.m = fused->m; fu.v = fused->v; fu.g0 = fused->g0; fu.step_dev = fused->step_dev;
+      fu.lr = fused->lr; fu.b1 = fused->b1; fu.b2 = fused->b2; fu.eps = fused->eps;
+      for (int q = 0; q < k; ++q)
+        if (fused->nonneg[done + q]) fu.nonneg |= 1u << q;
+      fu.ew_block0 = tiles;
+      if (done == 0) {
+        fu.ew_n = fused->ew_n;
+        for (int q = 0; q < fused->ew_n; ++q) {
+          fu.ew_off[q] = fused->ew_off[q];
+          fu.ew_cnt[q] = fused->ew_cnt[q];
+          fu.ew_blk[q] = grid - tiles;
+          grid += (int)((fused->ew_cnt[q] + kFusedEwPerBlock - 1) / kFusedEwPerBlock);
+        }
+        fu.ew_blk[fused->ew_n] = grid - tiles;
+      }
+    }
     const GemmTable& t = gemm_table();
     const void* fn = lds_tiles ? t.grouped_lds[arith_index(ar)] : t.grouped_frag[arith_index(ar)];
     int threads = lds_tiles ? 512 : 256;
@@ -1805,7 +1976,7 @@
     }
     (void)ensure_dyn_lds(fn, lds);
     void* args[] = {&grp};
-    (void)hipLaunchKernel(fn, dim3(tiles), dim3(threads), args, lds, st);
+    (void)hipLaunchKernel(fn, dim3(grid), dim3(threads), args, lds, st);
     LP_LAUNCH_CHECK();
     done += k;
   }
diff --git a/asr-using-robust-nn_amd/csrc/mlp.h b/asr-using-robust-nn_amd/csrc/mlp.h
--- a/asr-using-robust-nn_amd/csrc/mlp.h
+++ b/asr-using-robust-nn_amd/csrc/mlp.h
@@ -43,4 +43,12 @@
   int* xc_err = nullptr;
   size_t xc_gran_off[2][LIPASR_MAX_LAYERS] = {};
   size_t xc_ctrl_off[2][LIPASR_MAX_LAYERS] = {};
+  int fused_on = 0;
+  float fu_lr = 0.f, fu_b1 = 0.f, fu_b2 = 0.f, fu_eps = 0.f;
+  float* fu_m = nullptr;
+  float* fu_v = nullptr;
+  int* fu_step = nullptr;
+  float* fu_params = nullptr;
+  const float* fu_grads = nullptr;
+  int fused_pending = 0;
 };
diff --git a/asr-using-robust-nn_amd/csrc/mlp.hip b/asr-using-robust-nn_amd/csrc/mlp.hip
--- a/asr-using-robust-nn_amd/csrc/mlp.hip
+++ b/asr-using-robust-nn_amd/csrc/mlp.hip
@@ -709,6 +709,28 @@
   }
   if (!LP_ON) return LIPASR_OK;
 #undef LP_ON
+  m->fused_pending = 0;
+  if (m->fused_on && dw_mode == 0 && sa.seg < 0) {
+    LP_CHECK_ARG(((reinterpret_cast<uintptr_t>(params) | reinterpret_cast<uintptr_t>(grads)) & 15) == 0,
+                 "lipasr_mlp_train_fwd_bwd: the fused update needs 16-byte aligned params and grads");
+    FusedUpdate fu;
+    memset(&fu, 0, sizeof(fu));
+    unsigned char nn[LIPASR_MAX_LAYERS];
+    fu.w = const_cast<float*>(params); fu.m = m->fu_m; fu.v = m->fu_v; fu.g0 = grads; fu.step_dev = m->fu_step;
+    fu.lr = m->fu_lr; fu.b1 = m->fu_b1; fu.b2 = m->fu_b2; fu.eps = m->fu_eps;
+    for (int l = 0; l < Lc; ++l) {
+      const MlpLayer& L = m->L[l];
+      nn[l] = L.nonneg ? 1 : 0;
+      if (L.bn) {
+        fu.ew_off[fu.ew_n] = (unsigned)L.offg; fu.ew_cnt[fu.ew_n++] = (unsigned)L.n_out;
+        fu.ew_off[fu.ew_n] = (unsigned)L.offbe; fu.ew_cnt[fu.ew_n++] = (unsigned)L.n_out;
+      }
+    }
+    fu.nonneg = nn;
+    rc = launch_gemm_group_tn(gw, Lc, st, &fu);
+    if (rc == LIPASR_OK) { m->fused_pending = 1; m->fu_params = fu.w; m->fu_grads = grads; }
+    return rc;
+  }
   if (dw_mode == 0 || Lc == 1) return launch_gemm_group_tn(gw, Lc, st);
   rc = launch_gemm_group_tn(gw + 1, Lc - 1, st);
   if (rc != LIPASR_OK || dw_mode == 2) return rc;
@@ -916,6 +938,38 @@
   return LIPASR_OK;
 }
 
+int lipasr_mlp_set_fused_update(lipasr_mlp_t m, int on, float lr, float beta1, float beta2, float eps, float* adam_m, float* adam_v,
+                                int* step_dev) {
+  LP_CHECK_ARG(m, "lipasr_mlp_set_fused_update: null plan");
+  if (!on) {
+    LP_CHECK_ARG(!m->fused_pending, "lipasr_mlp_set_fused_update: an in-place update is waiting for its Adam call");
+    m->fused_on = 0;
+    return LIPASR_OK;
+  }
+  LP_CHECK_ARG(adam_m && adam_v && step_dev, "lipasr_mlp_set_fused_update: null argument");
+  LP_CHECK_ARG(((reinterpret_cast<uintptr_t>(adam_m) | reinterpret_cast<uintptr_t>(adam_v)) & 15) == 0,
+               "lipasr_mlp_set_fused_update: flat buffers must be 16-byte aligned");
+  LP_CHECK_ARG(lr > 0.0f && beta1 >= 0.0f && beta1 < 1.0f && beta2 >= 0.0f && beta2 < 1.0f && eps >= 0.0f,
+               "lipasr_mlp_set_fused_update: bad hyper-parameters");
+  int n_bn = 0;
+  for (int l = 0; l < m->n_layers; ++l) n_bn += m->L[l].bn ? 1 : 0;
+  if (2 * n_bn > kFusedEwMax) {
+    set_error("lipasr_mlp_set_fused_update: %d BatchNorm layers; the fused launch carries at most %d", n_bn, kFusedEwMax / 2);
+    return LIPASR_EUNSUPPORTED;
+  }
+  m->fu_lr = lr; m->fu_b1 = beta1; m->fu_b2 = beta2; m->fu_eps = eps;
+  m->fu_m = adam_m; m->fu_v = adam_v; m->fu_step = step_dev;
+  m->fused_on = 1;
+  return LIPASR_OK;
+}
+
+int lipasr_mlp_fused_update_state(lipasr_mlp_t m, int* on, int* pending) {
+  LP_CHECK_ARG(m, "lipasr_mlp_fused_update_state: null plan");
+  if (on) *on = m->fused_on;
+  if (pending) *pending = m->fused_pending;
+  return LIPASR_OK;
+}
+
 int lipasr_mlp_set_cu_budget(lipasr_mlp_t m, int n_cus) {
   LP_CHECK_ARG(m != nullptr && n_cus >= 0, "lipasr_mlp_set_cu_budget: bad argument");
   m->cu_budget = n_cus;
diff --git a/asr-using-robust-nn_amd/csrc/optim.hip b/asr-using-robust-nn_amd/csrc/optim.hip
--- a/asr-using-robust-nn_amd/csrc/optim.hip
+++ b/asr-using-robust-nn_amd/csrc/optim.hip
@@ -1,4 +1,5 @@
 #include "mlp.h"
+#include "adam.h"
 
 namespace lipasr {
 
@@ -13,10 +14,7 @@
                                                            SegTable segs, const int* __restrict__ step_dev, float lr,
                                                            float b1, float b2, float eps, float gscale) {
   __shared__ float lr_t_s;
-  if (threadIdx.x == 0) {
-    const double t = (double)(*step_dev + 1);
-    lr_t_s = (float)((double)lr * sqrt(1.0 - pow((double)b2, t)) / (1.0 - pow((double)b1, t)));
-  }
+  if (threadIdx.x == 0) lr_t_s = adam_lr_t(step_dev, lr, b1, b2);
   __syncthreads();
   const float lr_t = lr_t_s;
   const float ob1 = 1.0f - b1, ob2 = 1.0f - b2;
@@ -30,16 +28,10 @@
     float4 gv = reinterpret_cast<const float4*>(g)[i];
     float4 mv = reinterpret_cast<float4*>(m)[i];
     float4 vv = reinterpret_cast<float4*>(v)[i];
-#define LP_ADAM1(c)                                  \
-  {                                                  \
-    const float gg = gv.c * gscale;                  \
-    mv.c = mv.c * b1 + gg * ob1;                     \
-    vv.c = vv.c * b2 + (gg * gg) * ob2;              \
-    float x = wv.c - lr_t * mv.c / (sqrtf(vv.c) + eps); \
-    wv.c = (nn && !(x >= 0.0f)) ? 0.0f : x;          \
-  }
-    LP_ADAM1(x) LP_ADAM1(y) LP_ADAM1(z) LP_ADAM1(w)
-#undef LP_ADAM1
+    adam_nonneg_elem(wv.x, mv.x, vv.x, gv.x, gscale, lr_t, b1, ob1, b2, ob2, eps, nn);
+    adam_nonneg_elem(wv.y, mv.y, vv.y, gv.y, gscale, lr_t, b1, ob1, b2, ob2, eps, nn);
+    adam_nonneg_elem(wv.z, mv.z, vv.z, gv.z, gscale, lr_t, b1, ob1, b2, ob2, eps, nn);
+    adam_nonneg_elem(wv.w, mv.w, vv.w, gv.w, gscale, lr_t, b1, ob1, b2, ob2, eps, nn);
     reinterpret_cast<float4*>(w)[i] = wv;
     reinterpret_cast<float4*>(m)[i] = mv;
     reinterpret_cast<float4*>(v)[i] = vv;
@@ -131,6 +123,17 @@
                "lipasr_mlp_adam_nonneg: flat buffers must be 16-byte aligned");
   LP_CHECK_ARG(lr > 0.0f && beta1 >= 0.0f && beta1 < 1.0f && beta2 >= 0.0f && beta2 < 1.0f && eps >= 0.0f,
                "lipasr_mlp_adam_nonneg: bad hyper-parameters");
+  if (m->fused_pending) {
+    LP_CHECK_ARG(params == m->fu_params && grads == m->fu_grads && adam_m == m->fu_m && adam_v == m->fu_v && step_dev == m->fu_step &&
+                     lr == m->fu_lr && beta1 == m->fu_b1 && beta2 == m->fu_b2 && eps == m->fu_eps && grad_scale == 1.0f,
+                 "lipasr_mlp_adam_nonneg: the fused update already applied these gradients (other buffers, hyper-parameters or grad_scale != 1)");
+    m->fused_pending = 0;
+    if (bump_step) {
+      hipLaunchKernelGGL(step_inc_kernel, dim3(1), dim3(1), 0, S(stream), step_dev);
+      LP_LAUNCH_CHECK();
+    }
+    return LIPASR_OK;
+  }
   SegTable segs;
   memset(&segs, 0, sizeof(segs));
   int n = 0;
diff --git a/asr-using-robust-nn_amd/csrc/spectral.hip b/asr-using-robust-nn_amd/csrc/spectral.hip
--- a/asr-using-robust-nn_amd/csrc/spectral.hip
+++ b/asr-using-robust-nn_amd/csrc/spectral.hip
@@ -380,6 +380,12 @@
   }
 }
 
+__device__ __forceinline__ void ssl_wave_sync() {
+  __builtin_amdgcn_fence(__ATOMIC_RELEASE, "workgroup");
+  __builtin_amdgcn_wave_barrier();
+  __builtin_amdgcn_fence(__ATOMIC_ACQUIRE, "workgroup");
+}
+constexpr int kSslPre = 4;
 #ifndef LIPASR_SSL_THREADS
 #define LIPASR_SSL_THREADS 512
 #endif
@@ -395,6 +401,21 @@
   double* gpart0 = B + RR;
   float* Ps = reinterpret_cast<float*>(gpart0 + kSslWaves * RR);
   __shared__ float sc_s[LIPASR_MAX_LAYERS];
+  int l = 0;
+  while (l + 1 < lp.n_layers && (int)blockIdx.x >= lp.wg_start[l + 1]) ++l;
+  float* w = lp.W[l];
+  const size_t nw = (size_t)lp.rows[l] * lp.cols[l];
+  const size_t i0 = (size_t)((int)blockIdx.x - lp.wg_start[l]) * kSslThreads + threadIdx.x;
+  const size_t stride = (size_t)(lp.wg_start[l + 1] - lp.wg_start[l]) * kSslThreads;
+  const bool w_vec = (reinterpret_cast<uintptr_t>(w) & 15) == 0;
+  const size_t n4 = nw >> 2;
+  float4* w4 = reinterpret_cast<float4*>(w);
+  float4 pre[kSslPre];
+#pragma unroll
+  for (int q = 0; q < kSslPre; ++q) {
+    const size_t i = i0 + q * stride;
+    pre[q] = (w_vec && i < n4) ? w4[i] : make_float4(0.f, 0.f, 0.f, 0.f);
+  }
   if ((total & 3) == 0 && (reinterpret_cast<uintptr_t>(P) & 15) == 0) {
     const float4* src = reinterpret_cast<const float4*>(P);
     float4* dst = reinterpret_cast<float4*>(Ps);
@@ -404,7 +425,7 @@
   }
   __syncthreads();
   {
-    const int w = tid >> 6, lane = tid & 63;
+    const int wv = tid >> 6, lane = tid & 63;
     const int n_ent = R * (R + 1) / 2, nq = n >> 2;
     for (int e = lane; e < n_ent; e += 64) {
       int a = 0, rem = e;
@@ -414,109 +435,109 @@
       const float* pb = Ps + (size_t)b * n;
       double s = 0.0;
       if ((n & 3) == 0) {
-        for (int q = w; q < nq; q += kSslWaves) {
+        for (int q = wv; q < nq; q += kSslWaves) {
           const float4 x = *reinterpret_cast<const float4*>(pa + 4 * q), y = *reinterpret_cast<const float4*>(pb + 4 * q);
           s = fma((double)x.x, (double)y.x, s); s = fma((double)x.y, (double)y.y, s);
           s = fma((double)x.z, (double)y.z, s); s = fma((double)x.w, (double)y.w, s);
         }
       } else {
-        for (int i = w; i < n; i += kSslWaves) s = fma((double)pa[i], (double)pb[i], s);
-      }
-      gpart0[w * RR + a * R + b] = s;
-      gpart0[w * RR + b * R + a] = s;
-    }
-  }
-  __syncthreads();
-  for (int e = tid; e < RR; e += kSslThreads) {
-    double part[kSslWaves];
-#pragma unroll
-    for (int w = 0; w < kSslWaves; ++w) part[w] = gpart0[w * RR + e];
-#pragma unroll
-    for (int h = kSslWaves / 2; h >= 1; h >>= 1)
-#pragma unroll
-      for (int w = 0; w < h; ++w) part[w] = part[2 * w] + part[2 * w + 1];
-    A[e] = part[0];
-  }
-  __syncthreads();
-  double t0 = 0.0;
-  for (int a = 0; a < R; ++a) t0 += A[a * R + a];
+        for (int i = wv; i < n; i += kSslWaves) s = fma((double)pa[i], (double)pb[i], s);
+      }
+      gpart0[wv * RR + a * R + b] = s;
+      gpart0[wv * RR + b * R + a] = s;
+    }
+  }
   __syncthreads();
   __shared__ double tj_s[kSquarings + 1];
-  __shared__ double ll_s;
-  const bool zero = !(t0 > 0.0);
-  int n_it = 0;
-  if (!zero) {
-    for (int e = tid; e < RR; e += kSslThreads) A[e] /= t0;
-    __syncthreads();
-    double* cur = A;
-    double* nxt = B;
-    double c2 = 1.0;
-    for (int it = 0; it < kSquarings; ++it) {
-      for (int e = tid; e < RR; e += kSslThreads) {
-        const int a = e / R, b = e - a * R;
-        double s = 0.0;
-        for (int c = 0; c < R; ++c) s = fma(cur[a * R + c], cur[c * R + b], s);
-        nxt[e] = s * c2;
-      }
-      __syncthreads();
-      double tj = 0.0;
-      for (int a = 0; a < R; ++a) tj += nxt[a * R + a];
-      if (tid == 0) tj_s[it] = tj;
-      n_it = it + 1;
-      const double inv = 1.0 / tj;
-      c2 = inv * inv;
-      double* t = cur; cur = nxt; nxt = t;
-      if (fabs(tj - 1.0) < 1e-12) break;
-    }
-    if (tid < 64) {
+  if (tid < 64) {
+    for (int e = tid; e < RR; e += 64) {
+      double part[kSslWaves];
+#pragma unroll
+      for (int wv = 0; wv < kSslWaves; ++wv) part[wv] = gpart0[wv * RR + e];
+#pragma unroll
+      for (int h = kSslWaves / 2; h >= 1; h >>= 1)
+#pragma unroll
+        for (int wv = 0; wv < h; ++wv) part[wv] = part[2 * wv] + part[2 * wv + 1];
+      A[e] = part[0];
+    }
+    ssl_wave_sync();
+    double t0 = 0.0;
+    for (int a = 0; a < R; ++a) t0 += A[a * R + a];
+    ssl_wave_sync();
+    const bool zero = !(t0 > 0.0);
+    int n_it = 0;
+    double log_lambda = 0.0;
+    if (!zero) {
+      for (int e = tid; e < RR; e += 64) A[e] /= t0;
+      ssl_wave_sync();
+      double* cur = A;
+      double* nxt = B;
+      double c2 = 1.0;
+      for (int it = 0; it < kSquarings; ++it) {
+        for (int e = tid; e < RR; e += 64) {
+          const int a = e / R, b = e - a * R;
+          double s = 0.0;
+          for (int c = 0; c < R; ++c) s = fma(cur[a * R + c], cur[c * R + b], s);
+          nxt[e] = s * c2;
+        }
+        ssl_wave_sync();
+        double tj = 0.0;
+        for (int a = 0; a < R; ++a) tj += nxt[a * R + a];
+        if (tid == 0) tj_s[it] = tj;
+        n_it = it + 1;
+        const double inv = 1.0 / tj;
+        c2 = inv * inv;
+        double* t = cur; cur = nxt; nxt = t;
+        if (fabs(tj - 1.0) < 1e-12) break;
+      }
+      ssl_wave_sync();
       double term = 0.0;
       if (tid < n_it) term = ldexp(log(tj_s[tid]), -(tid + 1));
       term = wave_sum_d(term);
-      if (tid == 0) ll_s = log(t0) + term;
-    }
-    __syncthreads();
-  }
-  const double log_lambda = zero ? 0.0 : ll_s;
-  if (tid == 0) {
-    const bool first = blockIdx.x == 0;
-    if (first && bump) *bump += 1;
-    const double sigma = zero ? 0.0 : exp(0.5 * log_lambda);
-    if (first && sigma_out) *sigma_out = (float)sigma;
-    double sc[LIPASR_MAX_LAYERS];
-    for (int l = 0; l < oa.n_layers; ++l) sc[l] = 1.0;
-    double nrm = sigma;
-    for (int v = 0; v < oa.n_order; ++v) {
-      if (first) norms_out[v] = (float)nrm;
-      const double s = root_m(rho / (nrm + kEps), oa.n_layers);
-      sc[oa.order[v]] *= s;
-      nrm *= s;
-    }
-    if (first) norms_out[oa.n_order] = (float)nrm;
-    for (int l = 0; l < oa.n_layers; ++l) {
-      sc_s[l] = (float)sc[l];
-      if (first && scales_out) scales_out[l] = (float)sc[l];
-    }
-  }
-  __syncthreads();
-  int l = 0;
-  while (l + 1 < lp.n_layers && (int)blockIdx.x >= lp.wg_start[l + 1]) ++l;
+      log_lambda = log(t0) + term;
+    }
+    if (tid == 0) {
+      const bool first = blockIdx.x == 0;
+      if (first && bump) *bump += 1;
+      const double sigma = zero ? 0.0 : exp(0.5 * log_lambda);
+      if (first && sigma_out) *sigma_out = (float)sigma;
+      double sc[LIPASR_MAX_LAYERS];
+      for (int k = 0; k < oa.n_layers; ++k) sc[k] = 1.0;
+      double nrm = sigma;
+      for (int v = 0; v < oa.n_order; ++v) {
+        if (first) norms_out[v] = (float)nrm;
+        const double s = root_m(rho / (nrm + kEps), oa.n_layers);
+        sc[oa.order[v]] *= s;
+        nrm *= s;
+      }
+      if (first) norms_out[oa.n_order] = (float)nrm;
+      for (int k = 0; k < oa.n_layers; ++k) {
+        sc_s[k] = (float)sc[k];
+        if (first && scales_out) scales_out[k] = (float)sc[k];
+      }
+    }
+  }
+  __syncthreads();
   const float s = sc_s[l];
   if (s == 1.0f) return;
-  float* w = lp.W[l];
-  const size_t nw = (size_t)lp.rows[l] * lp.cols[l];
-  const size_t j = (size_t)((int)blockIdx.x - lp.wg_start[l]);
-  const size_t stride = (size_t)(lp.wg_start[l + 1] - lp.wg_start[l]) * kSslThreads;
-  if ((reinterpret_cast<uintptr_t>(w) & 15) == 0) {
-    const size_t n4 = nw >> 2;
-    float4* w4 = reinterpret_cast<float4*>(w);
-    for (size_t i = j * kSslThreads + threadIdx.x; i < n4; i += stride) {
+  if (w_vec) {
+#pragma unroll
+    for (int q = 0; q < kSslPre; ++q) {
+      const size_t i = i0 + q * stride;
+      if (i < n4) {
+        float4 x = pre[q];
+        x.x *= s; x.y *= s; x.z *= s; x.w *= s;
+        w4[i] = x;
+      }
+    }
+    for (size_t i = i0 + kSslPre * stride; i < n4; i += stride) {
       float4 x = w4[i];
       x.x *= s; x.y *= s; x.z *= s; x.w *= s;
       w4[i] = x;
     }
-    for (size_t i = (n4 << 2) + j * kSslThreads + threadIdx.x; i < nw; i += stride) w[i] *= s;
+    for (size_t i = (n4 << 2) + i0; i < nw; i += stride) w[i] *= s;
   } else {
-    for (size_t i = j * kSslThreads + threadIdx.x; i < nw; i += stride) w[i] *= s;
+    for (size_t i = i0; i < nw; i += stride) w[i] *= s;
   }
 }
 
diff --git a/asr-using-robust-nn_amd/lipasr/_native.py b/asr-using-robust-nn_amd/lipasr/_native.py
--- a/asr-using-robust-nn_amd/lipasr/_native.py
+++ b/asr-using-robust-nn_amd/lipasr/_native.py
@@ -87,6 +87,8 @@
     "lipasr_mlp_set_gemm_tiles": (i32, [c_h, i32]),
     "lipasr_mlp_set_fuse_bn": (i32, [c_h, i32]),
     "lipasr_mlp_set_cu_budget": (i32, [c_h, i32]),
+    "lipasr_mlp_set_fused_update": (i32, [c_h, i32, f32, f32, f32, f32, c_f, c_f, c_f]),
+    "lipasr_mlp_fused_update_state": (i32, [c_h, PI, PI]),
     "lipasr_mlp_exchange_errors": (i32, [c_h, C.POINTER(C.c_int)]),
     "lipasr_mlp_output_vjp": (i32, [c_h, c_f, c_f, c_f, c_f, i32, i32, c_f, c_f, c_s]),
     "lipasr_mlp_attack_step": (i32, [c_h, c_f, c_f, c_f, c_f, c_f, i32, f32, f32, c_s]),
diff --git a/asr-using-robust-nn_amd/lipasr/keras.py b/asr-using-robust-nn_amd/lipasr/keras.py
--- a/asr-using-robust-nn_amd/lipasr/keras.py
+++ b/asr-using-robust-nn_amd/lipasr/keras.py
@@ -509,6 +509,16 @@
         n = N.sz()
         N.check(N.lib.lipasr_mlp_grad_split(self._plan, C.byref(n)))
         return int(n.value)
+
+    def set_fused_update(self, on):
+        lr, b1, b2, eps = self._adam
+        N.check(N.lib.lipasr_mlp_set_fused_update(self._plan, 1 if on else 0, lr, b1, b2, eps, N.ptr(self._adam_m), N.ptr(self._adam_v),
+                                                  N.ptr(self._step)))
+
+    def fused_update_state(self):
+        on, pending = C.c_int(), C.c_int()
+        N.check(N.lib.lipasr_mlp_fused_update_state(self._plan, C.byref(on), C.byref(pending)))
+        return bool(on.value), bool(pending.value)
 
     def apply_adam(self, grad_scale=1.0):
         lr, b1, b2, eps = self._adam
diff --git a/asr-using-robust-nn_amd/lipasr/pipeline.py b/asr-using-robust-nn_amd/lipasr/pipeline.py
--- a/asr-using-robust-nn_amd/lipasr/pipeline.py
+++ b/asr-using-robust-nn_amd/lipasr/pipeline.py
@@ -12,8 +12,9 @@
 class TrainPipeline:
     def __init__(self, model, batch, sr_in=16000, n_samp=16000, utterance_length=44, rho=0.1, constraint="product",
                  affine=None, pgd=None, dp=None, use_graph="auto", per_layer_iters=4, extractor=None, mfcc_cus="auto",
-                 sync_inputs=True, overlap_buckets=False, sync_bn=False, train_cus="auto"):
+                 sync_inputs=True, overlap_buckets=False, sync_bn=False, train_cus="auto", fused_update=True):
         self.sync_inputs = bool(sync_inputs)
+        self.fused_update = bool(fused_update)
         if pgd:
             from .attacks import _norm_value
 
@@ -195,6 +196,15 @@
             x = self._pgd_loop(bsz, x, y)
         m.train_fwd_bwd(x, y, inv_batch=1.0 / float(global_batch), defer_dw0=defer_dw0)
 
+    def _train_and_update_1gpu(self, bsz, b, gb):
+        m = self.model
+        m.set_fused_update(self.fused_update)
+        try:
+            self._attack_and_train(bsz, b, gb)
+            self._update()
+        finally:
+            m.set_fused_update(False)
+
     def _attack_only(self, bsz, b):
         x = self._feats2[b][:bsz]
         if not self.pgd:
@@ -361,8 +371,7 @@
                 self._syncbn_step(bsz, b, gb)
             elif not self.use_graph:
                 if self.dp.world == 1:
-                    self._attack_and_train(bsz, b, gb)
-                    self._update()
+                    self._train_and_update_1gpu(bsz, b, gb)
                 elif self.overlap_buckets:
                     self._attack_and_train(bsz, b, gb, defer_dw0=True)
                     self._reduce_and_update_eager(bsz, b)
@@ -374,7 +383,7 @@
                 g = self._graphs.get((bsz, b, gb))
                 if g is None:
                     if self.dp.world == 1:
-                        g = (self._capture(lambda: (self._attack_and_train(bsz, b, gb), self._update())),)
+                        g = (self._capture(self._train_and_update_1gpu, bsz, b, gb),)
                     elif self.overlap_buckets:
                         g = (self._capture(self._attack_and_train, bsz, b, gb, True), self._capture(self._dw0, bsz, b),
                              self._capture(self._update))
diff --git a/include/lipasr.h b/include/lipasr.h
--- a/include/lipasr.h
+++ b/include/lipasr.h
@@ -134,6 +134,10 @@
 int lipasr_mlp_adam_nonneg(lipasr_mlp_t m, float* params, const float* grads, float* adam_m,
                            float* adam_v, int* step_dev, float lr, float beta1, float beta2, float eps,
                            float grad_scale, lipasr_stream_t stream);
+
+int lipasr_mlp_set_fused_update(lipasr_mlp_t m, int on, float lr, float beta1, float beta2, float eps,
+                                float* adam_m, float* adam_v, int* step_dev);
+int lipasr_mlp_fused_update_state(lipasr_mlp_t m, int* on, int* pending);
 
 int lipasr_mlp_adam_project_product(lipasr_mlp_t m, float* params, const float* grads, float* adam_m,
                                     float* adam_v, int* step_dev, float lr, float beta1, float beta2,
```

Result: no change. 3.095 million utterances/sec, median of 3 (+0.8%).
